# KyanChen/RSPrompter

Measured on NVIDIA H100. Metric: images/sec, higher is better.
Workload: dtype bf16

## Files before the change

### include/rsp_b200.h

```cpp
#ifndef RSP_B200_H_
#define RSP_B200_H_

#include <stdint.h>

#ifdef __cplusplus
extern "C" {
#endif

#define RSP_ABI_VERSION 2

int rsp_abi_version(void);
const char* rsp_last_error(void);

int rsp_gemm_bf16(const void* A, int lda, const void* W, int ldw, void* out, int ldo, int M, int N,
                  int K, const float* bias, const void* residual, int ldr, int res_fp32, int res_mod,
                  const int32_t* row_map, int act, int out_fp32, void* stream);

int rsp_conv3x3_nhwc_bf16(const void* x, int B, int H, int W, int C, const void* Wt, int ldw, void* out, int ldo,
                          int N, const float* bias, const void* residual, int ldr, int res_fp32, int act,
                          int out_fp32, void* stream);
int rsp_conv3x3_geometry_ok(int B, int H, int W, int C);

int rsp_gemm_bf16_simt(const void* A, int lda, const void* W, int ldw, void* out, int ldo, int M,
                       int N, int K, const float* bias, const void* residual, int ldr, int res_fp32,
                       int res_mod, const int32_t* row_map, int act, int out_fp32, void* stream);

int rsp_vit_attention(const void* qkv, const void* rel_h, const void* rel_w, void* out, int n_seq,
                      int T, int S, int H, int hd, void* stream);
int rsp_vit_attention_scatter(const void* qkv, const void* rel_h, const void* rel_w, void* out, int n_seq, int T,
                              int Sg, int H, int hd, const int32_t* out_row_map, void* stream);

int rsp_vit_attention_simt(const void* qkv, const void* rel_h, const void* rel_w, void* out,
                           int n_seq, int T, int S, int H, int hd, void* stream);

int rsp_layernorm(const void* in, int in_fp32, int ld_in, void* out, int out_fp32, int ld_out,
                  const float* gamma, const float* beta, const int32_t* src_map, int rows_out, int C,
                  float eps, int act, void* copy_out, int ld_copy, void* stream);

int rsp_layernorm_add(const void* x, const void* res, int res_fp32, const int32_t* res_block_map,
                      int res_block_rows, const float* gamma, const float* beta, void* out, const float* pos,
                      int pos_mod, void* out_pe, long long rows, int C, float eps, void* stream);

int rsp_patchify16(const float* img, void* out, int B, int H, int W, void* stream);

int rsp_im2col_nhwc(const void* in, void* out, int B, int H, int W, int C, int KH, int KW,
                    int stride, int pad, void* stream);

int rsp_nhwc_to_nchw(const void* in, int in_fp32, float* out, int B, int HW, int C, void* stream);

int rsp_gemm_bf16_ex(const void* A, int lda, const void* W, int ldw, void* out, int ldo, int M, int N,
                     int K, const float* bias, const void* residual, int ldr, int res_fp32, int res_mod,
                     const int32_t* row_map, int act, int out_fp32, int epi_mode, const float* ln_gamma,
                     const float* ln_beta, float ln_eps, const int32_t* res_block_map,
                     int res_block_rows, const float* hyper, float* mask_out, int grid_h, int grid_w,
                     void* stream);

int rsp_add_cast_bf16(const float* a, const float* b, void* out, long long n, long long b_mod,
                      void* stream);

int rsp_token_self_attention(const void* q, const void* k, const void* v, void* out, int N, int T,
                             int heads, int c, void* stream);
int rsp_t2i_attention(const void* q, const void* K, const void* V, int ldkv, const int32_t* kv_block, void* out,
                      int N, int Tq, int HW, void* stream);
int rsp_i2t_attention(const void* Q, const int32_t* q_block, const void* ktok, const void* vtok,
                      void* out, int N, int Tq, int HW, void* stream);


int rsp_rpn_decode(const float* head_out, int ld, const int64_t* topk_idx, int K, int B, int H, int W,
                   int A, int stride, const float* base_anchors, const float* stds4, float img_h, float img_w,
                   float min_size, int out_off, int out_ld, float* boxes, float* scores, void* stream);
int rsp_rpn_decode_shapes(const float* head_out, int ld, const int64_t* topk_idx, int K, int B, int H, int W, int A,
                          int stride, const float* base_anchors, const float* stds4, const float* img_shapes,
                          float min_size, int out_off, int out_ld, float* boxes, float* scores, void* stream);

int rsp_bbox_cls_decode(const float* cls, int ld_cls, const float* reg, int ld_reg, const float* rois,
                        const uint8_t* roi_valid, int n, int C, const float* stds4, float img_h, float img_w,
                        float score_thr, float* scores, float* boxes, int64_t* labels, void* stream);
int rsp_bbox_cls_decode_shapes(const float* cls, int ld_cls, const float* reg, int ld_reg, const float* rois,
                               const uint8_t* roi_valid, int n, int C, const float* stds4, const float* img_shapes,
                               float score_thr, float* scores, float* boxes, int64_t* labels, void* stream);

int rsp_nms_batched(const float* boxes, const int64_t* ids, const int32_t* nvalid, int B, int n, float thr,
                    void* mask_ws, float* max_coord_ws, uint8_t* keep, void* stream);
int rsp_nms_batched_topk(const float* boxes, const int64_t* ids, const int32_t* nvalid, int B, int n, float thr,
                         void* mask_ws, float* max_coord_ws, uint8_t* keep, int max_keep, void* stream);

int rsp_compact_keep(const uint8_t* keep, const float* boxes, const float* scores, const int64_t* labels,
                     int B, int n, int K, float* out_boxes, float* out_scores, int64_t* out_labels,
                     int32_t* out_index, int32_t* counts, void* stream);

int rsp_roi_align_nhwc(const void* const* feats, const float* const* pes, const int32_t* Hs,
                       const int32_t* Ws, const float* scales, int num_levels, const float* rois, int n,
                       int C, int P, float finest_scale, void* out, void* stream);

int rsp_mask_paste(const float* logits, uint8_t* out, int n, int hm, int wm, int H, int W, float thr,
                   int mode, void* stream);

int rsp_sigmoid_f32(const float* in, float* out, long long n, void* stream);

int rsp_pool2_nhwc(const void* in, void* out, int B, int H, int W, int C, int mode, void* stream);

int rsp_zero_border_nhwc(void* x, int N, int H, int W, int C, void* stream);

int rsp_sin_fold(const float* in, float* out, long long n_out, void* stream);


int rsp_groupnorm_nhwc(const void* x, float* stats_ws, const float* gamma, const float* beta, const void* up,
                       void* out, int B, int H, int W, int C, int G, float eps, int relu, void* stream);

int rsp_ms_deform_attn_sample(const void* value, const float* ow, int ld_ow, const int32_t* hs, const int32_t* ws,
                              int L, int P, int B, int NQ, void* out, void* stream);
int rsp_ms_deform_attn_sample_c(const void* value, const float* ow, int ld_ow, const int32_t* hs, const int32_t* ws,
                                int L, int P, int B, int NQ, void* out, int channels, void* stream);

int rsp_mha_small(const void* Q, int ldq, const void* K, int ldk, const void* V, int ldv, const uint64_t* mask_bits,
                  int B, int nq, int nk, void* out, void* stream);
int rsp_mha_small_hd(const void* Q, int ldq, const void* K, int ldk, const void* V, int ldv, const uint64_t* mask_bits,
                     int B, int nq, int nk, void* out, int head_dim, void* stream);

int rsp_attn_mask_bits(const float* logits, int ld, int rows, int nk, uint64_t* mask_bits, void* stream);

int rsp_resize_bilinear_nhwc(const void* x, int B, int H, int W, int C, int h, int w, void* out, void* stream);

int rsp_mask_embed_src(const float* mpp, const float* const* wts, const float* emb, const float* pos, int N,
                       int n_per_img, int hm, int wm, int h, int w, float eps, void* src, void* src_pe, void* stream);

int rsp_mask_paste_rescale(const float* maps, uint8_t* out, int n, int hm, int wm, int Hb, int Wb, int crop_h, int crop_w,
                           int H, int W, float thr, int mode, void* stream);

int rsp_query_postprocess_rescale(const float* logits, const int32_t* sel, const float* cls_scores, int n_inst, int hm,
                                  int wm, int Hb, int Wb, int crop_h, int crop_w, int H, int W, uint8_t* masks,
                                  float* part_ws, float* scores, float* boxes, void* stream);

int rsp_query_postprocess(const float* logits, const int32_t* sel, const float* cls_scores, int n_inst, int hm, int wm,
                          int H, int W, uint8_t* masks, float* part_ws, float* scores, float* boxes, void* stream);

int rsp_attn_softmax_bias(const float* scores, int lds, const float* tab, int ldt, int NT, void* P, int ldp, int n_rows,
                          int T, int S, float scale, void* stream);

int rsp_transpose_cols(const void* in, int ld, int col0, int C, int n_seq, int T, void* out, void* stream);

int rsp_split_heads(const void* in, int ld, int col0, int H, int hd, int n_seq, int T, void* out, void* stream);

int rsp_gemm_bf16_grouped(const void* A, int lda, const void* W, int ldw, void* out, int ldo, int M, int N, int K,
                          int m_group_rows, int w_group_rows, const int32_t* row_map, int out_fp32, void* stream);


int rsp_query_postprocess_bits(const float* logits, const int32_t* sel, const float* cls_scores, int n_inst, int hm,
                               int wm, uint8_t* bits, float* part_ws, float* scores, float* boxes, void* stream);

int rsp_mask_paste_bits(const float* maps, uint8_t* bits, int n, int hm, int wm, float thr, int mode, void* stream);

int rsp_mask_paste_boxes(const float* probs, const float* boxes, uint8_t* out, int n, int hm, int wm, int H, int W,
                         float thr, int packed, void* stream);

int rsp_pack_mask_bits(const uint8_t* masks, uint8_t* bits, long long rows, int W, void* stream);
int rsp_unpack_mask_bits(const uint8_t* bits, uint8_t* masks, long long rows, int W, void* stream);

int rsp_mask_rle_lengths(const uint8_t* src, int packed, const int64_t* desc, const int64_t* desc_host, int n,
                         int64_t* offsets, void* stream);
int rsp_mask_rle_write(const uint8_t* src, int packed, const int64_t* desc, int n, const int64_t* offsets, char* pool,
                       int32_t* lengths, void* stream);
int rsp_mask_rle_placed_lengths(const uint8_t* src, int packed, const int64_t* desc, const int64_t* desc_host, int n,
                                int64_t* offsets, void* stream);
int rsp_mask_rle_placed_write(const uint8_t* src, int packed, const int64_t* desc, int n, const int64_t* offsets,
                              char* pool, int32_t* lengths, void* stream);


int rsp_preprocess_u8(const uint8_t* img, int h, int w, long long stride_c, long long stride_y, long long stride_x,
                      float* out, int H, int W, const float* mean3, const float* std3, int swap_rb, float pad_value,
                      void* stream);

int rsp_patchify16_u8(const uint8_t* img, int hwc, void* out, int B, int H, int W, const float* mean3, const float* std3,
                      int swap_rb, void* stream);

int rsp_cast_f32_bf16(const float* in, void* out, long long n, void* stream);

int rsp_add_table_bf16(const void* x, const float* table, void* out, long long n, long long period, void* stream);

#ifdef __cplusplus
}
#endif
#endif
```

### rsprompter_b200/_lib.py

```python
from __future__ import annotations

import ctypes
import os
import subprocess
from pathlib import Path

import torch

_PKG_DIR = Path(__file__).resolve().parent
LIB_PATH = _PKG_DIR / "librsp_b200.so"
CSRC_DIR = _PKG_DIR / "csrc"


class RspError(RuntimeError):
    """Raised when an ``rsp_*`` entry point returns a non-zero status."""


def build_library(verbose: bool = False) -> Path:
    cmd = ["make", "-C", str(CSRC_DIR), "-j", str(os.cpu_count() or 4), "all"]
    res = subprocess.run(cmd, capture_output=True, text=True)
    if res.returncode != 0:
        raise RuntimeError(f"building librsp_b200.so failed:\n{res.stdout[-4000:]}\n{res.stderr[-4000:]}")
    if verbose:
        print(res.stdout[-2000:])
    return LIB_PATH


def _load() -> ctypes.CDLL:
    if not LIB_PATH.exists():
        raise ImportError(
            f"{LIB_PATH} not found: the CUDA extension is mandatory (no fallback path). "
            "Run `python -c 'import __graft_entry__ as g; g.build()'` or `make -C rsprompter_b200/csrc`.")
    return ctypes.CDLL(str(LIB_PATH))


_lib = _load()

_vp, _i, _f = ctypes.c_void_p, ctypes.c_int, ctypes.c_float

_SIGNATURES = {
    "rsp_abi_version": ([], _i),
    "rsp_last_error": ([], ctypes.c_char_p),
    "rsp_gemm_bf16": ([_vp, _i, _vp, _i, _vp, _i, _i, _i, _i, _vp, _vp, _i, _i, _i, _vp, _i, _i, _vp], _i),
    "rsp_gemm_bf16_simt": ([_vp, _i, _vp, _i, _vp, _i, _i, _i, _i, _vp, _vp, _i, _i, _i, _vp, _i, _i, _vp], _i),
    "rsp_vit_attention": ([_vp, _vp, _vp, _vp, _i, _i, _i, _i, _i, _vp], _i),
    "rsp_vit_attention_scatter": ([_vp, _vp, _vp, _vp, _i, _i, _i, _i, _i, _vp, _vp], _i),
    "rsp_vit_attention_simt": ([_vp, _vp, _vp, _vp, _i, _i, _i, _i, _i, _vp], _i),
    "rsp_layernorm": ([_vp, _i, _i, _vp, _i, _i, _vp, _vp, _vp, _i, _i, _f, _i, _vp, _i, _vp], _i),
    "rsp_patchify16": ([_vp, _vp, _i, _i, _i, _vp], _i),
    "rsp_layernorm_add": ([_vp, _vp, _i, _vp, _i, _vp, _vp, _vp, _vp, _i, _vp, ctypes.c_longlong, _i, _f, _vp], _i),
    "rsp_im2col_nhwc": ([_vp, _vp, _i, _i, _i, _i, _i, _i, _i, _i, _vp], _i),
    "rsp_nhwc_to_nchw": ([_vp, _i, _vp, _i, _i, _i, _vp], _i),
    "rsp_cast_f32_bf16": ([_vp, _vp, ctypes.c_longlong, _vp], _i),
    "rsp_add_table_bf16": ([_vp, _vp, _vp, ctypes.c_longlong, ctypes.c_longlong, _vp], _i),
    "rsp_gemm_bf16_ex": ([_vp, _i, _vp, _i, _vp, _i, _i, _i, _i, _vp, _vp, _i, _i, _i, _vp, _i, _i,
                          _i, _vp, _vp, _f, _vp, _i, _vp, _vp, _i, _i, _vp], _i),
    "rsp_add_cast_bf16": ([_vp, _vp, _vp, ctypes.c_longlong, ctypes.c_longlong, _vp], _i),
    "rsp_token_self_attention": ([_vp, _vp, _vp, _vp, _i, _i, _i, _i, _vp], _i),
    "rsp_t2i_attention": ([_vp, _vp, _vp, _i, _vp, _vp, _i, _i, _i, _vp], _i),
    "rsp_i2t_attention": ([_vp, _vp, _vp, _vp, _vp, _i, _i, _i, _vp], _i),
    "rsp_rpn_decode": ([_vp, _i, _vp, _i, _i, _i, _i, _i, _i, _vp, _vp, _f, _f, _f, _i, _i, _vp, _vp, _vp], _i),
    "rsp_bbox_cls_decode": ([_vp, _i, _vp, _i, _vp, _vp, _i, _i, _vp, _f, _f, _f, _vp, _vp, _vp, _vp], _i),
    "rsp_rpn_decode_shapes": ([_vp, _i, _vp, _i, _i, _i, _i, _i, _i, _vp, _vp, _vp, _f, _i, _i, _vp, _vp, _vp], _i),
    "rsp_nms_batched_topk": ([_vp, _vp, _vp, _i, _i, _f, _vp, _vp, _vp, _i, _vp], _i),
    "rsp_bbox_cls_decode_shapes": ([_vp, _i, _vp, _i, _vp, _vp, _i, _i, _vp, _vp, _f, _vp, _vp, _vp, _vp], _i),
    "rsp_nms_batched": ([_vp, _vp, _vp, _i, _i, _f, _vp, _vp, _vp, _vp], _i),
    "rsp_compact_keep": ([_vp, _vp, _vp, _vp, _i, _i, _i, _vp, _vp, _vp, _vp, _vp, _vp], _i),
    "rsp_roi_align_nhwc": ([_vp, _vp, _vp, _vp, _vp, _i, _vp, _i, _i, _i, _f, _vp, _vp], _i),
    "rsp_mask_paste": ([_vp, _vp, _i, _i, _i, _i, _i, _f, _i, _vp], _i),
    "rsp_pool2_nhwc": ([_vp, _vp, _i, _i, _i, _i, _i, _vp], _i),
    "rsp_zero_border_nhwc": ([_vp, _i, _i, _i, _i, _vp], _i),
    "rsp_sigmoid_f32": ([_vp, _vp, ctypes.c_longlong, _vp], _i),
    "rsp_mask_paste_boxes": ([_vp, _vp, _vp, _i, _i, _i, _i, _i, _f, _i, _vp], _i),
    "rsp_groupnorm_nhwc": ([_vp, _vp, _vp, _vp, _vp, _vp, _i, _i, _i, _i, _i, _f, _i, _vp], _i),
    "rsp_ms_deform_attn_sample": ([_vp, _vp, _i, _vp, _vp, _i, _i, _i, _i, _vp, _vp], _i),
    "rsp_mha_small": ([_vp, _i, _vp, _i, _vp, _i, _vp, _i, _i, _i, _vp, _vp], _i),
    "rsp_ms_deform_attn_sample_c": ([_vp, _vp, _i, _vp, _vp, _i, _i, _i, _i, _vp, _i, _vp], _i),
    "rsp_mha_small_hd": ([_vp, _i, _vp, _i, _vp, _i, _vp, _i, _i, _i, _vp, _i, _vp], _i),
    "rsp_conv3x3_nhwc_bf16": ([_vp, _i, _i, _i, _i, _vp, _i, _vp, _i, _i, _vp, _vp, _i, _i, _i, _i, _vp], _i),
    "rsp_conv3x3_geometry_ok": ([_i, _i, _i, _i], _i),
    "rsp_mask_paste_rescale": ([_vp, _vp, _i, _i, _i, _i, _i, _i, _i, _i, _i, ctypes.c_float, _i, _vp], _i),
    "rsp_query_postprocess_rescale": ([_vp, _vp, _vp, _i, _i, _i, _i, _i, _i, _i, _i, _i, _vp, _vp, _vp, _vp, _vp], _i),
    "rsp_attn_mask_bits": ([_vp, _i, _i, _i, _vp, _vp], _i),
    "rsp_resize_bilinear_nhwc": ([_vp, _i, _i, _i, _i, _i, _i, _vp, _vp], _i),
    "rsp_mask_embed_src": ([_vp, _vp, _vp, _vp, _i, _i, _i, _i, _i, _i, _f, _vp, _vp, _vp], _i),
    "rsp_query_postprocess": ([_vp, _vp, _vp, _i, _i, _i, _i, _i, _vp, _vp, _vp, _vp, _vp], _i),
    "rsp_sin_fold": ([_vp, _vp, ctypes.c_longlong, _vp], _i),
    "rsp_attn_softmax_bias": ([_vp, _i, _vp, _i, _i, _vp, _i, _i, _i, _i, _f, _vp], _i),
    "rsp_transpose_cols": ([_vp, _i, _i, _i, _i, _i, _vp, _vp], _i),
    "rsp_split_heads": ([_vp, _i, _i, _i, _i, _i, _i, _vp, _vp], _i),
    "rsp_gemm_bf16_grouped": ([_vp, _i, _vp, _i, _vp, _i, _i, _i, _i, _i, _i, _vp, _i, _vp], _i),
    "rsp_query_postprocess_bits": ([_vp, _vp, _vp, _i, _i, _i, _vp, _vp, _vp, _vp, _vp], _i),
    "rsp_mask_paste_bits": ([_vp, _vp, _i, _i, _i, _f, _i, _vp], _i),
    "rsp_pack_mask_bits": ([_vp, _vp, ctypes.c_longlong, _i, _vp], _i),
    "rsp_unpack_mask_bits": ([_vp, _vp, ctypes.c_longlong, _i, _vp], _i),
    "rsp_preprocess_u8": ([_vp, _i, _i, ctypes.c_longlong, ctypes.c_longlong, ctypes.c_longlong, _vp, _i, _i, _vp, _vp,
                           _i, _f, _vp], _i),
    "rsp_patchify16_u8": ([_vp, _i, _vp, _i, _i, _i, _vp, _vp, _i, _vp], _i),
    "rsp_mask_rle_lengths": ([_vp, _i, _vp, _vp, _i, _vp, _vp], _i),
    "rsp_mask_rle_write": ([_vp, _i, _vp, _i, _vp, _vp, _vp, _vp], _i),
    "rsp_mask_rle_placed_lengths": ([_vp, _i, _vp, _vp, _i, _vp, _vp], _i),
    "rsp_mask_rle_placed_write": ([_vp, _i, _vp, _i, _vp, _vp, _vp, _vp], _i),
}


def declared_symbols() -> list[str]:
    return sorted(_SIGNATURES)


for _name, (_args, _ret) in _SIGNATURES.items():
    _fn = getattr(_lib, _name)
    _fn.argtypes = _args
    _fn.restype = _ret

ABI_VERSION = _lib.rsp_abi_version()

launch_count = 0

trace: list | None = None
trace_scope = ""


def _log(kind: str, flops: float) -> None:
    if trace is not None:
        trace.append(dict(kind=kind, scope=trace_scope, flops=float(flops)))


def _check(status: int, what: str) -> None:
    if status != 0:
        msg = _lib.rsp_last_error()
        raise RspError(f"{what} failed (status {status}): {msg.decode() if msg else ''}")


def _ptr(t: torch.Tensor | None) -> int | None:
    if t is None:
        return None
    return t.data_ptr()


def _stream() -> int:
    return torch.cuda.current_stream().cuda_stream


def _require_cuda(*ts: torch.Tensor | None) -> None:
    cur = None
    for t in ts:
        if t is None:
            continue
        if not t.is_cuda:
            raise RspError("rsprompter_b200 kernels take CUDA tensors only (there is no CPU path)")
        if cur is None:
            cur = torch.cuda.current_device()
        if t.device.index != cur:
            raise RspError(f"tensor on cuda:{t.device.index} but the current device is cuda:{cur}: "
                           "wrap the call in torch.cuda.device(...) (one process per GPU is the supported layout)")


def _host_f4(v):
    v = tuple(float(x) for x in v)
    assert len(v) == 4
    return (ctypes.c_float * 4)(*v)


ACT = {None: 0, "none": 0, "gelu": 1, "relu": 2}


def gemm(a: torch.Tensor, w: torch.Tensor, bias: torch.Tensor | None = None, *,
         out: torch.Tensor | None = None, out_dtype: torch.dtype = torch.bfloat16,
         act: str | None = None, residual: torch.Tensor | None = None, res_mod: int = 0,
         row_map: torch.Tensor | None = None, out_rows: int | None = None,
         simt: bool = False, ln: tuple | None = None, ln64_gelu: tuple | None = None,
         res_block_map: torch.Tensor | None = None, res_block_rows: int = 0) -> torch.Tensor:
    global launch_count
    _require_cuda(a, w, bias, out, residual, row_map, res_block_map)
    assert a.dtype == torch.bfloat16 and w.dtype == torch.bfloat16, "gemm operands must be bf16"
    assert a.dim() == 2 and w.dim() == 2 and a.stride(1) == 1 and w.stride(1) == 1
    M, K = a.shape
    N, K2 = w.shape
    assert K == K2, f"gemm K mismatch {K} vs {K2}"
    if bias is not None:
        assert bias.dtype == torch.float32 and bias.numel() == N and bias.is_contiguous()
    if out is None:
        rows = out_rows if out_rows is not None else M
        out = torch.empty((rows, N), device=a.device, dtype=out_dtype)
    assert out.dim() == 2 and out.stride(1) == 1 and out.shape[1] >= N
    assert out.dtype in (torch.bfloat16, torch.float32)
    ldr = 0
    res_fp32 = 1
    if residual is not None:
        assert residual.dim() == 2 and residual.stride(1) == 1
        assert residual.dtype in (torch.bfloat16, torch.float32)
        ldr = residual.stride(0)
        res_fp32 = int(residual.dtype == torch.float32)
    if row_map is not None:
        assert row_map.dtype == torch.int32 and row_map.numel() == M and row_map.is_contiguous()
    if res_block_map is not None:
        assert res_block_map.dtype == torch.int32 and res_block_map.is_contiguous() and res_block_rows > 0
    epi, g, b, eps = 0, None, None, 1e-6
    if ln is not None:
        epi, (g, b, eps) = 1, ln
    elif ln64_gelu is not None:
        epi, (g, b, eps) = 2, ln64_gelu
    if epi or res_block_map is not None:
        assert not simt
        if g is not None:
            assert g.dtype == torch.float32 and b.dtype == torch.float32 and g.is_contiguous() and b.is_contiguous()
        st = _lib.rsp_gemm_bf16_ex(_ptr(a), a.stride(0), _ptr(w), w.stride(0), _ptr(out), out.stride(0),
                                   M, N, K, _ptr(bias), _ptr(residual), ldr, res_fp32, res_mod,
                                   _ptr(row_map), ACT[act], int(out.dtype == torch.float32), epi,
                                   _ptr(g), _ptr(b), float(eps), _ptr(res_block_map), res_block_rows,
                                   None, None, 0, 0, _stream())
    else:
        fn = _lib.rsp_gemm_bf16_simt if simt else _lib.rsp_gemm_bf16
        st = fn(_ptr(a), a.stride(0), _ptr(w), w.stride(0), _ptr(out), out.stride(0), M, N, K, _ptr(bias),
                _ptr(residual), ldr, res_fp32, res_mod, _ptr(row_map), ACT[act],
                int(out.dtype == torch.float32), _stream())
    _check(st, "rsp_gemm_bf16")
    launch_count += 1
    if not simt:
        _log("gemm", 2.0 * M * N * K)
    return out


def conv3x3_ok(B: int, H: int, W: int, C: int) -> bool:
    return bool(_lib.rsp_conv3x3_geometry_ok(B, H, W, C))


def conv3x3_nhwc(x: torch.Tensor, w: torch.Tensor, bias: torch.Tensor | None = None, *, act: str | None = None,
                 residual: torch.Tensor | None = None, out_dtype: torch.dtype = torch.bfloat16) -> torch.Tensor:
    global launch_count
    _require_cuda(x, w, bias, residual)
    B, H, W, C = x.shape
    N = w.shape[0]
    assert x.dtype == torch.bfloat16 and x.is_contiguous() and w.dtype == torch.bfloat16 and w.stride(1) == 1
    assert w.shape[1] == 9 * C
    if bias is not None:
        assert bias.dtype == torch.float32 and bias.numel() == N and bias.is_contiguous()
    ldr, res_fp32 = 0, 1
    if residual is not None:
        assert residual.dim() == 2 and residual.stride(1) == 1 and residual.shape[0] == B * H * W
        ldr, res_fp32 = residual.stride(0), int(residual.dtype == torch.float32)
    out = torch.empty(B * H * W, N, device=x.device, dtype=out_dtype)
    _check(_lib.rsp_conv3x3_nhwc_bf16(_ptr(x), B, H, W, C, _ptr(w), w.stride(0), _ptr(out), out.stride(0), N, _ptr(bias),
                                      _ptr(residual), ldr, res_fp32, ACT[act], int(out_dtype == torch.float32),
                                      _stream()), "rsp_conv3x3_nhwc_bf16")
    launch_count += 1
    _log("gemm", 2.0 * B * H * W * N * 9 * C)
    return out


def gemm_upscale_mask(a: torch.Tensor, w: torch.Tensor, bias: torch.Tensor, hyper: torch.Tensor,
                      grid_h: int, grid_w: int, out: torch.Tensor | None = None) -> torch.Tensor:
    global launch_count
    _require_cuda(a, w, bias, hyper, out)
    M, K = a.shape
    P = M // (4 * grid_h * grid_w)
    assert a.dtype == torch.bfloat16 and w.dtype == torch.bfloat16 and w.shape == (128, K)
    assert hyper.dtype == torch.float32 and hyper.shape == (P, 32) and hyper.is_contiguous()
    assert bias.dtype == torch.float32 and bias.numel() == 128
    if out is None:
        out = torch.empty((P, 4 * grid_h, 4 * grid_w), device=a.device, dtype=torch.float32)
    assert out.is_contiguous() and out.dtype == torch.float32
    st = _lib.rsp_gemm_bf16_ex(_ptr(a), a.stride(0), _ptr(w), w.stride(0), None, 0, M, 128, K, _ptr(bias),
                               None, 0, 1, 0, None, 0, 0, 3, None, None, 0.0, None, 0, _ptr(hyper),
                               _ptr(out), grid_h, grid_w, _stream())
    _check(st, "rsp_gemm_bf16_ex(upscale_mask)")
    launch_count += 1
    _log("gemm", 2.0 * M * 128 * K)
    return out


def add_cast_bf16(a: torch.Tensor, b: torch.Tensor | None = None, out: torch.Tensor | None = None) -> torch.Tensor:
    global launch_count
    _require_cuda(a, b, out)
    assert a.dtype == torch.float32 and a.is_contiguous()
    b_mod = 0
    if b is not None:
        assert b.dtype == torch.float32 and b.is_contiguous() and a.numel() % b.numel() == 0
        b_mod = b.numel() if b.numel() != a.numel() else 0
    if out is None:
        out = torch.empty(a.shape, device=a.device, dtype=torch.bfloat16)
    _check(_lib.rsp_add_cast_bf16(_ptr(a), _ptr(b), _ptr(out), a.numel(), b_mod, _stream()), "rsp_add_cast_bf16")
    launch_count += 1
    return out


def token_self_attention(q: torch.Tensor, k: torch.Tensor, v: torch.Tensor, heads: int) -> torch.Tensor:
    global launch_count
    _require_cuda(q, k, v)
    N, T, D = q.shape
    for t in (q, k, v):
        assert t.dtype == torch.bfloat16 and t.is_contiguous() and t.shape == (N, T, D)
    out = torch.empty_like(q)
    _check(_lib.rsp_token_self_attention(_ptr(q), _ptr(k), _ptr(v), _ptr(out), N, T, heads, D // heads, _stream()),
           "rsp_token_self_attention")
    launch_count += 1
    return out


def t2i_attention(q: torch.Tensor, K: torch.Tensor, V: torch.Tensor, hw: int,
                  kv_block: torch.Tensor | None = None) -> torch.Tensor:
    global launch_count
    _require_cuda(q, K, V, kv_block)
    N, Tq, C = q.shape
    assert C == 128 and q.dtype == torch.bfloat16 and q.is_contiguous()
    assert K.dtype == torch.bfloat16 and V.dtype == torch.bfloat16 and K.stride(1) == 1 and V.stride(1) == 1
    assert K.stride(0) == V.stride(0)
    assert K.shape[1] == 128 and V.shape == K.shape and K.shape[0] % hw == 0
    if kv_block is not None:
        assert kv_block.dtype == torch.int32 and kv_block.numel() == N and kv_block.is_contiguous()
    else:
        assert K.shape[0] == N * hw
    out = torch.empty_like(q)
    _check(_lib.rsp_t2i_attention(_ptr(q), _ptr(K), _ptr(V), K.stride(0), _ptr(kv_block), _ptr(out), N, Tq, hw, _stream()),
           "rsp_t2i_attention")
    launch_count += 1
    return out


def i2t_attention(Q: torch.Tensor, ktok: torch.Tensor, vtok: torch.Tensor, hw: int,
                  q_block: torch.Tensor | None = None) -> torch.Tensor:
    global launch_count
    _require_cuda(Q, ktok, vtok, q_block)
    N, Tq, C = ktok.shape
    assert C == 128 and Q.dtype == torch.bfloat16 and Q.is_contiguous() and Q.shape[1] == 128
    assert ktok.dtype == torch.bfloat16 and vtok.dtype == torch.bfloat16
    assert ktok.is_contiguous() and vtok.is_contiguous() and vtok.shape == ktok.shape
    if q_block is not None:
        assert q_block.dtype == torch.int32 and q_block.numel() == N and q_block.is_contiguous()
    else:
        assert Q.shape[0] == N * hw
    out = torch.empty((N * hw, 128), device=Q.device, dtype=torch.bfloat16)
    _check(_lib.rsp_i2t_attention(_ptr(Q), _ptr(q_block), _ptr(ktok), _ptr(vtok), _ptr(out), N, Tq, hw, _stream()),
           "rsp_i2t_attention")
    launch_count += 1
    return out


def vit_attention(qkv: torch.Tensor, rel_h: torch.Tensor, rel_w: torch.Tensor, n_seq: int, S: int,
                  H: int, hd: int, *, out: torch.Tensor | None = None, simt: bool = False,
                  out_row_map: torch.Tensor | None = None, out_rows: int | None = None) -> torch.Tensor:
    global launch_count
    _require_cuda(qkv, rel_h, rel_w, out)
    T = S * S
    D = H * hd
    if not simt and out_row_map is None and S not in (14, 32, 64) and T % 128 == 0 and S % 4 == 0:
        return vit_attention_generic(qkv, rel_h, rel_w, n_seq, S, H, hd, out=out)
    if not simt and S in (14, 32, 64):
        _log("attention_window" if S == 14 else "attention_global", 4.0 * n_seq * H * T * T * hd)
    assert qkv.dtype == torch.bfloat16 and qkv.is_contiguous() and qkv.shape == (n_seq * T, 3 * D)
    assert rel_h.dtype == torch.bfloat16 and rel_h.is_contiguous() and rel_h.shape == (2 * S - 1, hd)
    assert rel_w.dtype == torch.bfloat16 and rel_w.is_contiguous() and rel_w.shape == (2 * S - 1, hd)
    if out_row_map is not None:
        assert not simt and out_row_map.dtype == torch.int32 and out_row_map.is_contiguous()
        assert out_row_map.numel() == n_seq * T and out_rows is not None
        _require_cuda(out_row_map)
        if out is None:
            out = torch.empty((out_rows, D), device=qkv.device, dtype=torch.bfloat16)
        assert out.dtype == torch.bfloat16 and out.is_contiguous() and out.shape == (out_rows, D)
        _check(_lib.rsp_vit_attention_scatter(_ptr(qkv), _ptr(rel_h), _ptr(rel_w), _ptr(out), n_seq, T, S, H, hd,
                                              _ptr(out_row_map), _stream()), "rsp_vit_attention_scatter")
        launch_count += 1
        return out
    if out is None:
        out = torch.empty((n_seq * T, D), device=qkv.device, dtype=torch.bfloat16)
    assert out.dtype == torch.bfloat16 and out.is_contiguous() and out.shape == (n_seq * T, D)
    fn = _lib.rsp_vit_attention_simt if simt else _lib.rsp_vit_attention
    _check(fn(_ptr(qkv), _ptr(rel_h), _ptr(rel_w), _ptr(out), n_seq, T, S, H, hd, _stream()),
           "rsp_vit_attention")
    launch_count += 1
    return out


def gemm_grouped(a: torch.Tensor, w: torch.Tensor, out: torch.Tensor, N: int, m_group_rows: int, w_group_rows: int,
                 row_map: torch.Tensor | None = None) -> torch.Tensor:
    global launch_count
    _require_cuda(a, w, out, row_map)
    assert a.dtype == torch.bfloat16 and w.dtype == torch.bfloat16 and a.dim() == 2 and w.dim() == 2
    assert a.stride(1) == 1 and w.stride(1) == 1 and out.dim() == 2 and out.stride(1) == 1
    M, K = a.shape
    assert w.shape[1] == K and M % m_group_rows == 0 and m_group_rows % 128 == 0
    assert w.shape[0] >= (M // m_group_rows - 1) * w_group_rows + N and out.shape[1] >= N
    assert out.dtype in (torch.bfloat16, torch.float32)
    if row_map is not None:
        assert row_map.dtype == torch.int32 and row_map.numel() == M and row_map.is_contiguous()
    _check(_lib.rsp_gemm_bf16_grouped(_ptr(a), a.stride(0), _ptr(w), w.stride(0), _ptr(out), out.stride(0), M, N, K,
                                      m_group_rows, w_group_rows, _ptr(row_map), int(out.dtype == torch.float32),
                                      _stream()), "rsp_gemm_bf16_grouped")
    launch_count += 1
    _log("gemm", 2.0 * M * N * K)
    return out


_head_scatter_maps: dict = {}


def vit_attention_generic(qkv: torch.Tensor, rel_h: torch.Tensor, rel_w: torch.Tensor, n_seq: int, S: int, H: int,
                          hd: int, out: torch.Tensor | None = None) -> torch.Tensor:
    global launch_count
    _require_cuda(qkv, rel_h, rel_w, out)
    T, D = S * S, H * hd
    assert qkv.dtype == torch.bfloat16 and qkv.is_contiguous() and qkv.shape == (n_seq * T, 3 * D)
    assert T % 128 == 0 and S % 4 == 0 and hd % 8 == 0, "generic attention path: T % 128 == 0, S % 4 == 0"
    dev = qkv.device
    if out is None:
        out = torch.empty((n_seq * T, D), device=dev, dtype=torch.bfloat16)
    assert out.dtype == torch.bfloat16 and out.is_contiguous() and out.shape == (n_seq * T, D)
    NT = (2 * S - 1 + 15) // 16 * 16
    tabs = torch.zeros(2 * NT, hd, device=dev, dtype=torch.bfloat16)
    tabs[:2 * S - 1] = rel_h
    tabs[NT:NT + 2 * S - 1] = rel_w
    qh = torch.empty(n_seq, H * T, hd, device=dev, dtype=torch.bfloat16)
    kh = torch.empty(n_seq, H * T, hd, device=dev, dtype=torch.bfloat16)
    vt = torch.empty(n_seq, D, T, device=dev, dtype=torch.bfloat16)
    _check(_lib.rsp_split_heads(_ptr(qkv), 3 * D, 0, H, hd, n_seq, T, _ptr(qh), _stream()), "rsp_split_heads")
    _check(_lib.rsp_split_heads(_ptr(qkv), 3 * D, D, H, hd, n_seq, T, _ptr(kh), _stream()), "rsp_split_heads")
    _check(_lib.rsp_transpose_cols(_ptr(qkv), 3 * D, 2 * D, D, n_seq, T, _ptr(vt), _stream()), "rsp_transpose_cols")
    launch_count += 3
    key = (T, H, dev)
    if key not in _head_scatter_maps:
        t = torch.arange(T, device=dev, dtype=torch.int32)
        h = torch.arange(H, device=dev, dtype=torch.int32)
        _head_scatter_maps[key] = (t.view(1, T) * H + h.view(H, 1)).reshape(-1).contiguous()
    rmap = _head_scatter_maps[key]
    scores = torch.empty(H * T, T, device=dev, dtype=torch.float32)
    tab = torch.empty(H * T, 2 * NT, device=dev, dtype=torch.float32)
    P = torch.empty(H * T, T, device=dev, dtype=torch.bfloat16)
    scale = float(hd) ** -0.5
    for b in range(n_seq):
        gemm_grouped(qh[b], kh[b], scores, T, T, T)
        gemm(qh[b], tabs, out=tab)
        _check(_lib.rsp_attn_softmax_bias(_ptr(scores), T, _ptr(tab), 2 * NT, NT, _ptr(P), T, H * T, T, S, scale,
                                          _stream()), "rsp_attn_softmax_bias")
        launch_count += 1
        gemm_grouped(P, vt[b], out[b * T:(b + 1) * T].view(T * H, hd), hd, T, hd, row_map=rmap)
    return out


def layernorm(x: torch.Tensor, gamma: torch.Tensor, beta: torch.Tensor, eps: float, *,
              out: torch.Tensor | None = None, out_dtype: torch.dtype = torch.bfloat16,
              src_map: torch.Tensor | None = None, gelu: bool = False,
              copy_out: torch.Tensor | None = None) -> torch.Tensor:
    global launch_count
    _require_cuda(x, gamma, beta, out, src_map, copy_out)
    if copy_out is not None:
        assert x.dtype == torch.float32 and copy_out.dtype == torch.bfloat16 and copy_out.shape == x.shape
        assert copy_out.stride(1) == 1
    assert x.dim() == 2 and x.stride(1) == 1 and x.dtype in (torch.float32, torch.bfloat16)
    C = x.shape[1]
    assert gamma.dtype == torch.float32 and beta.dtype == torch.float32
    assert gamma.numel() == C and beta.numel() == C and gamma.is_contiguous() and beta.is_contiguous()
    rows_out = src_map.numel() if src_map is not None else x.shape[0]
    if src_map is not None:
        assert src_map.dtype == torch.int32 and src_map.is_contiguous()
    if out is None:
        out = torch.empty((rows_out, C), device=x.device, dtype=out_dtype)
    assert out.shape == (rows_out, C) and out.stride(1) == 1
    _check(_lib.rsp_layernorm(_ptr(x), int(x.dtype == torch.float32), x.stride(0), _ptr(out),
                              int(out.dtype == torch.float32), out.stride(0), _ptr(gamma), _ptr(beta),
                              _ptr(src_map), rows_out, C, float(eps), int(gelu), _ptr(copy_out),
                              copy_out.stride(0) if copy_out is not None else 0, _stream()),
           "rsp_layernorm")
    launch_count += 1
    return out


def patchify16(img: torch.Tensor, out: torch.Tensor | None = None) -> torch.Tensor:
    global launch_count
    _require_cuda(img, out)
    assert img.dtype == torch.float32 and img.is_contiguous() and img.dim() == 4 and img.shape[1] == 3
    B, _, H, W = img.shape
    rows = B * (H // 16) * (W // 16)
    if out is None:
        out = torch.empty((rows, 768), device=img.device, dtype=torch.bfloat16)
    assert out.shape == (rows, 768) and out.is_contiguous() and out.dtype == torch.bfloat16
    _check(_lib.rsp_patchify16(_ptr(img), _ptr(out), B, H, W, _stream()), "rsp_patchify16")
    launch_count += 1
    return out


def im2col_nhwc(x: torch.Tensor, kh: int, kw: int, stride: int, pad: int,
                out: torch.Tensor | None = None) -> torch.Tensor:
    global launch_count
    _require_cuda(x, out)
    assert x.dtype == torch.bfloat16 and x.is_contiguous() and x.dim() == 4
    B, H, W, C = x.shape
    Ho = (H + 2 * pad - kh) // stride + 1
    Wo = (W + 2 * pad - kw) // stride + 1
    if out is None:
        out = torch.empty((B * Ho * Wo, kh * kw * C), device=x.device, dtype=torch.bfloat16)
    assert out.shape == (B * Ho * Wo, kh * kw * C) and out.is_contiguous()
    _check(_lib.rsp_im2col_nhwc(_ptr(x), _ptr(out), B, H, W, C, kh, kw, stride, pad, _stream()),
           "rsp_im2col_nhwc")
    launch_count += 1
    return out


def nhwc_to_nchw(x: torch.Tensor, out: torch.Tensor | None = None) -> torch.Tensor:
    global launch_count
    _require_cuda(x, out)
    assert x.is_contiguous() and x.dim() == 4 and x.dtype in (torch.float32, torch.bfloat16)
    B, H, W, C = x.shape
    if out is None:
        out = torch.empty((B, C, H, W), device=x.device, dtype=torch.float32)
    assert out.shape == (B, C, H, W) and out.is_contiguous() and out.dtype == torch.float32
    _check(_lib.rsp_nhwc_to_nchw(_ptr(x), int(x.dtype == torch.float32), _ptr(out), B, H * W, C, _stream()),
           "rsp_nhwc_to_nchw")
    launch_count += 1
    return out


def cast_bf16(x: torch.Tensor, out: torch.Tensor | None = None) -> torch.Tensor:
    global launch_count
    _require_cuda(x, out)
    assert x.dtype == torch.float32 and x.is_contiguous()
    if out is None:
        out = torch.empty(x.shape, device=x.device, dtype=torch.bfloat16)
    assert out.is_contiguous() and out.numel() == x.numel() and out.dtype == torch.bfloat16
    _check(_lib.rsp_cast_f32_bf16(_ptr(x), _ptr(out), x.numel(), _stream()), "rsp_cast_f32_bf16")
    launch_count += 1
    return out


def add_table_bf16(x: torch.Tensor, table: torch.Tensor) -> torch.Tensor:
    global launch_count
    _require_cuda(x, table)
    assert x.dtype == torch.bfloat16 and x.is_contiguous() and table.dtype == torch.float32 and table.is_contiguous()
    assert x.numel() % table.numel() == 0 and table.numel() % 8 == 0
    out = torch.empty_like(x)
    _check(_lib.rsp_add_table_bf16(_ptr(x), _ptr(table), _ptr(out), x.numel(), table.numel(), _stream()),
           "rsp_add_table_bf16")
    launch_count += 1
    return out


def rpn_decode(head_out: torch.Tensor, topk_idx: torch.Tensor, B: int, H: int, W: int, A: int, stride: int,
               base_anchors: torch.Tensor, img_hw: tuple, min_size: float, boxes: torch.Tensor,
               scores: torch.Tensor, out_off: int, stds=(1.0, 1.0, 1.0, 1.0),
               img_shapes: torch.Tensor | None = None) -> None:
    global launch_count
    _require_cuda(head_out, topk_idx, base_anchors, boxes, scores)
    assert head_out.dtype == torch.float32 and head_out.dim() == 2 and head_out.stride(1) == 1
    assert topk_idx.dtype == torch.int64 and topk_idx.is_contiguous() and topk_idx.shape[0] == B
    assert boxes.is_contiguous() and scores.is_contiguous() and boxes.dtype == torch.float32
    K = topk_idx.shape[1]
    if img_shapes is not None:
        _require_cuda(img_shapes)
        assert img_shapes.dtype == torch.float32 and img_shapes.is_contiguous() and img_shapes.shape == (B, 2)
        _check(_lib.rsp_rpn_decode_shapes(_ptr(head_out), head_out.stride(0), _ptr(topk_idx), K, B, H, W, A, stride,
                                          _ptr(base_anchors), _host_f4(stds), _ptr(img_shapes), float(min_size), out_off,
                                          scores.shape[1], _ptr(boxes), _ptr(scores), _stream()), "rsp_rpn_decode_shapes")
        launch_count += 1
        return
    _check(_lib.rsp_rpn_decode(_ptr(head_out), head_out.stride(0), _ptr(topk_idx), K, B, H, W, A, stride,
                               _ptr(base_anchors), _host_f4(stds), float(img_hw[0]), float(img_hw[1]), float(min_size),
                               out_off, scores.shape[1], _ptr(boxes), _ptr(scores), _stream()), "rsp_rpn_decode")
    launch_count += 1


def bbox_cls_decode(cls: torch.Tensor, reg: torch.Tensor, rois: torch.Tensor, roi_valid: torch.Tensor | None,
                    C: int, img_hw: tuple, score_thr: float, stds=(0.1, 0.1, 0.2, 0.2),
                    img_shapes: torch.Tensor | None = None):
    global launch_count
    _require_cuda(cls, reg, rois, roi_valid)
    n = rois.shape[0]
    assert cls.dtype == torch.float32 and reg.dtype == torch.float32 and rois.dtype == torch.float32
    assert cls.stride(1) == 1 and reg.stride(1) == 1 and rois.is_contiguous() and rois.shape[1] == 5
    scores = torch.empty(n * C, device=cls.device, dtype=torch.float32)
    boxes = torch.empty(n * C, 4, device=cls.device, dtype=torch.float32)
    labels = torch.empty(n * C, device=cls.device, dtype=torch.int64)
    if roi_valid is not None:
        assert roi_valid.dtype == torch.uint8 and roi_valid.numel() == n
    if img_shapes is not None:
        _require_cuda(img_shapes)
        assert img_shapes.dtype == torch.float32 and img_shapes.is_contiguous() and img_shapes.shape[1] == 2
        _check(_lib.rsp_bbox_cls_decode_shapes(_ptr(cls), cls.stride(0), _ptr(reg), reg.stride(0), _ptr(rois),
                                               _ptr(roi_valid), n, C, _host_f4(stds), _ptr(img_shapes), float(score_thr),
                                               _ptr(scores), _ptr(boxes), _ptr(labels), _stream()),
               "rsp_bbox_cls_decode_shapes")
    else:
        _check(_lib.rsp_bbox_cls_decode(_ptr(cls), cls.stride(0), _ptr(reg), reg.stride(0), _ptr(rois),
                                        _ptr(roi_valid), n, C, _host_f4(stds), float(img_hw[0]), float(img_hw[1]),
                                        float(score_thr), _ptr(scores), _ptr(boxes), _ptr(labels), _stream()),
               "rsp_bbox_cls_decode")
    launch_count += 1
    return scores, boxes, labels


def nms_batched(boxes: torch.Tensor, ids: torch.Tensor, nvalid: torch.Tensor, iou_thr: float,
                max_keep: int = 0) -> torch.Tensor:
    global launch_count
    _require_cuda(boxes, ids, nvalid)
    B, n, _ = boxes.shape
    assert boxes.dtype == torch.float32 and boxes.is_contiguous()
    assert ids.dtype == torch.int64 and ids.is_contiguous() and ids.shape == (B, n)
    assert nvalid.dtype == torch.int32 and nvalid.numel() == B
    words = (n + 63) // 64
    mask_ws = torch.empty(B * n * words, device=boxes.device, dtype=torch.int64)
    mx = torch.empty(B, device=boxes.device, dtype=torch.float32)
    keep = torch.empty(B, n, device=boxes.device, dtype=torch.uint8)
    _check(_lib.rsp_nms_batched_topk(_ptr(boxes), _ptr(ids), _ptr(nvalid), B, n, float(iou_thr), _ptr(mask_ws),
                                     _ptr(mx), _ptr(keep), int(max_keep), _stream()), "rsp_nms_batched_topk")
    launch_count += 3
    return keep


def compact_keep(keep: torch.Tensor, boxes: torch.Tensor, scores: torch.Tensor, labels: torch.Tensor | None,
                 K: int):
    global launch_count
    _require_cuda(keep, boxes, scores, labels)
    B, n = keep.shape
    dev = keep.device
    ob = torch.empty(B, K, 4, device=dev, dtype=torch.float32)
    os_ = torch.empty(B, K, device=dev, dtype=torch.float32)
    ol = torch.empty(B, K, device=dev, dtype=torch.int64) if labels is not None else None
    oi = torch.empty(B, K, device=dev, dtype=torch.int32)
    cnt = torch.empty(B, device=dev, dtype=torch.int32)
    assert boxes.is_contiguous() and scores.is_contiguous() and keep.is_contiguous()
    _check(_lib.rsp_compact_keep(_ptr(keep), _ptr(boxes), _ptr(scores), _ptr(labels), B, n, K, _ptr(ob),
                                 _ptr(os_), _ptr(ol), _ptr(oi), _ptr(cnt), _stream()), "rsp_compact_keep")
    launch_count += 1
    return ob, os_, ol, oi, cnt
# ... 458 lines not shown
```

### rsprompter_b200/csrc/abi.cu

```cuda
#include "../../include/rsp_b200.h"

#include "attention.h"
#include "gemm.h"
#include "rowops.h"

namespace rsp { const char* last_error(); }
using namespace rsp;

static inline cudaStream_t S(void* s) { return static_cast<cudaStream_t>(s); }

extern "C" {

int rsp_abi_version(void) { return RSP_ABI_VERSION; }
const char* rsp_last_error(void) { return rsp::last_error(); }

static GemmArgs make_gemm_args(const void* A, int lda, const void* W, int ldw, void* out, int ldo,
                               int M, int N, int K, const float* bias, const void* residual, int ldr,
                               int res_fp32, int res_mod, const int32_t* row_map, int act,
                               int out_fp32) {
  GemmArgs a;
  a.A = A; a.lda = lda; a.W = W; a.ldw = ldw; a.out = out; a.ldo = ldo;
  a.M = M; a.N = N; a.K = K; a.bias = bias; a.residual = residual; a.ldr = ldr;
  a.res_fp32 = res_fp32; a.res_mod = res_mod; a.row_map = row_map; a.act = act;
  a.out_fp32 = out_fp32;
  return a;
}

int rsp_gemm_bf16(const void* A, int lda, const void* W, int ldw, void* out, int ldo, int M, int N,
                  int K, const float* bias, const void* residual, int ldr, int res_fp32, int res_mod,
                  const int32_t* row_map, int act, int out_fp32, void* stream) {
  return gemm_bf16(make_gemm_args(A, lda, W, ldw, out, ldo, M, N, K, bias, residual, ldr, res_fp32,
                                  res_mod, row_map, act, out_fp32), S(stream));
}

int rsp_gemm_bf16_grouped(const void* A, int lda, const void* W, int ldw, void* out, int ldo, int M, int N, int K,
                          int m_group_rows, int w_group_rows, const int32_t* row_map, int out_fp32, void* stream) {
  GemmArgs a = make_gemm_args(A, lda, W, ldw, out, ldo, M, N, K, nullptr, nullptr, 0, 1, 0, row_map, 0, out_fp32);
  a.m_group_rows = m_group_rows; a.w_group_rows = w_group_rows;
  return gemm_bf16(a, S(stream));
}

int rsp_conv3x3_nhwc_bf16(const void* x, int B, int H, int W, int C, const void* Wt, int ldw, void* out, int ldo,
                          int N, const float* bias, const void* residual, int ldr, int res_fp32, int act,
                          int out_fp32, void* stream) {
  GemmArgs a = make_gemm_args(x, C, Wt, ldw, out, ldo, B * H * W, N, 9 * C, bias, residual, ldr, res_fp32, 0,
                              nullptr, act, out_fp32);
  a.conv_b = B; a.conv_h = H; a.conv_w = W; a.conv_c = C;
  return conv3x3_bf16(a, S(stream));
}

int rsp_conv3x3_geometry_ok(int B, int H, int W, int C) { return conv3x3_geometry_ok(B, H, W, C) ? 1 : 0; }

int rsp_gemm_bf16_simt(const void* A, int lda, const void* W, int ldw, void* out, int ldo, int M,
                       int N, int K, const float* bias, const void* residual, int ldr, int res_fp32,
                       int res_mod, const int32_t* row_map, int act, int out_fp32, void* stream) {
  return gemm_bf16_simt(make_gemm_args(A, lda, W, ldw, out, ldo, M, N, K, bias, residual, ldr,
                                       res_fp32, res_mod, row_map, act, out_fp32), S(stream));
}

static AttentionArgs make_att_args(const void* qkv, const void* rel_h, const void* rel_w, void* out,
                                   int n_seq, int T, int Sg, int H, int hd, const int32_t* out_row_map = nullptr) {
  AttentionArgs a;
  a.qkv = qkv; a.rel_h = rel_h; a.rel_w = rel_w; a.out = out;
  a.n_seq = n_seq; a.T = T; a.S = Sg; a.H = H; a.hd = hd; a.out_row_map = out_row_map;
  return a;
}

int rsp_vit_attention(const void* qkv, const void* rel_h, const void* rel_w, void* out, int n_seq,
                      int T, int Sg, int H, int hd, void* stream) {
  return vit_attention(make_att_args(qkv, rel_h, rel_w, out, n_seq, T, Sg, H, hd), S(stream));
}

int rsp_vit_attention_scatter(const void* qkv, const void* rel_h, const void* rel_w, void* out, int n_seq, int T,
                              int Sg, int H, int hd, const int32_t* out_row_map, void* stream) {
  return vit_attention(make_att_args(qkv, rel_h, rel_w, out, n_seq, T, Sg, H, hd, out_row_map), S(stream));
}

int rsp_vit_attention_simt(const void* qkv, const void* rel_h, const void* rel_w, void* out,
                           int n_seq, int T, int Sg, int H, int hd, void* stream) {
  return vit_attention_simt(make_att_args(qkv, rel_h, rel_w, out, n_seq, T, Sg, H, hd), S(stream));
}

int rsp_attn_softmax_bias(const float* scores, int lds, const float* tab, int ldt, int NT, void* P, int ldp, int n_rows,
                          int T, int Sg, float scale, void* stream) {
  return attn_softmax_bias(scores, lds, tab, ldt, NT, P, ldp, n_rows, T, Sg, scale, S(stream));
}

int rsp_transpose_cols(const void* in, int ld, int col0, int C, int n_seq, int T, void* out, void* stream) {
  return transpose_cols(in, ld, col0, C, n_seq, T, out, S(stream));
}

int rsp_split_heads(const void* in, int ld, int col0, int H, int hd, int n_seq, int T, void* out, void* stream) {
  return split_heads(in, ld, col0, H, hd, n_seq, T, out, S(stream));
}

int rsp_layernorm(const void* in, int in_fp32, int ld_in, void* out, int out_fp32, int ld_out,
                  const float* gamma, const float* beta, const int32_t* src_map, int rows_out, int C,
                  float eps, int act, void* copy_out, int ld_copy, void* stream) {
  LayerNormArgs a;
  a.copy_out = copy_out; a.ld_copy = ld_copy;
  a.in = in; a.in_fp32 = in_fp32; a.ld_in = ld_in; a.out = out; a.out_fp32 = out_fp32;
  a.ld_out = ld_out; a.gamma = gamma; a.beta = beta; a.src_map = src_map; a.rows_out = rows_out;
  a.C = C; a.eps = eps; a.act = act;
  return layernorm_rows(a, S(stream));
}

int rsp_layernorm_add(const void* x, const void* res, int res_fp32, const int32_t* res_block_map,
                      int res_block_rows, const float* gamma, const float* beta, void* out, const float* pos,
                      int pos_mod, void* out_pe, long long rows, int C, float eps, void* stream) {
  return layernorm_add(x, res, res_fp32, res_block_map, res_block_rows, gamma, beta, out, pos, pos_mod, out_pe, rows,
                       C, eps, S(stream));
}

int rsp_patchify16(const float* img, void* out, int B, int H, int W, void* stream) {
  return patchify16(img, out, B, H, W, S(stream));
}

int rsp_im2col_nhwc(const void* in, void* out, int B, int H, int W, int C, int KH, int KW,
                    int stride, int pad, void* stream) {
  return im2col_nhwc(in, out, B, H, W, C, KH, KW, stride, pad, S(stream));
}

int rsp_nhwc_to_nchw(const void* in, int in_fp32, float* out, int B, int HW, int C, void* stream) {
  return nhwc_to_nchw(in, in_fp32, out, B, HW, C, S(stream));
}

int rsp_cast_f32_bf16(const float* in, void* out, long long n, void* stream) {
  return cast_f32_bf16(in, out, n, S(stream));
}

int rsp_add_table_bf16(const void* x, const float* table, void* out, long long n, long long period, void* stream) {
  return add_table_bf16(x, table, out, n, period, S(stream));
}

}

#include "decoder.h"

extern "C" {

int rsp_gemm_bf16_ex(const void* A, int lda, const void* W, int ldw, void* out, int ldo, int M, int N,
                     int K, const float* bias, const void* residual, int ldr, int res_fp32, int res_mod,
                     const int32_t* row_map, int act, int out_fp32, int epi_mode, const float* ln_gamma,
                     const float* ln_beta, float ln_eps, const int32_t* res_block_map,
                     int res_block_rows, const float* hyper, float* mask_out, int grid_h, int grid_w,
                     void* stream) {
  GemmArgs a = make_gemm_args(A, lda, W, ldw, out, ldo, M, N, K, bias, residual, ldr, res_fp32,
                              res_mod, row_map, act, out_fp32);
  a.epi_mode = epi_mode; a.ln_gamma = ln_gamma; a.ln_beta = ln_beta; a.ln_eps = ln_eps;
  a.res_block_map = res_block_map; a.res_block_rows = res_block_rows;
  a.hyper = hyper; a.mask_out = mask_out; a.grid_h = grid_h; a.grid_w = grid_w;
  return gemm_bf16(a, S(stream));
}

int rsp_add_cast_bf16(const float* a, const float* b, void* out, long long n, long long b_mod,
                      void* stream) {
  return add_cast_bf16(a, b, out, n, b_mod, S(stream));
}

int rsp_token_self_attention(const void* q, const void* k, const void* v, void* out, int N, int T,
                             int heads, int c, void* stream) {
  return token_self_attention(q, k, v, out, N, T, heads, c, S(stream));
}

int rsp_t2i_attention(const void* q, const void* K, const void* V, int ldkv, const int32_t* kv_block, void* out,
                      int N, int Tq, int HW, void* stream) {
  return t2i_attention(q, K, V, ldkv, kv_block, out, N, Tq, HW, S(stream));
}

int rsp_i2t_attention(const void* Q, const int32_t* q_block, const void* ktok, const void* vtok,
                      void* out, int N, int Tq, int HW, void* stream) {
  return i2t_attention(Q, q_block, ktok, vtok, out, N, Tq, HW, S(stream));
}

}

#include "detect.h"

extern "C" {

int rsp_rpn_decode(const float* head_out, int ld, const int64_t* topk_idx, int K, int B, int H, int W,
                   int A, int stride, const float* base_anchors, const float* stds4, float img_h, float img_w,
                   float min_size, int out_off, int out_ld, float* boxes, float* scores, void* stream) {
  return rpn_decode(head_out, ld, reinterpret_cast<const long long*>(topk_idx), K, B, H, W, A, stride,
                    base_anchors, stds4, img_h, img_w, nullptr, min_size, out_off, out_ld, boxes, scores, S(stream));
}

int rsp_rpn_decode_shapes(const float* head_out, int ld, const int64_t* topk_idx, int K, int B, int H, int W, int A,
                          int stride, const float* base_anchors, const float* stds4, const float* img_shapes,
                          float min_size, int out_off, int out_ld, float* boxes, float* scores, void* stream) {
  RSP_CHECK_ARG(img_shapes, "rpn_decode_shapes: img_shapes is null");
  return rpn_decode(head_out, ld, reinterpret_cast<const long long*>(topk_idx), K, B, H, W, A, stride,
                    base_anchors, stds4, 0.f, 0.f, img_shapes, min_size, out_off, out_ld, boxes, scores, S(stream));
}

int rsp_bbox_cls_decode(const float* cls, int ld_cls, const float* reg, int ld_reg, const float* rois,
                        const uint8_t* roi_valid, int n, int C, const float* stds4, float img_h, float img_w,
                        float score_thr, float* scores, float* boxes, int64_t* labels, void* stream) {
  return bbox_cls_decode(cls, ld_cls, reg, ld_reg, rois, roi_valid, n, C, stds4, img_h, img_w, nullptr, score_thr,
                         scores, boxes, reinterpret_cast<long long*>(labels), S(stream));
}

int rsp_bbox_cls_decode_shapes(const float* cls, int ld_cls, const float* reg, int ld_reg, const float* rois,
                               const uint8_t* roi_valid, int n, int C, const float* stds4, const float* img_shapes,
                               float score_thr, float* scores, float* boxes, int64_t* labels, void* stream) {
  RSP_CHECK_ARG(img_shapes, "bbox_cls_decode_shapes: img_shapes is null");
  return bbox_cls_decode(cls, ld_cls, reg, ld_reg, rois, roi_valid, n, C, stds4, 0.f, 0.f, img_shapes, score_thr,
                         scores, boxes, reinterpret_cast<long long*>(labels), S(stream));
}

int rsp_nms_batched(const float* boxes, const int64_t* ids, const int32_t* nvalid, int B, int n, float thr,
                    void* mask_ws, float* max_coord_ws, uint8_t* keep, void* stream) {
  return nms_batched(boxes, reinterpret_cast<const long long*>(ids), nvalid, B, n, thr,
                     static_cast<unsigned long long*>(mask_ws), max_coord_ws, keep, 0, S(stream));
}

int rsp_nms_batched_topk(const float* boxes, const int64_t* ids, const int32_t* nvalid, int B, int n, float thr,
                         void* mask_ws, float* max_coord_ws, uint8_t* keep, int max_keep, void* stream) {
  return nms_batched(boxes, reinterpret_cast<const long long*>(ids), nvalid, B, n, thr,
                     static_cast<unsigned long long*>(mask_ws), max_coord_ws, keep, max_keep, S(stream));
}

int rsp_compact_keep(const uint8_t* keep, const float* boxes, const float* scores, const int64_t* labels,
                     int B, int n, int K, float* out_boxes, float* out_scores, int64_t* out_labels,
                     int32_t* out_index, int32_t* counts, void* stream) {
  return compact_keep(keep, boxes, scores, reinterpret_cast<const long long*>(labels), B, n, K, out_boxes,
                      out_scores, reinterpret_cast<long long*>(out_labels), out_index, counts, S(stream));
}

int rsp_roi_align_nhwc(const void* const* feats, const float* const* pes, const int32_t* Hs,
                       const int32_t* Ws, const float* scales, int num_levels, const float* rois, int n,
                       int C, int P, float finest_scale, void* out, void* stream) {
  return roi_align_nhwc(feats, pes, Hs, Ws, scales, num_levels, rois, n, C, P, finest_scale, out, S(stream));
}

int rsp_mask_paste(const float* logits, uint8_t* out, int n, int hm, int wm, int H, int W, float thr,
                   int mode, void* stream) {
  return mask_paste(logits, out, n, hm, wm, H, W, thr, mode, S(stream));
}

int rsp_sigmoid_f32(const float* in, float* out, long long n, void* stream) {
  return sigmoid_f32(in, out, n, S(stream));
}

int rsp_pool2_nhwc(const void* in, void* out, int B, int H, int W, int C, int mode, void* stream) {
  return pool2_nhwc(in, out, B, H, W, C, mode, S(stream));
}

int rsp_zero_border_nhwc(void* x, int N, int H, int W, int C, void* stream) {
  return zero_border_nhwc(x, N, H, W, C, S(stream));
}

int rsp_sin_fold(const float* in, float* out, long long n_out, void* stream) {
  return sin_fold(in, out, n_out, S(stream));
}

}

#include "query.h"

extern "C" {

int rsp_groupnorm_nhwc(const void* x, float* stats_ws, const float* gamma, const float* beta, const void* up,
                       void* out, int B, int H, int W, int C, int G, float eps, int relu, void* stream) {
  return groupnorm_nhwc(x, stats_ws, gamma, beta, up, out, B, H, W, C, G, eps, relu, S(stream));
}

int rsp_ms_deform_attn_sample(const void* value, const float* ow, int ld_ow, const int32_t* hs, const int32_t* ws,
                              int L, int P, int B, int NQ, void* out, void* stream) {
  return ms_deform_attn_sample(value, ow, ld_ow, hs, ws, L, P, B, NQ, out, 128, S(stream));
}

int rsp_ms_deform_attn_sample_c(const void* value, const float* ow, int ld_ow, const int32_t* hs, const int32_t* ws,
                                int L, int P, int B, int NQ, void* out, int channels, void* stream) {
  return ms_deform_attn_sample(value, ow, ld_ow, hs, ws, L, P, B, NQ, out, channels, S(stream));
}

int rsp_mha_small(const void* Q, int ldq, const void* K, int ldk, const void* V, int ldv, const uint64_t* mask_bits,
                  int B, int nq, int nk, void* out, void* stream) {
  return mha_small(Q, ldq, K, ldk, V, ldv, reinterpret_cast<const unsigned long long*>(mask_bits), B, nq, nk, out, 16,
                   S(stream));
}

int rsp_mha_small_hd(const void* Q, int ldq, const void* K, int ldk, const void* V, int ldv, const uint64_t* mask_bits,
                     int B, int nq, int nk, void* out, int head_dim, void* stream) {
  return mha_small(Q, ldq, K, ldk, V, ldv, reinterpret_cast<const unsigned long long*>(mask_bits), B, nq, nk, out,
                   head_dim, S(stream));
}

int rsp_attn_mask_bits(const float* logits, int ld, int rows, int nk, uint64_t* mask_bits, void* stream) {
  return attn_mask_bits(logits, ld, rows, nk, reinterpret_cast<unsigned long long*>(mask_bits), S(stream));
}

int rsp_resize_bilinear_nhwc(const void* x, int B, int H, int W, int C, int h, int w, void* out, void* stream) {
  return resize_bilinear_nhwc(x, B, H, W, C, h, w, out, S(stream));
}

int rsp_mask_embed_src(const float* mpp, const float* const* wts, const float* emb, const float* pos, int N,
                       int n_per_img, int hm, int wm, int h, int w, float eps, void* src, void* src_pe, void* stream) {
  return mask_embed_src(mpp, wts, emb, pos, N, n_per_img, hm, wm, h, w, eps, src, src_pe, S(stream));
}

int rsp_mask_paste_rescale(const float* maps, uint8_t* out, int n, int hm, int wm, int Hb, int Wb, int crop_h, int crop_w,
                           int H, int W, float thr, int mode, void* stream) {
  return mask_paste_rescale(maps, out, n, hm, wm, Hb, Wb, crop_h, crop_w, H, W, thr, mode, S(stream));
}

int rsp_query_postprocess_rescale(const float* logits, const int32_t* sel, const float* cls_scores, int n_inst, int hm,
                                  int wm, int Hb, int Wb, int crop_h, int crop_w, int H, int W, uint8_t* masks,
                                  float* part_ws, float* scores, float* boxes, void* stream) {
  return query_postprocess_rescale(logits, sel, cls_scores, n_inst, hm, wm, Hb, Wb, crop_h, crop_w, H, W, masks, part_ws,
                                   scores, boxes, S(stream));
}

int rsp_query_postprocess(const float* logits, const int32_t* sel, const float* cls_scores, int n_inst, int hm, int wm,
                          int H, int W, uint8_t* masks, float* part_ws, float* scores, float* boxes, void* stream) {
  return query_postprocess(logits, sel, cls_scores, n_inst, hm, wm, H, W, masks, part_ws, scores, boxes, S(stream));
}

int rsp_query_postprocess_bits(const float* logits, const int32_t* sel, const float* cls_scores, int n_inst, int hm,
                               int wm, uint8_t* bits, float* part_ws, float* scores, float* boxes, void* stream) {
  return query_postprocess_bits(logits, sel, cls_scores, n_inst, hm, wm, bits, part_ws, scores, boxes, S(stream));
}

int rsp_mask_paste_boxes(const float* probs, const float* boxes, uint8_t* out, int n, int hm, int wm, int H, int W,
                         float thr, int packed, void* stream) {
  return mask_paste_boxes(probs, boxes, out, n, hm, wm, H, W, thr, packed, S(stream));
}

int rsp_mask_paste_bits(const float* maps, uint8_t* bits, int n, int hm, int wm, float thr, int mode, void* stream) {
  return mask_paste_bits(maps, bits, n, hm, wm, thr, mode, S(stream));
}

}

#include "records.h"

extern "C" {

int rsp_pack_mask_bits(const uint8_t* masks, uint8_t* bits, long long rows, int W, void* stream) {
  return pack_mask_bits(masks, bits, rows, W, S(stream));
}

int rsp_unpack_mask_bits(const uint8_t* bits, uint8_t* masks, long long rows, int W, void* stream) {
  return unpack_mask_bits(bits, masks, rows, W, S(stream));
}

int rsp_preprocess_u8(const uint8_t* img, int h, int w, long long stride_c, long long stride_y, long long stride_x,
                      float* out, int H, int W, const float* mean3, const float* std3, int swap_rb, float pad_value,
                      void* stream) {
  return preprocess_u8(img, h, w, stride_c, stride_y, stride_x, out, H, W, mean3, std3, swap_rb, pad_value, S(stream));
}

int rsp_patchify16_u8(const uint8_t* img, int hwc, void* out, int B, int H, int W, const float* mean3, const float* std3,
                      int swap_rb, void* stream) {
  return patchify16_u8(img, hwc, out, B, H, W, mean3, std3, swap_rb, S(stream));
}

}

#include "rle.h"

extern "C" {

int rsp_mask_rle_lengths(const uint8_t* src, int packed, const int64_t* desc, const int64_t* desc_host, int n,
                         int64_t* offsets, void* stream) {
  return mask_rle_lengths(src, packed, reinterpret_cast<const long long*>(desc),
                          reinterpret_cast<const long long*>(desc_host), n, reinterpret_cast<long long*>(offsets),
                          S(stream));
}

int rsp_mask_rle_write(const uint8_t* src, int packed, const int64_t* desc, int n, const int64_t* offsets, char* pool,
                       int32_t* lengths, void* stream) {
  return mask_rle_write(src, packed, reinterpret_cast<const long long*>(desc), n,
                        reinterpret_cast<const long long*>(offsets), pool, lengths, S(stream));
}

int rsp_mask_rle_placed_lengths(const uint8_t* src, int packed, const int64_t* desc, const int64_t* desc_host, int n,
                                int64_t* offsets, void* stream) {
  return mask_rle_placed_lengths(src, packed, reinterpret_cast<const long long*>(desc),
                                 reinterpret_cast<const long long*>(desc_host), n, reinterpret_cast<long long*>(offsets),
                                 S(stream));
}

int rsp_mask_rle_placed_write(const uint8_t* src, int packed, const int64_t* desc, int n, const int64_t* offsets,
                              char* pool, int32_t* lengths, void* stream) {
  return mask_rle_placed_write(src, packed, reinterpret_cast<const long long*>(desc), n,
                               reinterpret_cast<const long long*>(offsets), pool, lengths, S(stream));
}

}
```

### rsprompter_b200/csrc/decoder.cu

```cuda
#include "decoder.h"
#include "sm90.cuh"

namespace rsp {

__device__ __forceinline__ void unpack8(const uint4& u, float (&f)[8]) {
  const uint32_t w[4] = {u.x, u.y, u.z, u.w};
#pragma unroll
  for (int j = 0; j < 4; ++j) {
    const __nv_bfloat162 h = *reinterpret_cast<const __nv_bfloat162*>(&w[j]);
    f[2 * j] = __bfloat162float(h.x);
    f[2 * j + 1] = __bfloat162float(h.y);
  }
}

__global__ void add_cast_bf16_kernel(const float* __restrict__ a, const float* __restrict__ b,
                                     __nv_bfloat16* __restrict__ out, long long n, long long b_mod) {
  const long long i = (static_cast<long long>(blockIdx.x) * blockDim.x + threadIdx.x) * 4;
  if (i >= n) return;
  float4 x = *reinterpret_cast<const float4*>(a + i);
  if (b) {
    const float4 y = *reinterpret_cast<const float4*>(b + (b_mod > 0 ? i % b_mod : i));
    x.x += y.x; x.y += y.y; x.z += y.z; x.w += y.w;
  }
  *reinterpret_cast<uint2*>(out + i) = make_uint2(pack_bf16x2(x.x, x.y), pack_bf16x2(x.z, x.w));
}

int add_cast_bf16(const float* a, const float* b, void* out, long long n, long long b_mod,
                  cudaStream_t stream) {
  RSP_CHECK_ARG(a && out && n > 0 && n % 4 == 0 && (b_mod == 0 || b_mod % 4 == 0), "add_cast: bad args");
  const long long n4 = n / 4;
  add_cast_bf16_kernel<<<static_cast<unsigned>((n4 + 255) / 256), 256, 0, stream>>>(
      a, b, static_cast<__nv_bfloat16*>(out), n, b_mod);
  RSP_CHECK_LAUNCH();
  return RSP_OK;
}

template <int C>
__global__ void token_self_attention_kernel(const __nv_bfloat16* __restrict__ q,
                                            const __nv_bfloat16* __restrict__ k,
                                            const __nv_bfloat16* __restrict__ v,
                                            __nv_bfloat16* __restrict__ out, int N, int T, int heads,
                                            float scale) {
  const int gw = (blockIdx.x * blockDim.x + threadIdx.x) >> 5;
  const int lane = threadIdx.x & 31;
  if (gw >= N * heads) return;
  const int n = gw / heads, h = gw % heads;
  const int D = heads * C;
  if (lane >= T) return;
  const __nv_bfloat16* qp = q + (static_cast<size_t>(n) * T + lane) * D + h * C;
  float qf[C];
#pragma unroll
  for (int d = 0; d < C; d += 8) {
    float t[8];
    unpack8(*reinterpret_cast<const uint4*>(qp + d), t);
#pragma unroll
    for (int j = 0; j < 8; ++j) qf[d + j] = t[j];
  }
  float s[16];
  float mx = -INFINITY;
  for (int j = 0; j < T; ++j) {
    const __nv_bfloat16* kp = k + (static_cast<size_t>(n) * T + j) * D + h * C;
    float acc = 0.f;
#pragma unroll
    for (int d = 0; d < C; d += 8) {
      float t[8];
      unpack8(*reinterpret_cast<const uint4*>(kp + d), t);
#pragma unroll
      for (int jj = 0; jj < 8; ++jj) acc += qf[d + jj] * t[jj];
    }
    s[j] = acc * scale;
    mx = fmaxf(mx, s[j]);
  }
  float l = 0.f;
  float o[C];
#pragma unroll
  for (int d = 0; d < C; ++d) o[d] = 0.f;
  for (int j = 0; j < T; ++j) {
    const float pj = __expf(s[j] - mx);
    l += pj;
    const __nv_bfloat16* vp = v + (static_cast<size_t>(n) * T + j) * D + h * C;
#pragma unroll
    for (int d = 0; d < C; d += 8) {
      float t[8];
      unpack8(*reinterpret_cast<const uint4*>(vp + d), t);
#pragma unroll
      for (int jj = 0; jj < 8; ++jj) o[d + jj] += pj * t[jj];
    }
  }
  const float inv = 1.0f / l;
  __nv_bfloat16* op = out + (static_cast<size_t>(n) * T + lane) * D + h * C;
#pragma unroll
  for (int d = 0; d < C; d += 8)
    *reinterpret_cast<uint4*>(op + d) =
        make_uint4(pack_bf16x2(o[d] * inv, o[d + 1] * inv), pack_bf16x2(o[d + 2] * inv, o[d + 3] * inv),
                   pack_bf16x2(o[d + 4] * inv, o[d + 5] * inv), pack_bf16x2(o[d + 6] * inv, o[d + 7] * inv));
}

int token_self_attention(const void* q, const void* k, const void* v, void* out, int N, int T,
                         int heads, int c, cudaStream_t stream) {
  RSP_CHECK_ARG(q && k && v && out && N > 0 && T > 0 && T <= 16 && heads > 0, "token_self_attention: bad args");
  RSP_CHECK_ARG(c == 32 || c == 16, "token_self_attention: per-head dim %d (16 or 32)", c);
  const int warps = N * heads;
  const int threads = 128;
  const int blocks = (warps * 32 + threads - 1) / threads;
  const float scale = 1.0f / sqrtf(static_cast<float>(c));
  if (c == 32)
    token_self_attention_kernel<32><<<blocks, threads, 0, stream>>>(
        static_cast<const __nv_bfloat16*>(q), static_cast<const __nv_bfloat16*>(k),
        static_cast<const __nv_bfloat16*>(v), static_cast<__nv_bfloat16*>(out), N, T, heads, scale);
  else
    token_self_attention_kernel<16><<<blocks, threads, 0, stream>>>(
        static_cast<const __nv_bfloat16*>(q), static_cast<const __nv_bfloat16*>(k),
        static_cast<const __nv_bfloat16*>(v), static_cast<__nv_bfloat16*>(out), N, T, heads, scale);
  RSP_CHECK_LAUNCH();
  return RSP_OK;
}

constexpr int T2I_TILE = 64;
constexpr int T2I_ROWB = 272;
constexpr int T2I_STAGE = 2 * T2I_TILE * T2I_ROWB;

__device__ __forceinline__ void mma_bf16_16816(float (&d)[4], const uint32_t (&a)[4], uint32_t b0, uint32_t b1) {
  asm volatile(
      "mma.sync.aligned.m16n8k16.row.col.f32.bf16.bf16.f32 {%0, %1, %2, %3}, {%4, %5, %6, %7}, {%8, %9}, "
      "{%0, %1, %2, %3};"
      : "+f"(d[0]), "+f"(d[1]), "+f"(d[2]), "+f"(d[3])
      : "r"(a[0]), "r"(a[1]), "r"(a[2]), "r"(a[3]), "r"(b0), "r"(b1));
}

__device__ __forceinline__ void cp_async16(uint32_t dst, const void* src) {
  asm volatile("cp.async.cg.shared.global [%0], [%1], 16;" ::"r"(dst), "l"(src) : "memory");
}

__global__ void __launch_bounds__(256)
t2i_attention_kernel(const __nv_bfloat16* __restrict__ q,
                     const __nv_bfloat16* __restrict__ K,
                     const __nv_bfloat16* __restrict__ V,
                     const int* __restrict__ kv_block,
                     __nv_bfloat16* __restrict__ out,
                     int Tq, int HW, int ldkv, float scale) {
  extern __shared__ __align__(16) uint8_t t2i_smem[];
  const uint32_t s_base = smem_u32(t2i_smem);
  const int n = blockIdx.x;
  const int blk = kv_block ? kv_block[n] : n;
  const __nv_bfloat16* Kb = K + static_cast<size_t>(blk) * HW * ldkv;
  const __nv_bfloat16* Vb = V + static_cast<size_t>(blk) * HW * ldkv;
  const int tid = threadIdx.x, lane = tid & 31, h = tid >> 5;
  const int g = lane >> 2, t = lane & 3;
  const int n_tiles = (HW + T2I_TILE - 1) / T2I_TILE;

  auto issue_tile = [&](int tile, int stage) {
    const int t0 = tile * T2I_TILE;
#pragma unroll
    for (int i = 0; i < 8; ++i) {
      const int idx = tid + i * 256;
      const int which = idx >> 10, j = idx & 1023;
      const int row = j >> 4, ch = j & 15;
      const int grow = min(t0 + row, HW - 1);
      const __nv_bfloat16* src = (which ? Vb : Kb) + static_cast<size_t>(grow) * ldkv + ch * 8;
      cp_async16(s_base + stage * T2I_STAGE + which * (T2I_TILE * T2I_ROWB) + row * T2I_ROWB + ch * 16, src);
    }
    asm volatile("cp.async.commit_group;" ::: "memory");
  };

  uint32_t qa[4];
  {
    auto ldq = [&](int row, int col) -> uint32_t {
      if (row >= Tq) return 0u;
      const __nv_bfloat162 v = *reinterpret_cast<const __nv_bfloat162*>(
          q + (static_cast<size_t>(n) * Tq + row) * 128 + h * 16 + col);
      return pack_bf16x2(__bfloat162float(v.x) * scale, __bfloat162float(v.y) * scale);
    };
    qa[0] = ldq(g, 2 * t); qa[1] = ldq(g + 8, 2 * t); qa[2] = ldq(g, 2 * t + 8); qa[3] = ldq(g + 8, 2 * t + 8);
  }
  float m0 = -INFINITY, m1 = -INFINITY, l0 = 0.f, l1 = 0.f;
  float o[2][4] = {{0.f, 0.f, 0.f, 0.f}, {0.f, 0.f, 0.f, 0.f}};

  issue_tile(0, 0);
  for (int tile = 0; tile < n_tiles; ++tile) {
    const int stage = tile & 1;
    if (tile + 1 < n_tiles) {
      issue_tile(tile + 1, stage ^ 1);
      asm volatile("cp.async.wait_group 1;" ::: "memory");
    } else {
      asm volatile("cp.async.wait_group 0;" ::: "memory");
    }
    __syncthreads();
    const uint32_t sK = s_base + stage * T2I_STAGE + h * 32;
    const uint32_t sV = sK + T2I_TILE * T2I_ROWB;
    const int valid = min(T2I_TILE, HW - tile * T2I_TILE);
    float s[8][4];
#pragma unroll
    for (int j = 0; j < 8; ++j) {
      uint32_t b0, b1;
      const uint32_t addr = sK + (j * 8 + g) * T2I_ROWB + t * 4;
      asm volatile("ld.shared.b32 %0, [%1];" : "=r"(b0) : "r"(addr));
      asm volatile("ld.shared.b32 %0, [%1];" : "=r"(b1) : "r"(addr + 16));
      s[j][0] = s[j][1] = s[j][2] = s[j][3] = 0.f;
      mma_bf16_16816(s[j], qa, b0, b1);
      if (valid < T2I_TILE) {
        const int key = j * 8 + 2 * t;
        if (key >= valid) { s[j][0] = -INFINITY; s[j][2] = -INFINITY; }
        if (key + 1 >= valid) { s[j][1] = -INFINITY; s[j][3] = -INFINITY; }
      }
    }
    float mx0 = -INFINITY, mx1 = -INFINITY;
#pragma unroll
    for (int j = 0; j < 8; ++j) {
      mx0 = fmaxf(mx0, fmaxf(s[j][0], s[j][1]));
      mx1 = fmaxf(mx1, fmaxf(s[j][2], s[j][3]));
    }
    mx0 = fmaxf(mx0, __shfl_xor_sync(0xffffffffu, mx0, 1)); mx0 = fmaxf(mx0, __shfl_xor_sync(0xffffffffu, mx0, 2));
    mx1 = fmaxf(mx1, __shfl_xor_sync(0xffffffffu, mx1, 1)); mx1 = fmaxf(mx1, __shfl_xor_sync(0xffffffffu, mx1, 2));
    const float mn0 = fmaxf(m0, mx0), mn1 = fmaxf(m1, mx1);
    const float a0 = __expf(m0 - mn0), a1 = __expf(m1 - mn1);
    m0 = mn0; m1 = mn1;
    float ps0 = 0.f, ps1 = 0.f;
#pragma unroll
    for (int j = 0; j < 8; ++j) {
      s[j][0] = __expf(s[j][0] - mn0); s[j][1] = __expf(s[j][1] - mn0);
      s[j][2] = __expf(s[j][2] - mn1); s[j][3] = __expf(s[j][3] - mn1);
      ps0 += s[j][0] + s[j][1];
      ps1 += s[j][2] + s[j][3];
    }
    l0 = l0 * a0 + ps0; l1 = l1 * a1 + ps1;
#pragma unroll
    for (int d = 0; d < 2; ++d) { o[d][0] *= a0; o[d][1] *= a0; o[d][2] *= a1; o[d][3] *= a1; }
#pragma unroll
    for (int c = 0; c < 4; ++c) {
      uint32_t pa[4];
      pa[0] = pack_bf16x2(s[2 * c][0], s[2 * c][1]);
      pa[1] = pack_bf16x2(s[2 * c][2], s[2 * c][3]);
      pa[2] = pack_bf16x2(s[2 * c + 1][0], s[2 * c + 1][1]);
      pa[3] = pack_bf16x2(s[2 * c + 1][2], s[2 * c + 1][3]);
#pragma unroll
      for (int d = 0; d < 2; ++d) {
        const uint32_t addr = sV + (c * 16 + 2 * t) * T2I_ROWB + (d * 8 + g) * 2;
        uint16_t v00, v01, v10, v11;
        asm volatile("ld.shared.u16 %0, [%1];" : "=h"(v00) : "r"(addr));
        asm volatile("ld.shared.u16 %0, [%1];" : "=h"(v01) : "r"(addr + T2I_ROWB));
        asm volatile("ld.shared.u16 %0, [%1];" : "=h"(v10) : "r"(addr + 8 * T2I_ROWB));
        asm volatile("ld.shared.u16 %0, [%1];" : "=h"(v11) : "r"(addr + 9 * T2I_ROWB));
        const uint32_t b0 = static_cast<uint32_t>(v00) | (static_cast<uint32_t>(v01) << 16);
        const uint32_t b1 = static_cast<uint32_t>(v10) | (static_cast<uint32_t>(v11) << 16);
        mma_bf16_16816(o[d], pa, b0, b1);
      }
    }
    __syncthreads();
  }
  l0 += __shfl_xor_sync(0xffffffffu, l0, 1); l0 += __shfl_xor_sync(0xffffffffu, l0, 2);
  l1 += __shfl_xor_sync(0xffffffffu, l1, 1); l1 += __shfl_xor_sync(0xffffffffu, l1, 2);
  const float i0 = 1.0f / l0, i1 = 1.0f / l1;
#pragma unroll
  for (int d = 0; d < 2; ++d) {
    if (g < Tq)
      *reinterpret_cast<uint32_t*>(out + (static_cast<size_t>(n) * Tq + g) * 128 + h * 16 + d * 8 + 2 * t) =
          pack_bf16x2(o[d][0] * i0, o[d][1] * i0);
    if (g + 8 < Tq)
      *reinterpret_cast<uint32_t*>(out + (static_cast<size_t>(n) * Tq + g + 8) * 128 + h * 16 + d * 8 + 2 * t) =
          pack_bf16x2(o[d][2] * i1, o[d][3] * i1);
  }
}

int t2i_attention(const void* q, const void* K, const void* V, int ldkv, const int* kv_block, void* out, int N,
                  int Tq, int HW, cudaStream_t stream) {
  RSP_CHECK_ARG(q && K && V && out && N > 0 && Tq > 0 && Tq <= 16 && HW > 0, "t2i_attention: bad args");
  RSP_CHECK_ARG(ldkv >= 128 && ldkv % 8 == 0 && (reinterpret_cast<uintptr_t>(K) & 15) == 0 &&
                (reinterpret_cast<uintptr_t>(V) & 15) == 0, "t2i_attention: K / V row stride / alignment");
  const int smem = 2 * T2I_STAGE;
  static bool attr_set_dev[kMaxDevices] = {};
  bool& attr_set = attr_set_dev[current_device()];
  if (!attr_set) {
    RSP_CHECK_CUDA(cudaFuncSetAttribute(t2i_attention_kernel, cudaFuncAttributeMaxDynamicSharedMemorySize, smem));
    attr_set = true;
  }
  t2i_attention_kernel<<<N, 256, smem, stream>>>(
      static_cast<const __nv_bfloat16*>(q), static_cast<const __nv_bfloat16*>(K),
      static_cast<const __nv_bfloat16*>(V), kv_block, static_cast<__nv_bfloat16*>(out), Tq, HW, ldkv, 0.25f);
  RSP_CHECK_LAUNCH();
  return RSP_OK;
}

constexpr int I2T_PIX = 128;
constexpr int I2T_ROWB = 272;

__global__ void __launch_bounds__(256)
i2t_attention_kernel(const __nv_bfloat16* __restrict__ Q,
                     const int* __restrict__ q_block,
                     const __nv_bfloat16* __restrict__ ktok,
                     const __nv_bfloat16* __restrict__ vtok,
                     __nv_bfloat16* __restrict__ out,
                     int Tq, int HW, float scale) {
  __shared__ __align__(16) uint8_t tile[I2T_PIX * I2T_ROWB];
  const uint32_t s_tile = smem_u32(tile);
  const int n = blockIdx.y;
  const int p0 = blockIdx.x * I2T_PIX;
  const int tid = threadIdx.x, lane = tid & 31, h = tid >> 5;
  const int g = lane >> 2, t = lane & 3;
  const int blk = q_block ? q_block[n] : n;
  const __nv_bfloat16* Qb = Q + (static_cast<size_t>(blk) * HW + p0) * 128;
  const int npix = min(I2T_PIX, HW - p0);
#pragma unroll
  for (int i = 0; i < 8; ++i) {
    const int idx = tid + i * 256;
    const int row = idx >> 4, ch = idx & 15;
    const int srow = min(row, npix - 1);
    cp_async16(s_tile + row * I2T_ROWB + ch * 16, Qb + static_cast<size_t>(srow) * 128 + ch * 8);
  }
  asm volatile("cp.async.commit_group;" ::: "memory");
  uint32_t kb[2][2], vb[2][2];
  {
    const __nv_bfloat16* kp = ktok + static_cast<size_t>(n) * Tq * 128 + h * 16;
    const __nv_bfloat16* vp = vtok + static_cast<size_t>(n) * Tq * 128 + h * 16;
#pragma unroll
    for (int j = 0; j < 2; ++j) {
      const int tok = j * 8 + g;
      kb[j][0] = kb[j][1] = 0u;
      if (tok < Tq) {
        const __nv_bfloat162 k0 = *reinterpret_cast<const __nv_bfloat162*>(kp + tok * 128 + 2 * t);
        const __nv_bfloat162 k1 = *reinterpret_cast<const __nv_bfloat162*>(kp + tok * 128 + 2 * t + 8);
        kb[j][0] = pack_bf16x2(__bfloat162float(k0.x) * scale, __bfloat162float(k0.y) * scale);
        kb[j][1] = pack_bf16x2(__bfloat162float(k1.x) * scale, __bfloat162float(k1.y) * scale);
      }
      auto ldv = [&](int tok2) -> uint32_t {
        return tok2 < Tq ? static_cast<uint32_t>(*reinterpret_cast<const uint16_t*>(vp + tok2 * 128 + j * 8 + g)) : 0u;
      };
      vb[j][0] = ldv(2 * t) | (ldv(2 * t + 1) << 16);
      vb[j][1] = ldv(2 * t + 8) | (ldv(2 * t + 9) << 16);
    }
  }
  asm volatile("cp.async.wait_group 0;" ::: "memory");
  __syncthreads();
  const uint32_t sq = s_tile + h * 32;
#pragma unroll 2
  for (int c = 0; c < I2T_PIX / 16; ++c) {
    uint32_t qa[4];
    const uint32_t a0 = sq + (c * 16 + g) * I2T_ROWB + t * 4;
    asm volatile("ld.shared.b32 %0, [%1];" : "=r"(qa[0]) : "r"(a0));
    asm volatile("ld.shared.b32 %0, [%1];" : "=r"(qa[1]) : "r"(a0 + 8 * I2T_ROWB));
    asm volatile("ld.shared.b32 %0, [%1];" : "=r"(qa[2]) : "r"(a0 + 16));
    asm volatile("ld.shared.b32 %0, [%1];" : "=r"(qa[3]) : "r"(a0 + 8 * I2T_ROWB + 16));
    float s0[4] = {0.f, 0.f, 0.f, 0.f}, s1[4] = {0.f, 0.f, 0.f, 0.f};
    mma_bf16_16816(s0, qa, kb[0][0], kb[0][1]);
    mma_bf16_16816(s1, qa, kb[1][0], kb[1][1]);
    if (2 * t >= Tq) { s0[0] = -INFINITY; s0[2] = -INFINITY; }
    if (2 * t + 1 >= Tq) { s0[1] = -INFINITY; s0[3] = -INFINITY; }
    if (8 + 2 * t >= Tq) { s1[0] = -INFINITY; s1[2] = -INFINITY; }
    if (9 + 2 * t >= Tq) { s1[1] = -INFINITY; s1[3] = -INFINITY; }
    float m0 = fmaxf(fmaxf(s0[0], s0[1]), fmaxf(s1[0], s1[1]));
    float m1 = fmaxf(fmaxf(s0[2], s0[3]), fmaxf(s1[2], s1[3]));
    m0 = fmaxf(m0, __shfl_xor_sync(0xffffffffu, m0, 1)); m0 = fmaxf(m0, __shfl_xor_sync(0xffffffffu, m0, 2));
    m1 = fmaxf(m1, __shfl_xor_sync(0xffffffffu, m1, 1)); m1 = fmaxf(m1, __shfl_xor_sync(0xffffffffu, m1, 2));
    s0[0] = __expf(s0[0] - m0); s0[1] = __expf(s0[1] - m0); s1[0] = __expf(s1[0] - m0); s1[1] = __expf(s1[1] - m0);
    s0[2] = __expf(s0[2] - m1); s0[3] = __expf(s0[3] - m1); s1[2] = __expf(s1[2] - m1); s1[3] = __expf(s1[3] - m1);
    float l0 = s0[0] + s0[1] + s1[0] + s1[1], l1 = s0[2] + s0[3] + s1[2] + s1[3];
    l0 += __shfl_xor_sync(0xffffffffu, l0, 1); l0 += __shfl_xor_sync(0xffffffffu, l0, 2);
    l1 += __shfl_xor_sync(0xffffffffu, l1, 1); l1 += __shfl_xor_sync(0xffffffffu, l1, 2);
    uint32_t pa[4] = {pack_bf16x2(s0[0], s0[1]), pack_bf16x2(s0[2], s0[3]), pack_bf16x2(s1[0], s1[1]),
                      pack_bf16x2(s1[2], s1[3])};
    float o0[4] = {0.f, 0.f, 0.f, 0.f}, o1[4] = {0.f, 0.f, 0.f, 0.f};
    mma_bf16_16816(o0, pa, vb[0][0], vb[0][1]);
    mma_bf16_16816(o1, pa, vb[1][0], vb[1][1]);
    const float i0 = 1.0f / l0, i1 = 1.0f / l1;
    __syncwarp();
    asm volatile("st.shared.b32 [%0], %1;" ::"r"(a0), "r"(pack_bf16x2(o0[0] * i0, o0[1] * i0)) : "memory");
    asm volatile("st.shared.b32 [%0], %1;" ::"r"(a0 + 8 * I2T_ROWB), "r"(pack_bf16x2(o0[2] * i1, o0[3] * i1)) : "memory");
    asm volatile("st.shared.b32 [%0], %1;" ::"r"(a0 + 16), "r"(pack_bf16x2(o1[0] * i0, o1[1] * i0)) : "memory");
    asm volatile("st.shared.b32 [%0], %1;" ::"r"(a0 + 8 * I2T_ROWB + 16), "r"(pack_bf16x2(o1[2] * i1, o1[3] * i1)) : "memory");
  }
  __syncthreads();
  __nv_bfloat16* Ob = out + (static_cast<size_t>(n) * HW + p0) * 128;
#pragma unroll
  for (int i = 0; i < 8; ++i) {
    const int idx = tid + i * 256;
    const int row = idx >> 4, ch = idx & 15;
    if (row < npix)
      *reinterpret_cast<uint4*>(Ob + static_cast<size_t>(row) * 128 + ch * 8) =
          *reinterpret_cast<const uint4*>(tile + row * I2T_ROWB + ch * 16);
  }
}

int i2t_attention(const void* Q, const int* q_block, const void* ktok, const void* vtok, void* out,
                  int N, int Tq, int HW, cudaStream_t stream) {
  RSP_CHECK_ARG(Q && ktok && vtok && out && N > 0 && Tq > 0 && Tq <= 16 && HW > 0, "i2t_attention: bad args");
  dim3 grid((HW + I2T_PIX - 1) / I2T_PIX, N);
  i2t_attention_kernel<<<grid, 256, 0, stream>>>(
      static_cast<const __nv_bfloat16*>(Q), q_block, static_cast<const __nv_bfloat16*>(ktok),
      static_cast<const __nv_bfloat16*>(vtok), static_cast<__nv_bfloat16*>(out), Tq, HW, 0.25f);
  RSP_CHECK_LAUNCH();
  return RSP_OK;
}

}
```

### rsprompter_b200/csrc/decoder.h

```cpp
#pragma once
#include "host_util.h"

namespace rsp {

int add_cast_bf16(const float* a, const float* b, void* out, long long n, long long b_mod,
                  cudaStream_t stream);
int token_self_attention(const void* q, const void* k, const void* v, void* out, int N, int T,
                         int heads, int c, cudaStream_t stream);
int t2i_attention(const void* q, const void* K, const void* V, int ldkv, const int* kv_block, void* out, int N,
                  int Tq, int HW, cudaStream_t stream);
int i2t_attention(const void* Q, const int* q_block, const void* ktok, const void* vtok, void* out,
                  int N, int Tq, int HW, cudaStream_t stream);

}
```

### rsprompter_b200/csrc/sm90.cuh

```cuda
#pragma once
#include <cuda.h>
#include <cuda_bf16.h>
#include <cuda_runtime.h>
#include <stdint.h>

namespace rsp {

__device__ __forceinline__ uint32_t smem_u32(const void* p) {
  return static_cast<uint32_t>(__cvta_generic_to_shared(p));
}

__device__ __forceinline__ uint32_t elect_one() {
  uint32_t pred = 0;
  asm volatile(
      "{\n"
      ".reg .b32 rx;\n"
      ".reg .pred px;\n"
      "elect.sync rx|px, 0xffffffff;\n"
      "selp.u32 %0, 1, 0, px;\n"
      "}\n"
      : "=r"(pred));
  return pred;
}

__device__ __forceinline__ void mbar_init(uint32_t bar, uint32_t count) {
  asm volatile("mbarrier.init.shared::cta.b64 [%0], %1;" ::"r"(bar), "r"(count) : "memory");
}
__device__ __forceinline__ void fence_barrier_init() {
  asm volatile("fence.mbarrier_init.release.cluster;" ::: "memory");
}
__device__ __forceinline__ void fence_proxy_async_smem() {
  asm volatile("fence.proxy.async.shared::cta;" ::: "memory");
}
__device__ __forceinline__ void mbar_expect_tx(uint32_t bar, uint32_t bytes) {
  asm volatile("mbarrier.arrive.expect_tx.shared::cta.b64 _, [%0], %1;" ::"r"(bar), "r"(bytes)
               : "memory");
}
__device__ __forceinline__ void mbar_arrive(uint32_t bar) {
  asm volatile("mbarrier.arrive.shared::cta.b64 _, [%0];" ::"r"(bar) : "memory");
}
__device__ __forceinline__ uint32_t mbar_try_wait(uint32_t bar, uint32_t parity) {
  uint32_t ok;
  asm volatile(
      "{\n"
      ".reg .pred p;\n"
      "mbarrier.try_wait.parity.shared::cta.b64 p, [%1], %2;\n"
      "selp.u32 %0, 1, 0, p;\n"
      "}\n"
      : "=r"(ok)
      : "r"(bar), "r"(parity)
      : "memory");
  return ok;
}
__device__ __forceinline__ void mbar_wait(uint32_t bar, uint32_t parity) {
  if (mbar_try_wait(bar, parity)) return;
  long long t0 = clock64();
  uint32_t spins = 0;
  while (!mbar_try_wait(bar, parity)) {
    if ((++spins & 0x3ff) == 0 && clock64() - t0 > (1ll << 31)) __trap();
  }
}

__device__ __forceinline__ void tma_prefetch_desc(const CUtensorMap* m) {
  asm volatile("prefetch.tensormap [%0];" ::"l"(m) : "memory");
}
__device__ __forceinline__ void tma_load_2d(uint32_t dst, const CUtensorMap* m, uint32_t bar,
                                            int c0, int c1) {
  asm volatile(
      "cp.async.bulk.tensor.2d.shared::cluster.global.mbarrier::complete_tx::bytes"
      " [%0], [%1, {%3, %4}], [%2];" ::"r"(dst),
      "l"(m), "r"(bar), "r"(c0), "r"(c1)
      : "memory");
}
__device__ __forceinline__ void tma_load_3d(uint32_t dst, const CUtensorMap* m, uint32_t bar,
                                            int c0, int c1, int c2) {
  asm volatile(
      "cp.async.bulk.tensor.3d.shared::cluster.global.mbarrier::complete_tx::bytes"
      " [%0], [%1, {%3, %4, %5}], [%2];" ::"r"(dst),
      "l"(m), "r"(bar), "r"(c0), "r"(c1), "r"(c2)
      : "memory");
}
__device__ __forceinline__ void tma_load_4d(uint32_t dst, const CUtensorMap* m, uint32_t bar,
                                            int c0, int c1, int c2, int c3) {
  asm volatile(
      "cp.async.bulk.tensor.4d.shared::cluster.global.mbarrier::complete_tx::bytes"
      " [%0], [%1, {%3, %4, %5, %6}], [%2];" ::"r"(dst),
      "l"(m), "r"(bar), "r"(c0), "r"(c1), "r"(c2), "r"(c3)
      : "memory");
}

__device__ __forceinline__ void tma_store_2d(const CUtensorMap* m, uint32_t src, int c0, int c1) {
  asm volatile("cp.async.bulk.tensor.2d.global.shared::cta.bulk_group [%0, {%2, %3}], [%1];" ::"l"(m), "r"(src),
               "r"(c0), "r"(c1)
               : "memory");
}
__device__ __forceinline__ void bulk_commit() { asm volatile("cp.async.bulk.commit_group;" ::: "memory"); }
__device__ __forceinline__ void bulk_wait_read0() { asm volatile("cp.async.bulk.wait_group.read 0;" ::: "memory"); }
__device__ __forceinline__ void bulk_wait0() { asm volatile("cp.async.bulk.wait_group 0;" ::: "memory"); }

__device__ __forceinline__ uint64_t make_gdesc(uint32_t saddr, uint32_t lbo_bytes, uint32_t sbo_bytes) {
  uint64_t d = 0;
  d |= static_cast<uint64_t>((saddr & 0x3ffff) >> 4);
  d |= static_cast<uint64_t>((lbo_bytes >> 4) & 0x3fff) << 16;
  d |= static_cast<uint64_t>((sbo_bytes >> 4) & 0x3fff) << 32;
  d |= 1ull << 62;
  return d;
}

__device__ __forceinline__ uint64_t make_gdesc_sw32(uint32_t saddr, uint32_t lbo_bytes, uint32_t sbo_bytes) {
  uint64_t d = 0;
  d |= static_cast<uint64_t>((saddr & 0x3ffff) >> 4);
  d |= static_cast<uint64_t>((lbo_bytes >> 4) & 0x3fff) << 16;
  d |= static_cast<uint64_t>((sbo_bytes >> 4) & 0x3fff) << 32;
  d |= 3ull << 62;
  return d;
}

__device__ __forceinline__ void wgmma_fence() { asm volatile("wgmma.fence.sync.aligned;" ::: "memory"); }
__device__ __forceinline__ void wgmma_commit() { asm volatile("wgmma.commit_group.sync.aligned;" ::: "memory"); }
template <int N>
__device__ __forceinline__ void wgmma_wait() { asm volatile("wgmma.wait_group.sync.aligned %0;" ::"n"(N) : "memory"); }
template <int R>
__device__ __forceinline__ void acc_fence(float (&d)[R]) {
#pragma unroll
  for (int i = 0; i < R; ++i) asm volatile("" : "+f"(d[i])::"memory");
}

template <int N>
struct Wgmma;
template <> struct Wgmma<32> {
  template <int TB>
  __device__ __forceinline__ static void ss(float (&d)[16], uint64_t a, uint64_t b, uint32_t acc) {
    asm volatile(
        "{\n.reg .pred p;\n"
        "setp.ne.b32 p, %18, 0;\n"
        "wgmma.mma_async.sync.aligned.m64n32k16.f32.bf16.bf16 "
        "{" 
        "%0, %1, %2, %3, %4, %5, %6, %7, %8, %9, %10, %11, %12, %13, %14, %15"
        "}, %16, %17, p, 1, 1, 0, %19;\n}\n"
        : "+f"(d[0]), "+f"(d[1]), "+f"(d[2]), "+f"(d[3]), "+f"(d[4]), "+f"(d[5]), "+f"(d[6]), "+f"(d[7]),
          "+f"(d[8]), "+f"(d[9]), "+f"(d[10]), "+f"(d[11]), "+f"(d[12]), "+f"(d[13]), "+f"(d[14]), "+f"(d[15])
        : "l"(a), "l"(b), "r"(acc), "n"(TB));
  }
};
template <> struct Wgmma<64> {
  template <int TB>
  __device__ __forceinline__ static void ss(float (&d)[32], uint64_t a, uint64_t b, uint32_t acc) {
    asm volatile(
        "{\n.reg .pred p;\n"
        "setp.ne.b32 p, %34, 0;\n"
        "wgmma.mma_async.sync.aligned.m64n64k16.f32.bf16.bf16 "
        "{" 
        "%0, %1, %2, %3, %4, %5, %6, %7, %8, %9, %10, %11, %12, %13, %14, %15, "
        "%16, %17, %18, %19, %20, %21, %22, %23, %24, %25, %26, %27, %28, %29, %30, %31"
        "}, %32, %33, p, 1, 1, 0, %35;\n}\n"
        : "+f"(d[0]), "+f"(d[1]), "+f"(d[2]), "+f"(d[3]), "+f"(d[4]), "+f"(d[5]), "+f"(d[6]), "+f"(d[7]),
          "+f"(d[8]), "+f"(d[9]), "+f"(d[10]), "+f"(d[11]), "+f"(d[12]), "+f"(d[13]), "+f"(d[14]), "+f"(d[15]),
          "+f"(d[16]), "+f"(d[17]), "+f"(d[18]), "+f"(d[19]), "+f"(d[20]), "+f"(d[21]), "+f"(d[22]), "+f"(d[23]),
          "+f"(d[24]), "+f"(d[25]), "+f"(d[26]), "+f"(d[27]), "+f"(d[28]), "+f"(d[29]), "+f"(d[30]), "+f"(d[31])
        : "l"(a), "l"(b), "r"(acc), "n"(TB));
  }
};
template <> struct Wgmma<128> {
  template <int TB>
  __device__ __forceinline__ static void ss(float (&d)[64], uint64_t a, uint64_t b, uint32_t acc) {
    asm volatile(
        "{\n.reg .pred p;\n"
        "setp.ne.b32 p, %66, 0;\n"
        "wgmma.mma_async.sync.aligned.m64n128k16.f32.bf16.bf16 "
        "{" 
        "%0, %1, %2, %3, %4, %5, %6, %7, %8, %9, %10, %11, %12, %13, %14, %15, "
        "%16, %17, %18, %19, %20, %21, %22, %23, %24, %25, %26, %27, %28, %29, %30, %31, "
        "%32, %33, %34, %35, %36, %37, %38, %39, %40, %41, %42, %43, %44, %45, %46, %47, "
        "%48, %49, %50, %51, %52, %53, %54, %55, %56, %57, %58, %59, %60, %61, %62, %63"
        "}, %64, %65, p, 1, 1, 0, %67;\n}\n"
        : "+f"(d[0]), "+f"(d[1]), "+f"(d[2]), "+f"(d[3]), "+f"(d[4]), "+f"(d[5]), "+f"(d[6]), "+f"(d[7]),
          "+f"(d[8]), "+f"(d[9]), "+f"(d[10]), "+f"(d[11]), "+f"(d[12]), "+f"(d[13]), "+f"(d[14]), "+f"(d[15]),
          "+f"(d[16]), "+f"(d[17]), "+f"(d[18]), "+f"(d[19]), "+f"(d[20]), "+f"(d[21]), "+f"(d[22]), "+f"(d[23]),
          "+f"(d[24]), "+f"(d[25]), "+f"(d[26]), "+f"(d[27]), "+f"(d[28]), "+f"(d[29]), "+f"(d[30]), "+f"(d[31]),
          "+f"(d[32]), "+f"(d[33]), "+f"(d[34]), "+f"(d[35]), "+f"(d[36]), "+f"(d[37]), "+f"(d[38]), "+f"(d[39]),
          "+f"(d[40]), "+f"(d[41]), "+f"(d[42]), "+f"(d[43]), "+f"(d[44]), "+f"(d[45]), "+f"(d[46]), "+f"(d[47]),
          "+f"(d[48]), "+f"(d[49]), "+f"(d[50]), "+f"(d[51]), "+f"(d[52]), "+f"(d[53]), "+f"(d[54]), "+f"(d[55]),
          "+f"(d[56]), "+f"(d[57]), "+f"(d[58]), "+f"(d[59]), "+f"(d[60]), "+f"(d[61]), "+f"(d[62]), "+f"(d[63])
        : "l"(a), "l"(b), "r"(acc), "n"(TB));
  }
};
template <> struct Wgmma<256> {
  template <int TB>
  __device__ __forceinline__ static void ss(float (&d)[128], uint64_t a, uint64_t b, uint32_t acc) {
    asm volatile(
        "{\n.reg .pred p;\n"
        "setp.ne.b32 p, %130, 0;\n"
        "wgmma.mma_async.sync.aligned.m64n256k16.f32.bf16.bf16 "
        "{" 
        "%0, %1, %2, %3, %4, %5, %6, %7, %8, %9, %10, %11, %12, %13, %14, %15, "
        "%16, %17, %18, %19, %20, %21, %22, %23, %24, %25, %26, %27, %28, %29, %30, %31, "
        "%32, %33, %34, %35, %36, %37, %38, %39, %40, %41, %42, %43, %44, %45, %46, %47, "
        "%48, %49, %50, %51, %52, %53, %54, %55, %56, %57, %58, %59, %60, %61, %62, %63, "
        "%64, %65, %66, %67, %68, %69, %70, %71, %72, %73, %74, %75, %76, %77, %78, %79, "
        "%80, %81, %82, %83, %84, %85, %86, %87, %88, %89, %90, %91, %92, %93, %94, %95, "
        "%96, %97, %98, %99, %100, %101, %102, %103, %104, %105, %106, %107, %108, %109, %110, %111, "
        "%112, %113, %114, %115, %116, %117, %118, %119, %120, %121, %122, %123, %124, %125, %126, %127"
        "}, %128, %129, p, 1, 1, 0, %131;\n}\n"
        : "+f"(d[0]), "+f"(d[1]), "+f"(d[2]), "+f"(d[3]), "+f"(d[4]), "+f"(d[5]), "+f"(d[6]), "+f"(d[7]),
          "+f"(d[8]), "+f"(d[9]), "+f"(d[10]), "+f"(d[11]), "+f"(d[12]), "+f"(d[13]), "+f"(d[14]), "+f"(d[15]),
          "+f"(d[16]), "+f"(d[17]), "+f"(d[18]), "+f"(d[19]), "+f"(d[20]), "+f"(d[21]), "+f"(d[22]), "+f"(d[23]),
          "+f"(d[24]), "+f"(d[25]), "+f"(d[26]), "+f"(d[27]), "+f"(d[28]), "+f"(d[29]), "+f"(d[30]), "+f"(d[31]),
          "+f"(d[32]), "+f"(d[33]), "+f"(d[34]), "+f"(d[35]), "+f"(d[36]), "+f"(d[37]), "+f"(d[38]), "+f"(d[39]),
          "+f"(d[40]), "+f"(d[41]), "+f"(d[42]), "+f"(d[43]), "+f"(d[44]), "+f"(d[45]), "+f"(d[46]), "+f"(d[47]),
          "+f"(d[48]), "+f"(d[49]), "+f"(d[50]), "+f"(d[51]), "+f"(d[52]), "+f"(d[53]), "+f"(d[54]), "+f"(d[55]),
          "+f"(d[56]), "+f"(d[57]), "+f"(d[58]), "+f"(d[59]), "+f"(d[60]), "+f"(d[61]), "+f"(d[62]), "+f"(d[63]),
          "+f"(d[64]), "+f"(d[65]), "+f"(d[66]), "+f"(d[67]), "+f"(d[68]), "+f"(d[69]), "+f"(d[70]), "+f"(d[71]),
          "+f"(d[72]), "+f"(d[73]), "+f"(d[74]), "+f"(d[75]), "+f"(d[76]), "+f"(d[77]), "+f"(d[78]), "+f"(d[79]),
          "+f"(d[80]), "+f"(d[81]), "+f"(d[82]), "+f"(d[83]), "+f"(d[84]), "+f"(d[85]), "+f"(d[86]), "+f"(d[87]),
          "+f"(d[88]), "+f"(d[89]), "+f"(d[90]), "+f"(d[91]), "+f"(d[92]), "+f"(d[93]), "+f"(d[94]), "+f"(d[95]),
          "+f"(d[96]), "+f"(d[97]), "+f"(d[98]), "+f"(d[99]), "+f"(d[100]), "+f"(d[101]), "+f"(d[102]), "+f"(d[103]),
          "+f"(d[104]), "+f"(d[105]), "+f"(d[106]), "+f"(d[107]), "+f"(d[108]), "+f"(d[109]), "+f"(d[110]), "+f"(d[111]),
          "+f"(d[112]), "+f"(d[113]), "+f"(d[114]), "+f"(d[115]), "+f"(d[116]), "+f"(d[117]), "+f"(d[118]), "+f"(d[119]),
          "+f"(d[120]), "+f"(d[121]), "+f"(d[122]), "+f"(d[123]), "+f"(d[124]), "+f"(d[125]), "+f"(d[126]), "+f"(d[127])
        : "l"(a), "l"(b), "r"(acc), "n"(TB));
  }
};

template <int N>
struct WgmmaRsF16;
template <> struct WgmmaRsF16<16> {
  __device__ __forceinline__ static void rs(float (&d)[8], const uint32_t (&a)[4], uint64_t b) {
    asm volatile(
        "{\n.reg .pred p;\n"
        "setp.ne.b32 p, 1, 0;\n"
        "wgmma.mma_async.sync.aligned.m64n16k16.f32.f16.f16 "
        "{%0, %1, %2, %3, %4, %5, %6, %7}, {%8, %9, %10, %11}, %12, p, 1, 1, 1;\n}\n"
        : "+f"(d[0]), "+f"(d[1]), "+f"(d[2]), "+f"(d[3]), "+f"(d[4]), "+f"(d[5]), "+f"(d[6]), "+f"(d[7])
        : "r"(a[0]), "r"(a[1]), "r"(a[2]), "r"(a[3]), "l"(b));
  }
};
template <> struct WgmmaRsF16<64> {
  __device__ __forceinline__ static void rs(float (&d)[32], const uint32_t (&a)[4], uint64_t b) {
    asm volatile(
        "{\n.reg .pred p;\n"
        "setp.ne.b32 p, 1, 0;\n"
        "wgmma.mma_async.sync.aligned.m64n64k16.f32.f16.f16 "
        "{"
        "%0, %1, %2, %3, %4, %5, %6, %7, %8, %9, %10, %11, %12, %13, %14, %15, "
        "%16, %17, %18, %19, %20, %21, %22, %23, %24, %25, %26, %27, %28, %29, %30, %31"
        "}, {%32, %33, %34, %35}, %36, p, 1, 1, 1;\n}\n"
        : "+f"(d[0]), "+f"(d[1]), "+f"(d[2]), "+f"(d[3]), "+f"(d[4]), "+f"(d[5]), "+f"(d[6]), "+f"(d[7]),
          "+f"(d[8]), "+f"(d[9]), "+f"(d[10]), "+f"(d[11]), "+f"(d[12]), "+f"(d[13]), "+f"(d[14]), "+f"(d[15]),
          "+f"(d[16]), "+f"(d[17]), "+f"(d[18]), "+f"(d[19]), "+f"(d[20]), "+f"(d[21]), "+f"(d[22]), "+f"(d[23]),
          "+f"(d[24]), "+f"(d[25]), "+f"(d[26]), "+f"(d[27]), "+f"(d[28]), "+f"(d[29]), "+f"(d[30]), "+f"(d[31])
        : "r"(a[0]), "r"(a[1]), "r"(a[2]), "r"(a[3]), "l"(b));
  }
};

__device__ __forceinline__ uint32_t acc_row(uint32_t base, int ld, int row) {
  return base + static_cast<uint32_t>(row * ld) * 4u;
}
__device__ __forceinline__ void acc_ld32(uint32_t addr, uint32_t (&r)[32]) {
#pragma unroll
  for (int i = 0; i < 8; ++i)
    asm volatile("ld.shared.v4.b32 {%0, %1, %2, %3}, [%4];"
                 : "=r"(r[4 * i]), "=r"(r[4 * i + 1]), "=r"(r[4 * i + 2]), "=r"(r[4 * i + 3])
                 : "r"(addr + 16 * i));
}
__device__ __forceinline__ void acc_st32(uint32_t addr, const uint32_t (&r)[32]) {
#pragma unroll
  for (int i = 0; i < 8; ++i)
    asm volatile("st.shared.v4.b32 [%0], {%1, %2, %3, %4};" ::"r"(addr + 16 * i), "r"(r[4 * i]), "r"(r[4 * i + 1]),
                 "r"(r[4 * i + 2]), "r"(r[4 * i + 3])
                 : "memory");
}
template <int BN>
__device__ __forceinline__ void acc_store(const float (&d)[BN / 2], uint32_t base, int ld, int wg, int t) {
  const int row = wg * 64 + (t >> 5) * 16 + ((t & 31) >> 2);
  const int col = 2 * (t & 3);
  const uint32_t a0 = acc_row(base, ld, row) + col * 4, a1 = acc_row(base, ld, row + 8) + col * 4;
#pragma unroll
  for (int j = 0; j < BN / 8; ++j) {
    asm volatile("st.shared.v2.f32 [%0], {%1, %2};" ::"r"(a0 + 32 * j), "f"(d[4 * j]), "f"(d[4 * j + 1]) : "memory");
    asm volatile("st.shared.v2.f32 [%0], {%1, %2};" ::"r"(a1 + 32 * j), "f"(d[4 * j + 2]), "f"(d[4 * j + 3]) : "memory");
  }
}
__device__ __forceinline__ void named_bar_sync(int id, int nthreads) {
  asm volatile("bar.sync %0, %1;" ::"r"(id), "r"(nthreads) : "memory");
}

template <int R>
__device__ __forceinline__ void setmaxnreg_inc() { asm volatile("setmaxnreg.inc.sync.aligned.u32 %0;" ::"n"(R)); }
template <int R>
__device__ __forceinline__ void setmaxnreg_dec() { asm volatile("setmaxnreg.dec.sync.aligned.u32 %0;" ::"n"(R)); }

template <int BN, bool B_MN, int STAGES>
__device__ __forceinline__ void wg_mainloop(float (&d)[BN / 2], uint32_t base, int stage_bytes, int a_bytes,
                                            int num_kb, int wg, int& stage, uint32_t& phase, uint64_t* bar_full,
                                            uint64_t* bar_empty) {
  constexpr bool IN_FLIGHT = STAGES > 1;
  const int lane = threadIdx.x & 31;
  int prev = 0;
#pragma unroll 1
  for (int kb = 0; kb < num_kb; ++kb) {
    mbar_wait(smem_u32(&bar_full[stage]), phase);
    const uint32_t sa = base + stage * stage_bytes + wg * 8192;
    const uint32_t sb = base + stage * stage_bytes + a_bytes;
    acc_fence(d);
    wgmma_fence();
#pragma unroll
    for (int k = 0; k < 4; ++k) {
      const uint64_t adesc = make_gdesc(sa + k * 32, 16, 1024);
      const uint64_t bdesc = B_MN ? make_gdesc(sb + k * 2048, 64 * 128, 1024) : make_gdesc(sb + k * 32, 16, 1024);
      Wgmma<BN>::template ss<B_MN ? 1 : 0>(d, adesc, bdesc, (kb | k) != 0);
    }
    wgmma_commit();
    if constexpr (IN_FLIGHT) {
      wgmma_wait<1>();
      acc_fence(d);
      if (kb > 0) {
        __syncwarp();
        if (lane == 0) mbar_arrive(smem_u32(&bar_empty[prev]));
      }
    } else {
      wgmma_wait<0>();
      acc_fence(d);
      __syncwarp();
      if (lane == 0) mbar_arrive(smem_u32(&bar_empty[stage]));
    }
    prev = stage;
    if (++stage == STAGES) { stage = 0; phase ^= 1; }
  }
  if constexpr (IN_FLIGHT) {
    wgmma_wait<0>();
    acc_fence(d);
    __syncwarp();
    if (lane == 0 && num_kb > 0) mbar_arrive(smem_u32(&bar_empty[prev]));
  }
}

__device__ __forceinline__ uint32_t pack_bf16x2(float lo, float hi) {
  __nv_bfloat162 v = __floats2bfloat162_rn(lo, hi);
  return *reinterpret_cast<uint32_t*>(&v);
}
__device__ __forceinline__ float gelu_erf(float x) {
  return 0.5f * x * (1.0f + erff(x * 0.70710678118654752440f));
}

__device__ __forceinline__ float gelu_fast(float x) {
  const float x2 = x * x;
  float p = fmaf(3.229002131292087e-06f, x2, -8.823835998556129e-05f);
  p = fmaf(p, x2, -0.0003602734064506858f);
  p = fmaf(p, x2, 0.10522668605353103f);
  p = fmaf(p, x2, 2.302045390974673f);
  float e;
  asm("ex2.approx.ftz.f32 %0, %1;" : "=f"(e) : "f"(-p * x));
  return __fdividef(x, 1.0f + e);
}

}
```

### rsprompter_b200/sam_decoder.py

```python
from __future__ import annotations

import math

import torch
from torch import nn

from . import _lib
from .registry import MODELS, BaseModule
from .sam_config import SamDecoderArch, decoder_arch, vision_arch
from .sam_encoder import _Affine, _load_pretrained


class _Embedding(nn.Module):
    def __init__(self, n: int, c: int):
        super().__init__()
        self.weight = nn.Parameter(torch.empty(n, c), requires_grad=False)


class _SamAttention(nn.Module):
    def __init__(self, C: int, internal: int):
        super().__init__()
        self.q_proj = _Affine((internal, C))
        self.k_proj = _Affine((internal, C))
        self.v_proj = _Affine((internal, C))
        self.out_proj = _Affine((C, internal))


class _Mlp(nn.Module):
    def __init__(self, C: int, M: int):
        super().__init__()
        self.lin1 = _Affine((M, C))
        self.lin2 = _Affine((C, M))


class _TwoWayBlock(nn.Module):
    def __init__(self, a: SamDecoderArch):
        super().__init__()
        C = a.hidden_size
        self.self_attn = _SamAttention(C, C)
        self.layer_norm1 = _Affine((C,))
        self.cross_attn_token_to_image = _SamAttention(C, C // a.attention_downsample_rate)
        self.layer_norm2 = _Affine((C,))
        self.mlp = _Mlp(C, a.mlp_dim)
        self.layer_norm3 = _Affine((C,))
        self.layer_norm4 = _Affine((C,))
        self.cross_attn_image_to_token = _SamAttention(C, C // a.attention_downsample_rate)


class _TwoWayTransformer(nn.Module):
    def __init__(self, a: SamDecoderArch):
        super().__init__()
        self.layers = nn.ModuleList(_TwoWayBlock(a) for _ in range(a.num_layers))
        self.final_attn_token_to_image = _SamAttention(a.hidden_size, a.hidden_size // a.attention_downsample_rate)
        self.layer_norm_final_attn = _Affine((a.hidden_size,))


class _FeedForward(nn.Module):
    def __init__(self, cin: int, hidden: int, cout: int, num_layers: int):
        super().__init__()
        self.proj_in = _Affine((hidden, cin))
        self.proj_out = _Affine((cout, hidden))
        self.layers = nn.ModuleList(_Affine((hidden, hidden)) for _ in range(num_layers - 2))


class _ConvT(nn.Module):
    def __init__(self, cin: int, cout: int):
        super().__init__()
        self.weight = nn.Parameter(torch.empty(cin, cout, 2, 2), requires_grad=False)
        self.bias = nn.Parameter(torch.empty(cout), requires_grad=False)


class SamMaskDecoderB200(nn.Module):

    def __init__(self, arch: SamDecoderArch | None = None):
        super().__init__()
        a = self.arch = arch or SamDecoderArch()
        C = a.hidden_size
        self.num_mask_tokens = a.num_multimask_outputs + 1
        self.iou_token = _Embedding(1, C)
        self.mask_tokens = _Embedding(self.num_mask_tokens, C)
        self.transformer = _TwoWayTransformer(a)
        self.upscale_conv1 = _ConvT(C, C // 4)
        self.upscale_conv2 = _ConvT(C // 4, C // 8)
        self.upscale_layer_norm = _Affine((C // 4,))
        self.output_hypernetworks_mlps = nn.ModuleList(
            _FeedForward(C, C, C // 8, 3) for _ in range(self.num_mask_tokens))
        self.iou_prediction_head = _FeedForward(C, a.iou_head_hidden_dim, self.num_mask_tokens, a.iou_head_depth)
        self._prep: dict | None = None
        self.register_load_state_dict_post_hook(lambda *_: setattr(self, "_prep", None))

    def _apply(self, fn, *a, **k):
        self._prep = None
        return super()._apply(fn, *a, **k)

    @torch.no_grad()
    def _prepare(self) -> dict:
        if self.iou_token.weight.device.type != "cuda":
            raise _lib.RspError("SamMaskDecoderB200 runs on CUDA only")
        bf = lambda t: t.detach().to(torch.bfloat16).contiguous()
        f32 = lambda t: t.detach().to(torch.float32).contiguous()

        def attn(m: _SamAttention) -> dict:
            return dict(qw=bf(m.q_proj.weight), qb=f32(m.q_proj.bias), kw=bf(m.k_proj.weight),
                        kb=f32(m.k_proj.bias), vw=bf(m.v_proj.weight), vb=f32(m.v_proj.bias),
                        ow=bf(m.out_proj.weight), ob=f32(m.out_proj.bias),
                        kvw=bf(torch.cat([m.k_proj.weight, m.v_proj.weight], dim=0)),
                        kvb=f32(torch.cat([m.k_proj.bias, m.v_proj.bias], dim=0)))

        def ln(m: _Affine) -> tuple:
            return (f32(m.weight), f32(m.bias))

        def ff(m: _FeedForward) -> list:
            mods = [m.proj_in, *m.layers, m.proj_out]
            return [(bf(x.weight), f32(x.bias)) for x in mods]

        p: dict = {"layers": []}
        for blk in self.transformer.layers:
            p["layers"].append(dict(
                sa=attn(blk.self_attn), t2i=attn(blk.cross_attn_token_to_image),
                i2t=attn(blk.cross_attn_image_to_token),
                w1=bf(blk.mlp.lin1.weight), b1=f32(blk.mlp.lin1.bias),
                w2=bf(blk.mlp.lin2.weight), b2=f32(blk.mlp.lin2.bias),
                ln1=ln(blk.layer_norm1), ln2=ln(blk.layer_norm2), ln3=ln(blk.layer_norm3),
                ln4=ln(blk.layer_norm4)))
        p["final"] = attn(self.transformer.final_attn_token_to_image)
        p["lnf"] = ln(self.transformer.layer_norm_final_attn)
        c4, c8 = self.upscale_conv1.weight.shape[1], self.upscale_conv2.weight.shape[1]
        p["up1_w"] = bf(self.upscale_conv1.weight.permute(2, 3, 1, 0).reshape(4 * c4, -1))
        p["up1_b"] = f32(self.upscale_conv1.bias.repeat(4))
        p["up_ln"] = ln(self.upscale_layer_norm)
        p["up2_w"] = bf(self.upscale_conv2.weight.permute(2, 3, 1, 0).reshape(4 * c8, -1))
        p["up2_b"] = f32(self.upscale_conv2.bias.repeat(4))
        p["hyper"] = [ff(m) for m in self.output_hypernetworks_mlps]
        p["iou"] = ff(self.iou_prediction_head)
        p["out_tokens"] = f32(torch.cat([self.iou_token.weight, self.mask_tokens.weight], dim=0))
        p["pos_terms"] = {}
        self._prep = p
        return p

    def _pos_terms(self, p: dict, pos_rows: torch.Tensor) -> dict:
        key = (pos_rows.data_ptr(), pos_rows.shape[0])
        if key not in p["pos_terms"]:
            pb = _lib.cast_bf16(pos_rows)
            layers = [L["t2i"] for L in p["layers"]] + [p["final"]]
            kv = []
            for a in layers:
                t = torch.zeros(pos_rows.shape[0], a["kvw"].shape[0], device=pos_rows.device, dtype=torch.bfloat16)
                n_k = a["kw"].shape[0]
                t[:, :n_k] = _lib.gemm(pb, a["kw"])
                kv.append(t)
            q = [_lib.gemm(pb, L["i2t"]["qw"]) for L in p["layers"]]
            p["pos_terms"] = {key: dict(kv=kv, q=q)}
        return p["pos_terms"][key]

    @staticmethod
    def _ff(x_bf: torch.Tensor, layers: list) -> torch.Tensor:
        h = x_bf
        for w, b in layers[:-1]:
            h = _lib.gemm(h, w, b, act="relu")
        w, b = layers[-1]
        return _lib.gemm(h, w, b, out_dtype=torch.float32)

    @torch.no_grad()
    def decode(self, emb_rows: torch.Tensor, pos_rows: torch.Tensor, sparse: torch.Tensor,
               hw: tuple[int, int], prompt_img: torch.Tensor | None = None,
               dense_vec: torch.Tensor | None = None, dense_rows: torch.Tensor | None = None,
               multimask_output: bool = False, src_pair: tuple | None = None):
        p = self._prep or self._prepare()
        a = self.arch
        C, H = a.hidden_size, a.num_heads
        h, w = hw
        HW = h * w
        N, P, _ = sparse.shape
        Tt = 1 + self.num_mask_tokens + P
        dev = sparse.device
        assert pos_rows.shape == (HW, C) and (emb_rows is None or emb_rows.shape[1] == C)
        shared = prompt_img is not None and dense_rows is None
        pos_rows = pos_rows.contiguous()
        if src_pair is not None:
            src_b = src_pair[0]
            src32, blk = src_b, None
        elif dense_rows is not None:
            if prompt_img is not None:
                emb_rows = emb_rows.view(-1, HW, C)[prompt_img.long()].reshape(N * HW, C)
            src32 = emb_rows + dense_rows
            blk = None
        else:
            src32 = emb_rows if dense_vec is None else emb_rows + dense_vec.view(1, C)
            blk = prompt_img if shared else None
        if src_pair is None:
            src32 = src32.contiguous()
            src_b = _lib.cast_bf16(src32)
        pt = self._pos_terms(p, pos_rows)
        tokens = torch.cat([p["out_tokens"].unsqueeze(0).expand(N, -1, -1), sparse.to(torch.float32)], dim=1)
        tokens = tokens.reshape(N * Tt, C).contiguous()

        def t2i(layer: dict, queries: torch.Tensor, keys_b: torch.Tensor, pos_kv: torch.Tensor, kv_blk, ln):
            qin = _lib.add_cast_bf16(queries, tokens)
            q = _lib.gemm(qin, layer["qw"], layer["qb"])
            KV = _lib.gemm(keys_b, layer["kvw"], layer["kvb"], residual=pos_kv, res_mod=HW)
            n_k = layer["kw"].shape[0]
            att = _lib.t2i_attention(q.view(N, Tt, -1), KV[:, :n_k], KV[:, n_k:], HW, kv_block=kv_blk)
            return _lib.gemm(att.view(N * Tt, -1), layer["ow"], layer["ob"], residual=queries,
                             out_dtype=torch.float32, ln=ln)

        keys_b, keys_res, kblk = src_b, src_b, blk
        queries = None
        for li, L in enumerate(p["layers"]):
            sa = L["sa"]
            if li == 0:
                tb = _lib.cast_bf16(tokens)
                q = _lib.gemm(tb, sa["qw"], sa["qb"])
                k = _lib.gemm(tb, sa["kw"], sa["kb"])
                v = _lib.gemm(tb, sa["vw"], sa["vb"])
                att = _lib.token_self_attention(q.view(N, Tt, C), k.view(N, Tt, C), v.view(N, Tt, C), H)
                queries = _lib.gemm(att.view(N * Tt, C), sa["ow"], sa["ob"], out_dtype=torch.float32,
                                    ln=(*L["ln1"], a.layer_norm_eps))
            else:
                qin = _lib.add_cast_bf16(queries, tokens)
                q = _lib.gemm(qin, sa["qw"], sa["qb"])
                k = _lib.gemm(qin, sa["kw"], sa["kb"])
                v = _lib.gemm(_lib.cast_bf16(queries), sa["vw"], sa["vb"])
                att = _lib.token_self_attention(q.view(N, Tt, C), k.view(N, Tt, C), v.view(N, Tt, C), H)
                queries = _lib.gemm(att.view(N * Tt, C), sa["ow"], sa["ob"], residual=queries,
                                    out_dtype=torch.float32, ln=(*L["ln1"], a.layer_norm_eps))
            queries = t2i(L["t2i"], queries, keys_b, pt["kv"][li], kblk, (*L["ln2"], a.layer_norm_eps))
            hdn = _lib.gemm(_lib.cast_bf16(queries), L["w1"], L["b1"], act="relu")
            queries = _lib.gemm(hdn, L["w2"], L["b2"], residual=queries, out_dtype=torch.float32,
                                ln=(*L["ln3"], a.layer_norm_eps))
            i2t = L["i2t"]
            qin = _lib.add_cast_bf16(queries, tokens)
            ktok = _lib.gemm(qin, i2t["kw"], i2t["kb"])
            vtok = _lib.gemm(_lib.cast_bf16(queries), i2t["vw"], i2t["vb"])
            Qimg = _lib.gemm(keys_b, i2t["qw"], i2t["qb"], residual=pt["q"][li], res_mod=HW)
            att = _lib.i2t_attention(Qimg, ktok.view(N, Tt, -1), vtok.view(N, Tt, -1), HW, q_block=kblk)
            keys_b = _lib.gemm(att, i2t["ow"], i2t["ob"], residual=keys_res, ln=(*L["ln4"], a.layer_norm_eps),
                               res_block_map=kblk, res_block_rows=HW if kblk is not None else 0)
            keys_res, kblk = keys_b, None
        queries = t2i(p["final"], queries, keys_b, pt["kv"][-1], None, (*p["lnf"], 1e-5))
        qv = queries.view(N, Tt, C)
        iou_tok = _lib.cast_bf16(qv[:, 0].contiguous())
        iou = self._ff(iou_tok, p["iou"])
        up1 = _lib.gemm(keys_b, p["up1_w"], p["up1_b"], ln64_gelu=(*p["up_ln"], 1e-6))
        up1 = up1.view(N * HW * 4, -1)
        sel = range(1, self.num_mask_tokens) if multimask_output else range(0, 1)
        masks = []
        for i in sel:
            mt = _lib.cast_bf16(qv[:, 1 + i].contiguous())
            hyper = self._ff(mt, p["hyper"][i])
            masks.append(_lib.gemm_upscale_mask(up1, p["up2_w"], p["up2_b"], hyper, h, w))
        masks = torch.stack(masks, dim=1) if len(masks) > 1 else masks[0].unsqueeze(1)
        iou = iou[:, 1:] if multimask_output else iou[:, 0:1]
        return masks, iou

    def forward(self, image_embeddings, image_positional_embeddings, sparse_prompt_embeddings,
                dense_prompt_embeddings, multimask_output, attention_similarity=None,
                target_embedding=None, output_attentions=None):
        if attention_similarity is not None or target_embedding is not None:
            raise NotImplementedError("attention_similarity / target_embedding are not used by RSPrompter")
        N, C, h, w = image_embeddings.shape
        assert sparse_prompt_embeddings.shape[1] == 1, "point_batch_size must be 1"
        to_rows = lambda t: t.to(torch.float32).permute(0, 2, 3, 1).reshape(-1, C).contiguous()
        pos_rows = to_rows(image_positional_embeddings[:1])
        masks, iou = self.decode(to_rows(image_embeddings), pos_rows, sparse_prompt_embeddings[:, 0],
                                 (h, w), dense_rows=to_rows(dense_prompt_embeddings),
                                 multimask_output=multimask_output)
        return masks.unsqueeze(1), iou.unsqueeze(1), None


@MODELS.register_module(force=True)
class RSSamMaskDecoder(BaseModule):

    def __init__(self, hf_pretrain_name, extra_config=None, init_cfg=None):
        BaseModule.__init__(self, init_cfg=None)
        self.mask_decoder = SamMaskDecoderB200(decoder_arch(hf_pretrain_name, extra_config))
        _load_pretrained(self.mask_decoder, init_cfg, [(r"^module\.", ""), (r"^mask_decoder\.", "")])

    def init_weights(self):
        pass

    def forward(self, *args, **kwargs):
        return self.mask_decoder(*args, **kwargs)


class SamPositionalEmbeddingB200(nn.Module):

    def __init__(self, num_pos_feats: int = 128, scale: float = 1.0):
        super().__init__()
        self.scale = scale
        self.positional_embedding = nn.Parameter(scale * torch.randn(2, num_pos_feats), requires_grad=False)
        self._cache: dict = {}

    def forward(self, input_coords, input_shape=None):
        c = input_coords.clone()
        if input_shape is not None:
            c[..., 0] = c[..., 0] / input_shape[1]
            c[..., 1] = c[..., 1] / input_shape[0]
        c = (2 * c - 1).to(self.positional_embedding.dtype) @ self.positional_embedding
        c = 2 * math.pi * c
        return torch.cat([torch.sin(c), torch.cos(c)], dim=-1)

    def image_wide_rows(self, size: int) -> torch.Tensor:
        key = (size, self.positional_embedding.device, self.positional_embedding._version)
        if key not in self._cache:
            g = torch.ones(size, size, device=self.positional_embedding.device, dtype=torch.float32)
            y = (g.cumsum(0) - 0.5) / size
            x = (g.cumsum(1) - 0.5) / size
            self._cache = {key: self.forward(torch.stack([x, y], dim=-1)).reshape(size * size, -1).contiguous()}
        return self._cache[key]


@MODELS.register_module(force=True)
class RSSamPositionalEmbedding(BaseModule):

    def __init__(self, hf_pretrain_name, extra_config=None, init_cfg=None):
        BaseModule.__init__(self, init_cfg=None)
        va = vision_arch(hf_pretrain_name, extra_config)
        self.shared_image_embedding = SamPositionalEmbeddingB200(va.num_pos_feats, va.pe_scale())
        _load_pretrained(self.shared_image_embedding, init_cfg,
                         [(r"^module\.", ""), (r"^shared_image_embedding\.", "")])

    def init_weights(self):
        pass

    def forward(self, *args, **kwargs):
        return self.shared_image_embedding(*args, **kwargs)


class _MaskEmbed(nn.Module):

    def __init__(self, a: SamDecoderArch):
        super().__init__()
        mc = a.mask_input_channels
        self.conv1 = _Affine((mc // 4, 1, 2, 2))
        self.conv2 = _Affine((mc, mc // 4, 2, 2))
        self.conv3 = _Affine((a.hidden_size, mc, 1, 1))
        self.layer_norm1 = _Affine((mc // 4,))
        self.layer_norm2 = _Affine((mc,))


class SamPromptEncoderB200(nn.Module):

    def __init__(self, a: SamDecoderArch):
        super().__init__()
        self.no_mask_embed = _Embedding(1, a.hidden_size)
        self.mask_embed = _MaskEmbed(a)


@MODELS.register_module(force=True)
class RSSamPromptEncoder(BaseModule):

    def __init__(self, hf_pretrain_name, extra_config=None, init_cfg=None):
        BaseModule.__init__(self, init_cfg=None)
        self.prompt_encoder = SamPromptEncoderB200(decoder_arch(hf_pretrain_name, extra_config))
        _load_pretrained(self.prompt_encoder, init_cfg, [(r"^module\.", ""), (r"^prompt_encoder\.", "")])

    def init_weights(self):
        pass


__all__ = ["SamMaskDecoderB200", "RSSamMaskDecoder", "RSSamPositionalEmbedding", "RSSamPromptEncoder",
           "SamPositionalEmbeddingB200", "SamPromptEncoderB200"]
```

Measured before the change: 43.42.

## Fuse SAM decoder image-side projections with t2i and i2t attention

Adds two fused kernels. t2i_fused computes the k|v projection of image keys on the fly inside the token-to-image attention, so the large KV intermediate is never written to global memory. i2t_fused combines the image-side q projection, image-to-token attention, out_proj, residual add and LayerNorm in one TMA/wgmma kernel, removing the round trips of the Qimg and attention-output tensors. The old path remains for the first layer, where a block map is used, and for grids where HW is not a multiple of 64. A profiling script is also added. The trade-off is much more complex kernels with higher register and shared-memory pressure, which may lower occupancy.

```diff
diff --git a/include/rsp_b200.h b/include/rsp_b200.h
--- a/include/rsp_b200.h
+++ b/include/rsp_b200.h
@@ -64,6 +64,13 @@
                       int N, int Tq, int HW, void* stream);
 int rsp_i2t_attention(const void* Q, const int32_t* q_block, const void* ktok, const void* vtok,
                       void* out, int N, int Tq, int HW, void* stream);
+
+int rsp_t2i_fused(const void* keys, int ldk, const void* kvw, const float* kvb, const void* pe_kv, const void* q,
+                  void* out, int N, int Tq, int HW, void* stream);
+
+int rsp_i2t_fused(const void* keys, int ldk, const void* wq, const float* qb, const void* pe_q, const void* ktok,
+                  const void* vtok, const void* wo, const float* ob, const float* ln_g, const float* ln_b, float eps,
+                  void* out, int N, int Tq, int HW, void* stream);
 
 
 int rsp_rpn_decode(const float* head_out, int ld, const int64_t* topk_idx, int K, int B, int H, int W,
diff --git a/profiles/decoder_bench.py b/profiles/decoder_bench.py
--- /dev/null
+++ b/profiles/decoder_bench.py
@@ -0,0 +1,214 @@
+#!/usr/bin/env python
+from __future__ import annotations
+
+import argparse
+import collections
+import json
+import os
+import subprocess
+import sys
+
+ROOT = os.path.dirname(os.path.dirname(os.path.abspath(__file__)))
+if ROOT not in sys.path:
+    sys.path.insert(0, ROOT)
+
+import torch
+
+from rsprompter_b200 import _lib, synthetic
+from rsprompter_b200.sam_config import SamDecoderArch
+from rsprompter_b200.sam_decoder import SamMaskDecoderB200
+
+NQ = 100
+
+
+def _card() -> dict:
+    q = subprocess.run(["nvidia-smi", "--query-gpu=name,power.limit,clocks.max.sm", "--format=csv,noheader"],
+                       capture_output=True, text=True)
+    name, power, clk = (s.strip() for s in q.stdout.strip().splitlines()[0].split(","))
+    return dict(name=name, power_limit=power, max_sm_clock=clk)
+
+
+def setup(n: int, side: int, points: int, seed: int = 0):
+    arch = SamDecoderArch()
+    dec = SamMaskDecoderB200(arch)
+    dec.load_state_dict(synthetic.mask_decoder_state_dict(arch, seed=seed + 1))
+    dec = dec.cuda()
+    pe = synthetic.prompt_encoder_state_dict(arch, seed=seed + 2)
+    C = arch.hidden_size
+    me = [pe[k].float().contiguous().cuda() for k in (
+        "mask_embed.conv1.weight", "mask_embed.conv1.bias", "mask_embed.layer_norm1.weight",
+        "mask_embed.layer_norm1.bias", "mask_embed.conv2.weight", "mask_embed.conv2.bias",
+        "mask_embed.layer_norm2.weight", "mask_embed.layer_norm2.bias")]
+    me += [pe["mask_embed.conv3.weight"].reshape(C, -1).float().contiguous().cuda(),
+           pe["mask_embed.conv3.bias"].float().contiguous().cuda()]
+    g = torch.Generator().manual_seed(seed)
+    B = max(1, n // NQ)
+    hw = side * side
+    emb_rows = (0.5 * torch.randn(B * hw, C, generator=g)).cuda()
+    pos_rows = torch.randn(hw, C, generator=g).cuda()
+    mpp = (2.0 * torch.randn(n, 4 * side, 4 * side, generator=g)).cuda()
+    sparse = (0.5 * torch.randn(n, points, C, generator=g)).cuda()
+    src_pair = _lib.mask_embed_src(mpp, me, emb_rows, pos_rows, min(NQ, n), (side, side))
+    return dec, pos_rows, sparse, src_pair
+
+
+def _nb(t) -> int:
+    return 0 if t is None else t.numel() * t.element_size()
+
+
+def _gemm_cost(a, w, *args, **kw):
+    M, K = a.shape
+    N = w.shape[0]
+    out_b = 4 if kw.get("out_dtype", torch.bfloat16) == torch.float32 else 2
+    res = kw.get("residual")
+    byts = M * K * 2 + _nb(w) + M * N * out_b + (_nb(res) if res is not None and res.shape[0] <= M else 0)
+    if res is not None and res.shape[0] > M:
+        byts += M * N * res.element_size()
+    return 2.0 * M * N * K, byts
+
+
+def _upscale_cost(a, w, bias, hyper, gh, gw, *args, **kw):
+    M, K = a.shape
+    P = M // (4 * gh * gw)
+    return 2.0 * M * 128 * K, M * K * 2 + P * 16 * gh * gw * 4
+
+
+def _t2i_cost(q, K, V, hw, kv_block=None):
+    N, Tq, C = q.shape
+    rows = K.shape[0]
+    return 4.0 * N * Tq * hw * C, 2 * rows * C * 2 + 2 * _nb(q)
+
+
+def _i2t_cost(Q, ktok, vtok, hw, q_block=None):
+    N, Tq, C = ktok.shape
+    return 4.0 * N * Tq * hw * C, Q.shape[0] * C * 2 + N * hw * C * 2
+
+
+def _t2i_fused_cost(q, keys, kvw, kvb, pe_kv, hw):
+    N, Tq, C = q.shape
+    return 2.0 * keys.shape[0] * 256 * 256 + 4.0 * N * Tq * hw * C, keys.shape[0] * 256 * 2 + 2 * _nb(q)
+
+
+def _i2t_fused_cost(keys, wq, qb, pe_q, ktok, vtok, wo, ob, ln, hw):
+    N, Tq, C = ktok.shape
+    R = keys.shape[0]
+    return 2.0 * R * 256 * 128 * 2 + 4.0 * N * Tq * hw * C, R * 256 * 2 * 2
+
+
+def _family(name: str, args, kw, n_img_rows: int) -> str:
+    if name == "gemm":
+        a, w = args[0], args[1]
+        if a.shape[0] < n_img_rows:
+            return "token-side gemm"
+        if kw.get("ln64_gelu") is not None:
+            return "up1 gemm (LN64 + GELU)"
+        if kw.get("ln") is not None:
+            return "i2t out_proj gemm (+ LN4)"
+        if w.shape[0] == 256:
+            return "t2i k|v gemm"
+        return "i2t q gemm"
+    return {"gemm_upscale_mask": "up2 gemm (GELU + hyper)", "t2i_attention": "t2i attention",
+            "i2t_attention": "i2t attention", "t2i_fused": "t2i fused (k|v gemm + attention)",
+            "i2t_fused": "i2t fused (q gemm + attention + out_proj + LN4)"}.get(name, "token-side " + name)
+
+
+COSTS = {"gemm": _gemm_cost, "gemm_upscale_mask": _upscale_cost, "t2i_attention": _t2i_cost,
+         "i2t_attention": _i2t_cost, "t2i_fused": _t2i_fused_cost, "i2t_fused": _i2t_fused_cost}
+WRAPPED = ("gemm", "gemm_upscale_mask", "t2i_attention", "i2t_attention", "t2i_fused", "i2t_fused", "add_cast_bf16",
+           "cast_bf16", "token_self_attention")
+
+
+def per_family(run, n_img_rows: int, iters: int) -> dict:
+    calls = []
+    orig = {k: getattr(_lib, k) for k in WRAPPED if hasattr(_lib, k)}
+
+    def wrap(name, fn):
+        def inner(*args, **kw):
+            s, e = torch.cuda.Event(enable_timing=True), torch.cuda.Event(enable_timing=True)
+            s.record()
+            out = fn(*args, **kw)
+            e.record()
+            cost = COSTS[name](*args, **kw) if name in COSTS else (0.0, 0)
+            calls.append((_family(name, args, kw, n_img_rows), s, e, cost))
+            return out
+        return inner
+
+    try:
+        for k, fn in orig.items():
+            setattr(_lib, k, wrap(k, fn))
+        for _ in range(iters):
+            run()
+        torch.cuda.synchronize()
+    finally:
+        for k, fn in orig.items():
+            setattr(_lib, k, fn)
+    fam = collections.defaultdict(lambda: [0.0, 0.0, 0, 0])
+    for f, s, e, (fl, by) in calls:
+        r = fam[f]
+        r[0] += s.elapsed_time(e) / iters
+        r[1] += fl / iters
+        r[2] += by // iters
+        r[3] += 1
+    out = {}
+    for f, (ms, fl, by, cnt) in sorted(fam.items(), key=lambda kv: -kv[1][0]):
+        out[f] = dict(ms=round(ms, 3), calls=cnt // iters, GB=round(by / 1e9, 3),
+                      GB_s=round(by / (ms * 1e-3) / 1e9, 1) if ms > 0 and by else None,
+                      TFLOP_s=round(fl / (ms * 1e-3) / 1e12, 1) if ms > 0 and fl else None)
+    return out
+
+
+def main():
+    ap = argparse.ArgumentParser()
+    ap.add_argument("--n", type=int, default=800, help="prompts (C3: 8 images x 100 queries)")
+    ap.add_argument("--hw", type=int, default=64, help="side of the image-token grid")
+    ap.add_argument("--points", type=int, default=5, help="sparse points per prompt (Tt = 5 + points)")
+    ap.add_argument("--iters", type=int, default=20)
+    ap.add_argument("--warmup", type=int, default=3)
+    ap.add_argument("--multimask", action="store_true")
+    ap.add_argument("--trace-dir", default=None, help="also write the profiler's kernel table here")
+    args = ap.parse_args()
+    if not torch.cuda.is_available():
+        raise SystemExit("decoder_bench needs a GPU")
+    torch.cuda.set_device(0)
+    dec, pos_rows, sparse, src_pair = setup(args.n, args.hw, args.points)
+    hw = (args.hw, args.hw)
+
+    def run():
+        return dec.decode(None, pos_rows, sparse, hw, src_pair=src_pair, multimask_output=args.multimask)
+
+    for _ in range(args.warmup):
+        run()
+    torch.cuda.synchronize()
+    s, e = torch.cuda.Event(enable_timing=True), torch.cuda.Event(enable_timing=True)
+    s.record()
+    for _ in range(args.iters):
+        run()
+    e.record()
+    torch.cuda.synchronize()
+    decode_ms = s.elapsed_time(e) / args.iters
+    fams = per_family(run, args.n * args.hw * args.hw, args.iters)
+    from torch.profiler import ProfilerActivity, profile
+    n_prof = max(3, args.iters // 4)
+    with profile(activities=[ProfilerActivity.CUDA]) as prof:
+        for _ in range(n_prof):
+            run()
+        torch.cuda.synchronize()
+    kern = collections.defaultdict(lambda: [0.0, 0])
+    for ev in prof.events():
+        if ev.device_type == torch.autograd.DeviceType.CUDA:
+            kern[ev.name][0] += ev.device_time_total / 1e3 / n_prof
+            kern[ev.name][1] += 1
+    kernels = {k[:120]: dict(ms=round(v[0], 3), launches=v[1] // n_prof)
+               for k, v in sorted(kern.items(), key=lambda kv: -kv[1][0])}
+    if args.trace_dir:
+        os.makedirs(args.trace_dir, exist_ok=True)
+        with open(os.path.join(args.trace_dir, "decoder_kernels.txt"), "w") as f:
+            f.write(prof.key_averages().table(sort_by="cuda_time_total", row_limit=60))
+    res = dict(card=_card(), n=args.n, hw=args.hw * args.hw, tt=5 + args.points, multimask=args.multimask,
+               decode_ms=round(decode_ms, 3), kernel_ms=round(sum(v["ms"] for v in kernels.values()), 3),
+               families=fams, kernels=kernels)
+    print(json.dumps(res))
+
+
+if __name__ == "__main__":
+    main()
diff --git a/rsprompter_b200/_lib.py b/rsprompter_b200/_lib.py
--- a/rsprompter_b200/_lib.py
+++ b/rsprompter_b200/_lib.py
@@ -59,6 +59,8 @@
     "rsp_token_self_attention": ([_vp, _vp, _vp, _vp, _i, _i, _i, _i, _vp], _i),
     "rsp_t2i_attention": ([_vp, _vp, _vp, _i, _vp, _vp, _i, _i, _i, _vp], _i),
     "rsp_i2t_attention": ([_vp, _vp, _vp, _vp, _vp, _i, _i, _i, _vp], _i),
+    "rsp_t2i_fused": ([_vp, _i, _vp, _vp, _vp, _vp, _vp, _i, _i, _i, _vp], _i),
+    "rsp_i2t_fused": ([_vp, _i, _vp, _vp, _vp, _vp, _vp, _vp, _vp, _vp, _vp, _f, _vp, _i, _i, _i, _vp], _i),
     "rsp_rpn_decode": ([_vp, _i, _vp, _i, _i, _i, _i, _i, _i, _vp, _vp, _f, _f, _f, _i, _i, _vp, _vp, _vp], _i),
     "rsp_bbox_cls_decode": ([_vp, _i, _vp, _i, _vp, _vp, _i, _i, _vp, _f, _f, _f, _vp, _vp, _vp, _vp], _i),
     "rsp_rpn_decode_shapes": ([_vp, _i, _vp, _i, _i, _i, _i, _i, _i, _vp, _vp, _vp, _f, _i, _i, _vp, _vp, _vp], _i),
@@ -318,6 +320,45 @@
     return out
 
 
+def t2i_fused(q: torch.Tensor, keys: torch.Tensor, kvw: torch.Tensor, kvb: torch.Tensor, pe_kv: torch.Tensor,
+              hw: int) -> torch.Tensor:
+    global launch_count
+    _require_cuda(q, keys, kvw, kvb, pe_kv)
+    N, Tq, C = q.shape
+    assert C == 128 and q.dtype == torch.bfloat16 and q.is_contiguous()
+    assert keys.dtype == torch.bfloat16 and keys.dim() == 2 and keys.stride(1) == 1 and keys.shape == (N * hw, 256)
+    assert kvw.dtype == torch.bfloat16 and kvw.shape == (256, 256) and kvw.is_contiguous()
+    assert kvb.dtype == torch.float32 and kvb.numel() == 256 and kvb.is_contiguous()
+    assert pe_kv.dtype == torch.bfloat16 and pe_kv.shape == (hw, 256) and pe_kv.is_contiguous()
+    out = torch.empty_like(q)
+    _check(_lib.rsp_t2i_fused(_ptr(keys), keys.stride(0), _ptr(kvw), _ptr(kvb), _ptr(pe_kv), _ptr(q), _ptr(out), N, Tq,
+                              hw, _stream()), "rsp_t2i_fused")
+    launch_count += 1
+    _log("gemm", 2.0 * N * hw * 256 * 256)
+    return out
+
+
+def i2t_fused(keys: torch.Tensor, wq: torch.Tensor, qb: torch.Tensor, pe_q: torch.Tensor, ktok: torch.Tensor,
+              vtok: torch.Tensor, wo: torch.Tensor, ob: torch.Tensor, ln: tuple, hw: int) -> torch.Tensor:
+    global launch_count
+    g, b, eps = ln
+    _require_cuda(keys, wq, qb, pe_q, ktok, vtok, wo, ob, g, b)
+    N, Tq, C = ktok.shape
+    assert C == 128 and hw % 64 == 0
+    assert keys.dtype == torch.bfloat16 and keys.dim() == 2 and keys.stride(1) == 1 and keys.shape == (N * hw, 256)
+    for t, shape in ((wq, (128, 256)), (pe_q, (hw, 128)), (ktok, (N, Tq, 128)), (vtok, (N, Tq, 128)), (wo, (256, 128))):
+        assert t.dtype == torch.bfloat16 and t.shape == shape and t.is_contiguous()
+    for t, n in ((qb, 128), (ob, 256), (g, 256), (b, 256)):
+        assert t.dtype == torch.float32 and t.numel() == n and t.is_contiguous()
+    out = torch.empty((N * hw, 256), device=keys.device, dtype=torch.bfloat16)
+    _check(_lib.rsp_i2t_fused(_ptr(keys), keys.stride(0), _ptr(wq), _ptr(qb), _ptr(pe_q), _ptr(ktok), _ptr(vtok),
+                              _ptr(wo), _ptr(ob), _ptr(g), _ptr(b), float(eps), _ptr(out), N, Tq, hw, _stream()),
+           "rsp_i2t_fused")
+    launch_count += 1
+    _log("gemm", 2.0 * N * hw * 256 * 256)
+    return out
+
+
 def i2t_attention(Q: torch.Tensor, ktok: torch.Tensor, vtok: torch.Tensor, hw: int,
                   q_block: torch.Tensor | None = None) -> torch.Tensor:
     global launch_count
diff --git a/rsprompter_b200/csrc/abi.cu b/rsprompter_b200/csrc/abi.cu
--- a/rsprompter_b200/csrc/abi.cu
+++ b/rsprompter_b200/csrc/abi.cu
@@ -173,6 +173,17 @@
   return i2t_attention(Q, q_block, ktok, vtok, out, N, Tq, HW, S(stream));
 }
 
+int rsp_t2i_fused(const void* keys, int ldk, const void* kvw, const float* kvb, const void* pe_kv, const void* q,
+                  void* out, int N, int Tq, int HW, void* stream) {
+  return t2i_fused(keys, ldk, kvw, kvb, pe_kv, q, out, N, Tq, HW, S(stream));
+}
+
+int rsp_i2t_fused(const void* keys, int ldk, const void* wq, const float* qb, const void* pe_q, const void* ktok,
+                  const void* vtok, const void* wo, const float* ob, const float* ln_g, const float* ln_b, float eps,
+                  void* out, int N, int Tq, int HW, void* stream) {
+  return i2t_fused(keys, ldk, wq, qb, pe_q, ktok, vtok, wo, ob, ln_g, ln_b, eps, out, N, Tq, HW, S(stream));
+}
+
 }
 
 #include "detect.h"
diff --git a/rsprompter_b200/csrc/decoder.cu b/rsprompter_b200/csrc/decoder.cu
--- a/rsprompter_b200/csrc/decoder.cu
+++ b/rsprompter_b200/csrc/decoder.cu
@@ -132,6 +132,108 @@
   asm volatile("cp.async.cg.shared.global [%0], [%1], 16;" ::"r"(dst), "l"(src) : "memory");
 }
 
+struct T2iHead {
+  uint32_t qa[4];
+  float m0, m1, l0, l1;
+  float o[2][4];
+};
+
+__device__ __forceinline__ void t2i_head_init(T2iHead& st, const __nv_bfloat16* __restrict__ q, int n, int Tq, int h,
+                                              float scale) {
+  const int lane = threadIdx.x & 31, g = lane >> 2, t = lane & 3;
+  auto ldq = [&](int row, int col) -> uint32_t {
+    if (row >= Tq) return 0u;
+    const __nv_bfloat162 v = *reinterpret_cast<const __nv_bfloat162*>(
+        q + (static_cast<size_t>(n) * Tq + row) * 128 + h * 16 + col);
+    return pack_bf16x2(__bfloat162float(v.x) * scale, __bfloat162float(v.y) * scale);
+  };
+  st.qa[0] = ldq(g, 2 * t); st.qa[1] = ldq(g + 8, 2 * t); st.qa[2] = ldq(g, 2 * t + 8); st.qa[3] = ldq(g + 8, 2 * t + 8);
+  st.m0 = -INFINITY; st.m1 = -INFINITY; st.l0 = 0.f; st.l1 = 0.f;
+#pragma unroll
+  for (int d = 0; d < 2; ++d) st.o[d][0] = st.o[d][1] = st.o[d][2] = st.o[d][3] = 0.f;
+}
+
+__device__ __forceinline__ void t2i_head_tile(T2iHead& st, uint32_t sK, uint32_t sV, int valid) {
+  const int lane = threadIdx.x & 31, g = lane >> 2, t = lane & 3;
+  float& m0 = st.m0; float& m1 = st.m1; float& l0 = st.l0; float& l1 = st.l1;
+  float (&o)[2][4] = st.o;
+  const uint32_t (&qa)[4] = st.qa;
+  float s[8][4];
+#pragma unroll
+  for (int j = 0; j < 8; ++j) {
+    uint32_t b0, b1;
+    const uint32_t addr = sK + (j * 8 + g) * T2I_ROWB + t * 4;
+    asm volatile("ld.shared.b32 %0, [%1];" : "=r"(b0) : "r"(addr));
+    asm volatile("ld.shared.b32 %0, [%1];" : "=r"(b1) : "r"(addr + 16));
+    s[j][0] = s[j][1] = s[j][2] = s[j][3] = 0.f;
+    mma_bf16_16816(s[j], qa, b0, b1);
+    if (valid < T2I_TILE) {
+      const int key = j * 8 + 2 * t;
+      if (key >= valid) { s[j][0] = -INFINITY; s[j][2] = -INFINITY; }
+      if (key + 1 >= valid) { s[j][1] = -INFINITY; s[j][3] = -INFINITY; }
+    }
+  }
+  float mx0 = -INFINITY, mx1 = -INFINITY;
+#pragma unroll
+  for (int j = 0; j < 8; ++j) {
+    mx0 = fmaxf(mx0, fmaxf(s[j][0], s[j][1]));
+    mx1 = fmaxf(mx1, fmaxf(s[j][2], s[j][3]));
+  }
+  mx0 = fmaxf(mx0, __shfl_xor_sync(0xffffffffu, mx0, 1)); mx0 = fmaxf(mx0, __shfl_xor_sync(0xffffffffu, mx0, 2));
+  mx1 = fmaxf(mx1, __shfl_xor_sync(0xffffffffu, mx1, 1)); mx1 = fmaxf(mx1, __shfl_xor_sync(0xffffffffu, mx1, 2));
+  const float mn0 = fmaxf(m0, mx0), mn1 = fmaxf(m1, mx1);
+  const float a0 = __expf(m0 - mn0), a1 = __expf(m1 - mn1);
+  m0 = mn0; m1 = mn1;
+  float ps0 = 0.f, ps1 = 0.f;
+#pragma unroll
+  for (int j = 0; j < 8; ++j) {
+    s[j][0] = __expf(s[j][0] - mn0); s[j][1] = __expf(s[j][1] - mn0);
+    s[j][2] = __expf(s[j][2] - mn1); s[j][3] = __expf(s[j][3] - mn1);
+    ps0 += s[j][0] + s[j][1];
+    ps1 += s[j][2] + s[j][3];
+  }
+  l0 = l0 * a0 + ps0; l1 = l1 * a1 + ps1;
+#pragma unroll
+  for (int d = 0; d < 2; ++d) { o[d][0] *= a0; o[d][1] *= a0; o[d][2] *= a1; o[d][3] *= a1; }
+#pragma unroll
+  for (int c = 0; c < 4; ++c) {
+    uint32_t pa[4];
+    pa[0] = pack_bf16x2(s[2 * c][0], s[2 * c][1]);
+    pa[1] = pack_bf16x2(s[2 * c][2], s[2 * c][3]);
+    pa[2] = pack_bf16x2(s[2 * c + 1][0], s[2 * c + 1][1]);
+    pa[3] = pack_bf16x2(s[2 * c + 1][2], s[2 * c + 1][3]);
+#pragma unroll
+    for (int d = 0; d < 2; ++d) {
+      const uint32_t addr = sV + (c * 16 + 2 * t) * T2I_ROWB + (d * 8 + g) * 2;
+      uint16_t v00, v01, v10, v11;
+      asm volatile("ld.shared.u16 %0, [%1];" : "=h"(v00) : "r"(addr));
+      asm volatile("ld.shared.u16 %0, [%1];" : "=h"(v01) : "r"(addr + T2I_ROWB));
+      asm volatile("ld.shared.u16 %0, [%1];" : "=h"(v10) : "r"(addr + 8 * T2I_ROWB));
+      asm volatile("ld.shared.u16 %0, [%1];" : "=h"(v11) : "r"(addr + 9 * T2I_ROWB));
+      const uint32_t b0 = static_cast<uint32_t>(v00) | (static_cast<uint32_t>(v01) << 16);
+      const uint32_t b1 = static_cast<uint32_t>(v10) | (static_cast<uint32_t>(v11) << 16);
+      mma_bf16_16816(o[d], pa, b0, b1);
+    }
+  }
+}
+
+__device__ __forceinline__ void t2i_head_store(T2iHead& st, __nv_bfloat16* __restrict__ out, int n, int Tq, int h) {
+  const int lane = threadIdx.x & 31, g = lane >> 2, t = lane & 3;
+  float l0 = st.l0, l1 = st.l1;
+  l0 += __shfl_xor_sync(0xffffffffu, l0, 1); l0 += __shfl_xor_sync(0xffffffffu, l0, 2);
+  l1 += __shfl_xor_sync(0xffffffffu, l1, 1); l1 += __shfl_xor_sync(0xffffffffu, l1, 2);
+  const float i0 = 1.0f / l0, i1 = 1.0f / l1;
+#pragma unroll
+  for (int d = 0; d < 2; ++d) {
+    if (g < Tq)
+      *reinterpret_cast<uint32_t*>(out + (static_cast<size_t>(n) * Tq + g) * 128 + h * 16 + d * 8 + 2 * t) =
+          pack_bf16x2(st.o[d][0] * i0, st.o[d][1] * i0);
+    if (g + 8 < Tq)
+      *reinterpret_cast<uint32_t*>(out + (static_cast<size_t>(n) * Tq + g + 8) * 128 + h * 16 + d * 8 + 2 * t) =
+          pack_bf16x2(st.o[d][2] * i1, st.o[d][3] * i1);
+  }
+}
+
 __global__ void __launch_bounds__(256)
 t2i_attention_kernel(const __nv_bfloat16* __restrict__ q,
                      const __nv_bfloat16* __restrict__ K,
@@ -145,8 +247,7 @@
   const int blk = kv_block ? kv_block[n] : n;
   const __nv_bfloat16* Kb = K + static_cast<size_t>(blk) * HW * ldkv;
   const __nv_bfloat16* Vb = V + static_cast<size_t>(blk) * HW * ldkv;
-  const int tid = threadIdx.x, lane = tid & 31, h = tid >> 5;
-  const int g = lane >> 2, t = lane & 3;
+  const int tid = threadIdx.x, h = tid >> 5;
   const int n_tiles = (HW + T2I_TILE - 1) / T2I_TILE;
 
   auto issue_tile = [&](int tile, int stage) {
@@ -163,19 +264,8 @@
     asm volatile("cp.async.commit_group;" ::: "memory");
   };
 
-  uint32_t qa[4];
-  {
-    auto ldq = [&](int row, int col) -> uint32_t {
-      if (row >= Tq) return 0u;
-      const __nv_bfloat162 v = *reinterpret_cast<const __nv_bfloat162*>(
-          q + (static_cast<size_t>(n) * Tq + row) * 128 + h * 16 + col);
-      return pack_bf16x2(__bfloat162float(v.x) * scale, __bfloat162float(v.y) * scale);
-    };
-    qa[0] = ldq(g, 2 * t); qa[1] = ldq(g + 8, 2 * t); qa[2] = ldq(g, 2 * t + 8); qa[3] = ldq(g + 8, 2 * t + 8);
-  }
-  float m0 = -INFINITY, m1 = -INFINITY, l0 = 0.f, l1 = 0.f;
-  float o[2][4] = {{0.f, 0.f, 0.f, 0.f}, {0.f, 0.f, 0.f, 0.f}};
-
+  T2iHead st;
+  t2i_head_init(st, q, n, Tq, h, scale);
   issue_tile(0, 0);
   for (int tile = 0; tile < n_tiles; ++tile) {
     const int stage = tile & 1;
@@ -187,79 +277,10 @@
     }
     __syncthreads();
     const uint32_t sK = s_base + stage * T2I_STAGE + h * 32;
-    const uint32_t sV = sK + T2I_TILE * T2I_ROWB;
-    const int valid = min(T2I_TILE, HW - tile * T2I_TILE);
-    float s[8][4];
-#pragma unroll
-    for (int j = 0; j < 8; ++j) {
-      uint32_t b0, b1;
-      const uint32_t addr = sK + (j * 8 + g) * T2I_ROWB + t * 4;
-      asm volatile("ld.shared.b32 %0, [%1];" : "=r"(b0) : "r"(addr));
-      asm volatile("ld.shared.b32 %0, [%1];" : "=r"(b1) : "r"(addr + 16));
-      s[j][0] = s[j][1] = s[j][2] = s[j][3] = 0.f;
-      mma_bf16_16816(s[j], qa, b0, b1);
-      if (valid < T2I_TILE) {
-        const int key = j * 8 + 2 * t;
-        if (key >= valid) { s[j][0] = -INFINITY; s[j][2] = -INFINITY; }
-        if (key + 1 >= valid) { s[j][1] = -INFINITY; s[j][3] = -INFINITY; }
-      }
-    }
-    float mx0 = -INFINITY, mx1 = -INFINITY;
-#pragma unroll
-    for (int j = 0; j < 8; ++j) {
-      mx0 = fmaxf(mx0, fmaxf(s[j][0], s[j][1]));
-      mx1 = fmaxf(mx1, fmaxf(s[j][2], s[j][3]));
-    }
-    mx0 = fmaxf(mx0, __shfl_xor_sync(0xffffffffu, mx0, 1)); mx0 = fmaxf(mx0, __shfl_xor_sync(0xffffffffu, mx0, 2));
-    mx1 = fmaxf(mx1, __shfl_xor_sync(0xffffffffu, mx1, 1)); mx1 = fmaxf(mx1, __shfl_xor_sync(0xffffffffu, mx1, 2));
-    const float mn0 = fmaxf(m0, mx0), mn1 = fmaxf(m1, mx1);
-    const float a0 = __expf(m0 - mn0), a1 = __expf(m1 - mn1);
-    m0 = mn0; m1 = mn1;
-    float ps0 = 0.f, ps1 = 0.f;
-#pragma unroll
-    for (int j = 0; j < 8; ++j) {
-      s[j][0] = __expf(s[j][0] - mn0); s[j][1] = __expf(s[j][1] - mn0);
-      s[j][2] = __expf(s[j][2] - mn1); s[j][3] = __expf(s[j][3] - mn1);
-      ps0 += s[j][0] + s[j][1];
-      ps1 += s[j][2] + s[j][3];
-    }
-    l0 = l0 * a0 + ps0; l1 = l1 * a1 + ps1;
-#pragma unroll
-    for (int d = 0; d < 2; ++d) { o[d][0] *= a0; o[d][1] *= a0; o[d][2] *= a1; o[d][3] *= a1; }
-#pragma unroll
-    for (int c = 0; c < 4; ++c) {
-      uint32_t pa[4];
-      pa[0] = pack_bf16x2(s[2 * c][0], s[2 * c][1]);
-      pa[1] = pack_bf16x2(s[2 * c][2], s[2 * c][3]);
-      pa[2] = pack_bf16x2(s[2 * c + 1][0], s[2 * c + 1][1]);
-      pa[3] = pack_bf16x2(s[2 * c + 1][2], s[2 * c + 1][3]);
-#pragma unroll
-      for (int d = 0; d < 2; ++d) {
-        const uint32_t addr = sV + (c * 16 + 2 * t) * T2I_ROWB + (d * 8 + g) * 2;
-        uint16_t v00, v01, v10, v11;
-        asm volatile("ld.shared.u16 %0, [%1];" : "=h"(v00) : "r"(addr));
-        asm volatile("ld.shared.u16 %0, [%1];" : "=h"(v01) : "r"(addr + T2I_ROWB));
-        asm volatile("ld.shared.u16 %0, [%1];" : "=h"(v10) : "r"(addr + 8 * T2I_ROWB));
-        asm volatile("ld.shared.u16 %0, [%1];" : "=h"(v11) : "r"(addr + 9 * T2I_ROWB));
-        const uint32_t b0 = static_cast<uint32_t>(v00) | (static_cast<uint32_t>(v01) << 16);
-        const uint32_t b1 = static_cast<uint32_t>(v10) | (static_cast<uint32_t>(v11) << 16);
-        mma_bf16_16816(o[d], pa, b0, b1);
-      }
-    }
+    t2i_head_tile(st, sK, sK + T2I_TILE * T2I_ROWB, min(T2I_TILE, HW - tile * T2I_TILE));
     __syncthreads();
   }
-  l0 += __shfl_xor_sync(0xffffffffu, l0, 1); l0 += __shfl_xor_sync(0xffffffffu, l0, 2);
-  l1 += __shfl_xor_sync(0xffffffffu, l1, 1); l1 += __shfl_xor_sync(0xffffffffu, l1, 2);
-  const float i0 = 1.0f / l0, i1 = 1.0f / l1;
-#pragma unroll
-  for (int d = 0; d < 2; ++d) {
-    if (g < Tq)
-      *reinterpret_cast<uint32_t*>(out + (static_cast<size_t>(n) * Tq + g) * 128 + h * 16 + d * 8 + 2 * t) =
-          pack_bf16x2(o[d][0] * i0, o[d][1] * i0);
-    if (g + 8 < Tq)
-      *reinterpret_cast<uint32_t*>(out + (static_cast<size_t>(n) * Tq + g + 8) * 128 + h * 16 + d * 8 + 2 * t) =
-          pack_bf16x2(o[d][2] * i1, o[d][3] * i1);
-  }
+  t2i_head_store(st, out, n, Tq, h);
 }
 
 int t2i_attention(const void* q, const void* K, const void* V, int ldkv, const int* kv_block, void* out, int N,
@@ -281,8 +302,195 @@
   return RSP_OK;
 }
 
+constexpr int TF_THREADS = 256;
+constexpr int TF_W_BYTES = 4 * 256 * 128;
+constexpr int TF_A_BYTES = 4 * T2I_TILE * 128;
+constexpr int TF_STAGES = 2;
+constexpr int TF_BAR_OFF = TF_W_BYTES + TF_STAGES * TF_A_BYTES + T2I_STAGE;
+constexpr int TF_SMEM = TF_BAR_OFF + 64;
+static_assert(TF_SMEM <= 227 * 1024, "t2i_fused shared memory");
+
+__global__ void __launch_bounds__(TF_THREADS, 1)
+t2i_fused_kernel(const __grid_constant__ CUtensorMap tma_keys,
+                 const __grid_constant__ CUtensorMap tma_w,
+                 const float* __restrict__ kvb,
+                 const __nv_bfloat16* __restrict__ pe_kv,
+                 const __nv_bfloat16* __restrict__ q,
+                 __nv_bfloat16* __restrict__ out,
+                 int Tq, int HW, float scale) {
+  extern __shared__ __align__(1024) uint8_t smem[];
+  const uint32_t s_w = smem_u32(smem);
+  const uint32_t s_a = s_w + TF_W_BYTES;
+  const uint32_t s_kv = s_a + TF_STAGES * TF_A_BYTES;
+  uint64_t* bars = reinterpret_cast<uint64_t*>(smem + TF_BAR_OFF);
+  const uint32_t bar_w = smem_u32(&bars[0]);
+  auto bar_full = [&](int s) { return smem_u32(&bars[1 + s]); };
+  const int n = blockIdx.x;
+  const int warp = threadIdx.x >> 5, lane = threadIdx.x & 31;
+  const int n_tiles = (HW + T2I_TILE - 1) / T2I_TILE;
+  auto load_tile = [&](int tile) {
+    const uint32_t full = bar_full(tile % TF_STAGES);
+    mbar_expect_tx(full, TF_A_BYTES);
+    for (int kb = 0; kb < 4; ++kb)
+      tma_load_2d(s_a + (tile % TF_STAGES) * TF_A_BYTES + kb * (T2I_TILE * 128), &tma_keys, full, kb * 64,
+                  n * HW + tile * T2I_TILE);
+  };
+
+  if (threadIdx.x == 0) {
+    tma_prefetch_desc(&tma_keys);
+    tma_prefetch_desc(&tma_w);
+    mbar_init(bar_w, 1);
+    for (int s = 0; s < TF_STAGES; ++s) mbar_init(bar_full(s), 1);
+    fence_barrier_init();
+  }
+  __syncthreads();
+  if (threadIdx.x == 0) {
+    mbar_expect_tx(bar_w, TF_W_BYTES);
+    for (int kb = 0; kb < 4; ++kb) tma_load_2d(s_w + kb * (256 * 128), &tma_w, bar_w, kb * 64, 0);
+    for (int tile = 0; tile < TF_STAGES && tile < n_tiles; ++tile) load_tile(tile);
+  }
+
+  const int wg = warp >> 2;
+  const int h = warp;
+  const int tw = threadIdx.x & 127;
+  const int g = lane >> 2, t = lane & 3;
+  const int frow = (tw >> 5) * 16 + g;
+  T2iHead st;
+  t2i_head_init(st, q, n, Tq, h, scale);
+  const uint32_t sK = s_kv + h * 32, sV = sK + T2I_TILE * T2I_ROWB;
+  const uint32_t s_dst = s_kv + wg * (T2I_TILE * T2I_ROWB) + frow * T2I_ROWB + t * 4;
+  const float* bias = kvb + wg * 128 + 2 * t;
+  const __nv_bfloat16* pe = pe_kv + wg * 128 + 2 * t;
+  const uint32_t sb = s_w + wg * (128 * 128);
+  mbar_wait(bar_w, 0);
+  float acc[64];
+#pragma unroll 1
+  for (int tile = 0; tile < n_tiles; ++tile) {
+    const int stage = tile % TF_STAGES;
+    mbar_wait(bar_full(stage), (tile / TF_STAGES) & 1);
+    const uint32_t sa = s_a + stage * TF_A_BYTES;
+    acc_fence(acc);
+    wgmma_fence();
+#pragma unroll
+    for (int kb = 0; kb < 4; ++kb) {
+#pragma unroll
+      for (int k = 0; k < 4; ++k)
+        Wgmma<128>::ss<0>(acc, make_gdesc(sa + kb * (T2I_TILE * 128) + k * 32, 16, 1024),
+                          make_gdesc(sb + kb * (256 * 128) + k * 32, 16, 1024), (kb | k) != 0);
+    }
+    wgmma_commit();
+    uint32_t r[2][16];
+    {
+      const int r0 = min(tile * T2I_TILE + frow, HW - 1), r1 = min(tile * T2I_TILE + frow + 8, HW - 1);
+#pragma unroll
+      for (int j = 0; j < 16; ++j) {
+        r[0][j] = __ldg(reinterpret_cast<const unsigned int*>(pe + static_cast<size_t>(r0) * 256 + 8 * j));
+        r[1][j] = __ldg(reinterpret_cast<const unsigned int*>(pe + static_cast<size_t>(r1) * 256 + 8 * j));
+      }
+    }
+    if (tile > 0) t2i_head_tile(st, sK, sV, T2I_TILE);
+    wgmma_wait<0>();
+    acc_fence(acc);
+    named_bar_sync(1, 256);
+    if (threadIdx.x == 0 && tile + TF_STAGES < n_tiles) load_tile(tile + TF_STAGES);
+#pragma unroll
+    for (int j = 0; j < 16; ++j) {
+      const float2 b = __ldg(reinterpret_cast<const float2*>(bias + 8 * j));
+      const float v0 = (acc[4 * j] + b.x) + __uint_as_float(r[0][j] << 16);
+      const float v1 = (acc[4 * j + 1] + b.y) + __uint_as_float(r[0][j] & 0xffff0000u);
+      const float v2 = (acc[4 * j + 2] + b.x) + __uint_as_float(r[1][j] << 16);
+      const float v3 = (acc[4 * j + 3] + b.y) + __uint_as_float(r[1][j] & 0xffff0000u);
+      asm volatile("st.shared.b32 [%0], %1;" ::"r"(s_dst + 16 * j), "r"(pack_bf16x2(v0, v1)) : "memory");
+      asm volatile("st.shared.b32 [%0], %1;" ::"r"(s_dst + 8 * T2I_ROWB + 16 * j), "r"(pack_bf16x2(v2, v3))
+                   : "memory");
+    }
+    named_bar_sync(1, 256);
+  }
+  t2i_head_tile(st, sK, sV, HW - (n_tiles - 1) * T2I_TILE);
+  t2i_head_store(st, out, n, Tq, h);
+}
+
+int t2i_fused(const void* keys, int ldk, const void* kvw, const float* kvb, const void* pe_kv, const void* q,
+              void* out, int N, int Tq, int HW, cudaStream_t stream) {
+  RSP_CHECK_ARG(keys && kvw && kvb && pe_kv && q && out, "t2i_fused: null pointer");
+  RSP_CHECK_ARG(N > 0 && Tq > 0 && Tq <= 16 && HW > 0 && static_cast<long long>(N) * HW < (1ll << 31),
+                "t2i_fused: N %d, Tq %d, HW %d (Tq <= 16, N * HW < 2^31)", N, Tq, HW);
+  RSP_CHECK_ARG(ldk >= 256 && ldk % 8 == 0 && (reinterpret_cast<uintptr_t>(keys) & 15) == 0 &&
+                (reinterpret_cast<uintptr_t>(kvw) & 15) == 0, "t2i_fused: keys / Wkv row stride or alignment");
+  RSP_CHECK_ARG((reinterpret_cast<uintptr_t>(kvb) & 7) == 0 && (reinterpret_cast<uintptr_t>(pe_kv) & 3) == 0 &&
+                (reinterpret_cast<uintptr_t>(q) & 3) == 0 && (reinterpret_cast<uintptr_t>(out) & 3) == 0,
+                "t2i_fused: bias / positional term / q / out alignment");
+  CUtensorMap ta, tw;
+  RSP_TRY(make_tmap_bf16_2d(&ta, keys, static_cast<uint64_t>(N) * HW, 256, static_cast<uint64_t>(ldk) * 2,
+                            T2I_TILE, 64));
+  RSP_TRY(make_tmap_bf16_2d(&tw, kvw, 256, 256, 256 * 2, 256, 64));
+  static bool attr_set_dev[kMaxDevices] = {};
+  bool& attr_set = attr_set_dev[current_device()];
+  if (!attr_set) {
+    RSP_CHECK_CUDA(cudaFuncSetAttribute(t2i_fused_kernel, cudaFuncAttributeMaxDynamicSharedMemorySize, TF_SMEM));
+    attr_set = true;
+  }
+  t2i_fused_kernel<<<N, TF_THREADS, TF_SMEM, stream>>>(
+      ta, tw, kvb, static_cast<const __nv_bfloat16*>(pe_kv), static_cast<const __nv_bfloat16*>(q),
+      static_cast<__nv_bfloat16*>(out), Tq, HW, 0.25f);
+  RSP_CHECK_LAUNCH();
+  return RSP_OK;
+}
+
 constexpr int I2T_PIX = 128;
 constexpr int I2T_ROWB = 272;
+
+__device__ __forceinline__ void i2t_token_frags(const __nv_bfloat16* kp, const __nv_bfloat16* vp, int Tq, float scale,
+                                                uint32_t (&kb)[2][2], uint32_t (&vb)[2][2]) {
+  const int lane = threadIdx.x & 31, g = lane >> 2, t = lane & 3;
+#pragma unroll
+  for (int j = 0; j < 2; ++j) {
+    const int tok = j * 8 + g;
+    kb[j][0] = kb[j][1] = 0u;
+    if (tok < Tq) {
+      const __nv_bfloat162 k0 = *reinterpret_cast<const __nv_bfloat162*>(kp + tok * 128 + 2 * t);
+      const __nv_bfloat162 k1 = *reinterpret_cast<const __nv_bfloat162*>(kp + tok * 128 + 2 * t + 8);
+      kb[j][0] = pack_bf16x2(__bfloat162float(k0.x) * scale, __bfloat162float(k0.y) * scale);
+      kb[j][1] = pack_bf16x2(__bfloat162float(k1.x) * scale, __bfloat162float(k1.y) * scale);
+    }
+    auto ldv = [&](int tok2) -> uint32_t {
+      return tok2 < Tq ? static_cast<uint32_t>(*reinterpret_cast<const uint16_t*>(vp + tok2 * 128 + j * 8 + g)) : 0u;
+    };
+    vb[j][0] = ldv(2 * t) | (ldv(2 * t + 1) << 16);
+    vb[j][1] = ldv(2 * t + 8) | (ldv(2 * t + 9) << 16);
+  }
+}
+
+__device__ __forceinline__ void i2t_chunk(const uint32_t (&qa)[4], const uint32_t (&kb)[2][2], const uint32_t (&vb)[2][2],
+                                          int Tq, uint32_t (&o)[4]) {
+  const int t = threadIdx.x & 3;
+  float s0[4] = {0.f, 0.f, 0.f, 0.f}, s1[4] = {0.f, 0.f, 0.f, 0.f};
+  mma_bf16_16816(s0, qa, kb[0][0], kb[0][1]);
+  mma_bf16_16816(s1, qa, kb[1][0], kb[1][1]);
+  if (2 * t >= Tq) { s0[0] = -INFINITY; s0[2] = -INFINITY; }
+  if (2 * t + 1 >= Tq) { s0[1] = -INFINITY; s0[3] = -INFINITY; }
+  if (8 + 2 * t >= Tq) { s1[0] = -INFINITY; s1[2] = -INFINITY; }
+  if (9 + 2 * t >= Tq) { s1[1] = -INFINITY; s1[3] = -INFINITY; }
+  float m0 = fmaxf(fmaxf(s0[0], s0[1]), fmaxf(s1[0], s1[1]));
+  float m1 = fmaxf(fmaxf(s0[2], s0[3]), fmaxf(s1[2], s1[3]));
+  m0 = fmaxf(m0, __shfl_xor_sync(0xffffffffu, m0, 1)); m0 = fmaxf(m0, __shfl_xor_sync(0xffffffffu, m0, 2));
+  m1 = fmaxf(m1, __shfl_xor_sync(0xffffffffu, m1, 1)); m1 = fmaxf(m1, __shfl_xor_sync(0xffffffffu, m1, 2));
+  s0[0] = __expf(s0[0] - m0); s0[1] = __expf(s0[1] - m0); s1[0] = __expf(s1[0] - m0); s1[1] = __expf(s1[1] - m0);
+  s0[2] = __expf(s0[2] - m1); s0[3] = __expf(s0[3] - m1); s1[2] = __expf(s1[2] - m1); s1[3] = __expf(s1[3] - m1);
+  float l0 = s0[0] + s0[1] + s1[0] + s1[1], l1 = s0[2] + s0[3] + s1[2] + s1[3];
+  l0 += __shfl_xor_sync(0xffffffffu, l0, 1); l0 += __shfl_xor_sync(0xffffffffu, l0, 2);
+  l1 += __shfl_xor_sync(0xffffffffu, l1, 1); l1 += __shfl_xor_sync(0xffffffffu, l1, 2);
+  uint32_t pa[4] = {pack_bf16x2(s0[0], s0[1]), pack_bf16x2(s0[2], s0[3]), pack_bf16x2(s1[0], s1[1]),
+                    pack_bf16x2(s1[2], s1[3])};
+  float o0[4] = {0.f, 0.f, 0.f, 0.f}, o1[4] = {0.f, 0.f, 0.f, 0.f};
+  mma_bf16_16816(o0, pa, vb[0][0], vb[0][1]);
+  mma_bf16_16816(o1, pa, vb[1][0], vb[1][1]);
+  const float i0 = 1.0f / l0, i1 = 1.0f / l1;
+  o[0] = pack_bf16x2(o0[0] * i0, o0[1] * i0);
+  o[1] = pack_bf16x2(o0[2] * i1, o0[3] * i1);
+  o[2] = pack_bf16x2(o1[0] * i0, o1[1] * i0);
+  o[3] = pack_bf16x2(o1[2] * i1, o1[3] * i1);
+}
 
 __global__ void __launch_bounds__(256)
 i2t_attention_kernel(const __nv_bfloat16* __restrict__ Q,
@@ -309,26 +517,8 @@
   }
   asm volatile("cp.async.commit_group;" ::: "memory");
   uint32_t kb[2][2], vb[2][2];
-  {
-    const __nv_bfloat16* kp = ktok + static_cast<size_t>(n) * Tq * 128 + h * 16;
-    const __nv_bfloat16* vp = vtok + static_cast<size_t>(n) * Tq * 128 + h * 16;
-#pragma unroll
-    for (int j = 0; j < 2; ++j) {
-      const int tok = j * 8 + g;
-      kb[j][0] = kb[j][1] = 0u;
-      if (tok < Tq) {
-        const __nv_bfloat162 k0 = *reinterpret_cast<const __nv_bfloat162*>(kp + tok * 128 + 2 * t);
-        const __nv_bfloat162 k1 = *reinterpret_cast<const __nv_bfloat162*>(kp + tok * 128 + 2 * t + 8);
-        kb[j][0] = pack_bf16x2(__bfloat162float(k0.x) * scale, __bfloat162float(k0.y) * scale);
-        kb[j][1] = pack_bf16x2(__bfloat162float(k1.x) * scale, __bfloat162float(k1.y) * scale);
-      }
-      auto ldv = [&](int tok2) -> uint32_t {
-        return tok2 < Tq ? static_cast<uint32_t>(*reinterpret_cast<const uint16_t*>(vp + tok2 * 128 + j * 8 + g)) : 0u;
-      };
-      vb[j][0] = ldv(2 * t) | (ldv(2 * t + 1) << 16);
-      vb[j][1] = ldv(2 * t + 8) | (ldv(2 * t + 9) << 16);
-    }
-  }
+  i2t_token_frags(ktok + static_cast<size_t>(n) * Tq * 128 + h * 16, vtok + static_cast<size_t>(n) * Tq * 128 + h * 16,
+                  Tq, scale, kb, vb);
   asm volatile("cp.async.wait_group 0;" ::: "memory");
   __syncthreads();
   const uint32_t sq = s_tile + h * 32;
@@ -340,33 +530,13 @@
     asm volatile("ld.shared.b32 %0, [%1];" : "=r"(qa[1]) : "r"(a0 + 8 * I2T_ROWB));
     asm volatile("ld.shared.b32 %0, [%1];" : "=r"(qa[2]) : "r"(a0 + 16));
     asm volatile("ld.shared.b32 %0, [%1];" : "=r"(qa[3]) : "r"(a0 + 8 * I2T_ROWB + 16));
-    float s0[4] = {0.f, 0.f, 0.f, 0.f}, s1[4] = {0.f, 0.f, 0.f, 0.f};
-    mma_bf16_16816(s0, qa, kb[0][0], kb[0][1]);
-    mma_bf16_16816(s1, qa, kb[1][0], kb[1][1]);
-    if (2 * t >= Tq) { s0[0] = -INFINITY; s0[2] = -INFINITY; }
-    if (2 * t + 1 >= Tq) { s0[1] = -INFINITY; s0[3] = -INFINITY; }
-    if (8 + 2 * t >= Tq) { s1[0] = -INFINITY; s1[2] = -INFINITY; }
-    if (9 + 2 * t >= Tq) { s1[1] = -INFINITY; s1[3] = -INFINITY; }
-    float m0 = fmaxf(fmaxf(s0[0], s0[1]), fmaxf(s1[0], s1[1]));
-    float m1 = fmaxf(fmaxf(s0[2], s0[3]), fmaxf(s1[2], s1[3]));
-    m0 = fmaxf(m0, __shfl_xor_sync(0xffffffffu, m0, 1)); m0 = fmaxf(m0, __shfl_xor_sync(0xffffffffu, m0, 2));
-    m1 = fmaxf(m1, __shfl_xor_sync(0xffffffffu, m1, 1)); m1 = fmaxf(m1, __shfl_xor_sync(0xffffffffu, m1, 2));
-    s0[0] = __expf(s0[0] - m0); s0[1] = __expf(s0[1] - m0); s1[0] = __expf(s1[0] - m0); s1[1] = __expf(s1[1] - m0);
-    s0[2] = __expf(s0[2] - m1); s0[3] = __expf(s0[3] - m1); s1[2] = __expf(s1[2] - m1); s1[3] = __expf(s1[3] - m1);
-    float l0 = s0[0] + s0[1] + s1[0] + s1[1], l1 = s0[2] + s0[3] + s1[2] + s1[3];
-    l0 += __shfl_xor_sync(0xffffffffu, l0, 1); l0 += __shfl_xor_sync(0xffffffffu, l0, 2);
-    l1 += __shfl_xor_sync(0xffffffffu, l1, 1); l1 += __shfl_xor_sync(0xffffffffu, l1, 2);
-    uint32_t pa[4] = {pack_bf16x2(s0[0], s0[1]), pack_bf16x2(s0[2], s0[3]), pack_bf16x2(s1[0], s1[1]),
-                      pack_bf16x2(s1[2], s1[3])};
-    float o0[4] = {0.f, 0.f, 0.f, 0.f}, o1[4] = {0.f, 0.f, 0.f, 0.f};
-    mma_bf16_16816(o0, pa, vb[0][0], vb[0][1]);
-    mma_bf16_16816(o1, pa, vb[1][0], vb[1][1]);
-    const float i0 = 1.0f / l0, i1 = 1.0f / l1;
+    uint32_t o[4];
+    i2t_chunk(qa, kb, vb, Tq, o);
     __syncwarp();
-    asm volatile("st.shared.b32 [%0], %1;" ::"r"(a0), "r"(pack_bf16x2(o0[0] * i0, o0[1] * i0)) : "memory");
-    asm volatile("st.shared.b32 [%0], %1;" ::"r"(a0 + 8 * I2T_ROWB), "r"(pack_bf16x2(o0[2] * i1, o0[3] * i1)) : "memory");
-    asm volatile("st.shared.b32 [%0], %1;" ::"r"(a0 + 16), "r"(pack_bf16x2(o1[0] * i0, o1[1] * i0)) : "memory");
-    asm volatile("st.shared.b32 [%0], %1;" ::"r"(a0 + 8 * I2T_ROWB + 16), "r"(pack_bf16x2(o1[2] * i1, o1[3] * i1)) : "memory");
+    asm volatile("st.shared.b32 [%0], %1;" ::"r"(a0), "r"(o[0]) : "memory");
+    asm volatile("st.shared.b32 [%0], %1;" ::"r"(a0 + 8 * I2T_ROWB), "r"(o[1]) : "memory");
+    asm volatile("st.shared.b32 [%0], %1;" ::"r"(a0 + 16), "r"(o[2]) : "memory");
+    asm volatile("st.shared.b32 [%0], %1;" ::"r"(a0 + 8 * I2T_ROWB + 16), "r"(o[3]) : "memory");
   }
   __syncthreads();
   __nv_bfloat16* Ob = out + (static_cast<size_t>(n) * HW + p0) * 128;
@@ -391,4 +561,250 @@
   return RSP_OK;
 }
 
-}
+constexpr int IF_THREADS = 256;
+constexpr int IF_TILE = 64;
+constexpr int IF_WQ_BYTES = 4 * 128 * 128;
+constexpr int IF_WO_BYTES = 2 * 256 * 128;
+constexpr int IF_A_BYTES = 4 * IF_TILE * 128;
+constexpr int IF_TOK_BYTES = 2 * 16 * 256;
+constexpr int IF_A_OFF = IF_WQ_BYTES + IF_WO_BYTES;
+constexpr int IF_TOK_OFF = IF_A_OFF + 2 * IF_A_BYTES;
+constexpr int IF_VEC_OFF = IF_TOK_OFF + 2 * IF_TOK_BYTES;
+constexpr int IF_BAR_OFF = IF_VEC_OFF + 3 * 256 * 4;
+constexpr int IF_SMEM = IF_BAR_OFF + 64;
+static_assert(IF_SMEM <= 227 * 1024, "i2t_fused shared memory");
+
+__device__ __forceinline__ float sel4(int c, float a0, float a1, float a2, float a3) {
+  const float lo = (c & 1) ? a1 : a0, hi = (c & 1) ? a3 : a2;
+  return (c & 2) ? hi : lo;
+}
+
+__global__ void __launch_bounds__(IF_THREADS, 1)
+i2t_fused_kernel(const __grid_constant__ CUtensorMap tma_keys,
+                 const __grid_constant__ CUtensorMap tma_out,
+                 const __grid_constant__ CUtensorMap tma_wq,
+                 const __grid_constant__ CUtensorMap tma_wo,
+                 const float* __restrict__ qb,
+                 const __nv_bfloat16* __restrict__ pe_q,
+                 const __nv_bfloat16* __restrict__ ktok,
+                 const __nv_bfloat16* __restrict__ vtok,
+                 const float* __restrict__ ob,
+                 const float* __restrict__ ln_g, const float* __restrict__ ln_b, float eps,
+                 int Tq, int HW, int num_tiles, float scale) {
+  extern __shared__ __align__(1024) uint8_t smem[];
+  const uint32_t s_wq = smem_u32(smem);
+  const uint32_t s_wo = s_wq + IF_WQ_BYTES;
+  const uint32_t s_a = s_wq + IF_A_OFF;
+  uint64_t* bars = reinterpret_cast<uint64_t*>(smem + IF_BAR_OFF);
+  const uint32_t bar_w = smem_u32(&bars[0]);
+  const int warp = threadIdx.x >> 5, lane = threadIdx.x & 31;
+  const int wg = warp >> 2;
+  const int tw = threadIdx.x & 127;
+  const uint32_t bar_full = smem_u32(&bars[1 + wg]);
+  const int stride = 2 * gridDim.x;
+  auto load_tile = [&](int tile) {
+    mbar_expect_tx(bar_full, IF_A_BYTES);
+    for (int kb = 0; kb < 4; ++kb)
+      tma_load_2d(s_a + wg * IF_A_BYTES + kb * (IF_TILE * 128), &tma_keys, bar_full, kb * 64, tile * IF_TILE);
+  };
+
+  float* vec = reinterpret_cast<float*>(smem + IF_VEC_OFF);
+  for (int i = threadIdx.x; i < 256; i += IF_THREADS) {
+    vec[i] = ob[i];
+    vec[256 + i] = ln_g[i];
+    vec[512 + i] = ln_b[i];
+  }
+  if (threadIdx.x == 0) {
+    tma_prefetch_desc(&tma_keys);
+    tma_prefetch_desc(&tma_out);
+    for (int b = 0; b < 3; ++b) mbar_init(smem_u32(&bars[b]), 1);
+    fence_barrier_init();
+  }
+  __syncthreads();
+  if (threadIdx.x == 0) {
+    mbar_expect_tx(bar_w, IF_WQ_BYTES + IF_WO_BYTES);
+    for (int kb = 0; kb < 4; ++kb) tma_load_2d(s_wq + kb * (128 * 128), &tma_wq, bar_w, kb * 64, 0);
+    for (int kb = 0; kb < 2; ++kb) tma_load_2d(s_wo + kb * (256 * 128), &tma_wo, bar_w, kb * 64, 0);
+  }
+  const int first = blockIdx.x + wg * gridDim.x;
+  if (tw == 0 && first < num_tiles) load_tile(first);
+  const int g = lane >> 2, t = lane & 3;
+  const int frow = (warp & 3) * 16 + g;
+  const uint32_t sa = s_a + wg * IF_A_BYTES;
+  uint8_t* tok = smem + IF_TOK_OFF + wg * IF_TOK_BYTES;
+  const __nv_bfloat16* tok_k = reinterpret_cast<const __nv_bfloat16*>(tok);
+  const __nv_bfloat16* tok_v = tok_k + 16 * 128;
+  const uint32_t rs_off = frow * 128 + 4 * t;
+  mbar_wait(bar_w, 0);
+  uint32_t phase = 0;
+#pragma unroll 1
+  for (int tile = first; tile < num_tiles; tile += stride, phase ^= 1) {
+    const int row0 = tile * IF_TILE;
+    const int p = row0 / HW, prow = row0 - p * HW + frow;
+    {
+      const __nv_bfloat16* kp = ktok + static_cast<size_t>(p) * Tq * 128;
+      const __nv_bfloat16* vp = vtok + static_cast<size_t>(p) * Tq * 128;
+      for (int i = tw; i < 2 * Tq * 16; i += 128) {
+        const int which = i >= Tq * 16, j = i - which * Tq * 16;
+        cp_async16(smem_u32(tok) + which * (16 * 256) + j * 16, (which ? vp : kp) + j * 8);
+      }
+      asm volatile("cp.async.commit_group;" ::: "memory");
+    }
+    mbar_wait(bar_full, phase);
+    uint32_t qf[16][2];
+    {
+      float acc[64];
+      wgmma_fence();
+#pragma unroll
+      for (int kb = 0; kb < 4; ++kb) {
+#pragma unroll
+        for (int k = 0; k < 4; ++k)
+          Wgmma<128>::ss<0>(acc, make_gdesc(sa + kb * (IF_TILE * 128) + k * 32, 16, 1024),
+                            make_gdesc(s_wq + kb * (128 * 128) + k * 32, 16, 1024), (kb | k) != 0);
+      }
+      wgmma_commit();
+      uint32_t r[2][16];
+#pragma unroll
+      for (int j = 0; j < 16; ++j) {
+        r[0][j] = __ldg(reinterpret_cast<const unsigned int*>(pe_q + static_cast<size_t>(prow) * 128 + 8 * j + 2 * t));
+        r[1][j] = __ldg(reinterpret_cast<const unsigned int*>(pe_q + static_cast<size_t>(prow + 8) * 128 + 8 * j + 2 * t));
+      }
+      wgmma_wait<0>();
+      acc_fence(acc);
+#pragma unroll
+      for (int j = 0; j < 16; ++j) {
+        const float2 b = __ldg(reinterpret_cast<const float2*>(qb + 8 * j + 2 * t));
+        qf[j][0] = pack_bf16x2((acc[4 * j] + b.x) + __uint_as_float(r[0][j] << 16),
+                               (acc[4 * j + 1] + b.y) + __uint_as_float(r[0][j] & 0xffff0000u));
+        qf[j][1] = pack_bf16x2((acc[4 * j + 2] + b.x) + __uint_as_float(r[1][j] << 16),
+                               (acc[4 * j + 3] + b.y) + __uint_as_float(r[1][j] & 0xffff0000u));
+      }
+    }
+    asm volatile("cp.async.wait_group 0;" ::: "memory");
+    named_bar_sync(1 + wg, 128);
+    uint32_t af[8][4];
+#pragma unroll
+    for (int h = 0; h < 8; ++h) {
+      uint32_t kb[2][2], vb[2][2];
+      i2t_token_frags(tok_k + h * 16, tok_v + h * 16, Tq, scale, kb, vb);
+      const uint32_t qa[4] = {qf[2 * h][0], qf[2 * h][1], qf[2 * h + 1][0], qf[2 * h + 1][1]};
+      i2t_chunk(qa, kb, vb, Tq, af[h]);
+    }
+    float acc[128];
+    wgmma_fence();
+#pragma unroll
+    for (int h = 0; h < 8; ++h)
+      wgmma_rs_bf16_n256(acc, af[h], make_gdesc(s_wo + (h >> 2) * (256 * 128) + (h & 3) * 32, 16, 1024), h != 0);
+    wgmma_commit();
+    wgmma_wait<0>();
+    acc_fence(acc);
+#pragma unroll
+    for (int j = 0; j < 32; ++j) {
+      const uint32_t a0 = sa + (j >> 3) * (IF_TILE * 128) + rs_off + ((((j & 7) ^ g)) << 4);
+      uint32_t w0, w1;
+      asm volatile("ld.shared.b32 %0, [%1];" : "=r"(w0) : "r"(a0));
+      asm volatile("ld.shared.b32 %0, [%1];" : "=r"(w1) : "r"(a0 + 8 * 128));
+      const float2 b = *reinterpret_cast<const float2*>(vec + 8 * j + 2 * t);
+      acc[4 * j] = (acc[4 * j] + b.x) + __uint_as_float(w0 << 16);
+      acc[4 * j + 1] = (acc[4 * j + 1] + b.y) + __uint_as_float(w0 & 0xffff0000u);
+      acc[4 * j + 2] = (acc[4 * j + 2] + b.x) + __uint_as_float(w1 << 16);
+      acc[4 * j + 3] = (acc[4 * j + 3] + b.y) + __uint_as_float(w1 & 0xffff0000u);
+    }
+    float sum = 0.f, sumsq = 0.f, piv = 0.f;
+#pragma unroll
+    for (int jj = 0; jj < 16; ++jj) {
+      float rc[4][2];
+#pragma unroll
+      for (int r = 0; r < 4; ++r) {
+        const int cs = (t - r) & 3;
+        const int src = (lane & ~3) | ((t + r) & 3);
+#pragma unroll
+        for (int e = 0; e < 2; ++e) {
+          const float mine = sel4(cs, acc[4 * jj + e], acc[4 * jj + 2 + e], acc[4 * (16 + jj) + e],
+                                  acc[4 * (16 + jj) + 2 + e]);
+          rc[r][e] = __shfl_sync(0xffffffffu, mine, src);
+        }
+      }
+#pragma unroll
+      for (int s = 0; s < 4; ++s) {
+        const int r = (s - t) & 3;
+#pragma unroll
+        for (int e = 0; e < 2; ++e) {
+          const float v = sel4(r, rc[0][e], rc[1][e], rc[2][e], rc[3][e]);
+          if (jj == 0 && s == 0 && e == 0) piv = v;
+          const float d = v - piv;
+          sum += d;
+          sumsq = fmaf(d, d, sumsq);
+        }
+      }
+    }
+    const float mean_h = piv + sum * (1.0f / 128.0f);
+    const float m2_h = fmaxf(sumsq - sum * sum * (1.0f / 128.0f), 0.f);
+    const float ot_x = __shfl_xor_sync(0xffffffffu, mean_h, 2), ot_y = __shfl_xor_sync(0xffffffffu, m2_h, 2);
+    const float mean = 0.5f * (mean_h + ot_x);
+    const float dm = mean_h - ot_x;
+    const float var = (m2_h + ot_y + dm * dm * 64.0f) * (1.0f / 256.0f);
+    const float rstd = rsqrtf(var + eps);
+    const float mean0 = __shfl_sync(0xffffffffu, mean, lane & ~3), rstd0 = __shfl_sync(0xffffffffu, rstd, lane & ~3);
+    const float mean1 = __shfl_sync(0xffffffffu, mean, (lane & ~3) | 1);
+    const float rstd1 = __shfl_sync(0xffffffffu, rstd, (lane & ~3) | 1);
+#pragma unroll
+    for (int j = 0; j < 32; ++j) {
+      const uint32_t a0 = sa + (j >> 3) * (IF_TILE * 128) + rs_off + ((((j & 7) ^ g)) << 4);
+      const float2 gm = *reinterpret_cast<const float2*>(vec + 256 + 8 * j + 2 * t);
+      const float2 bt = *reinterpret_cast<const float2*>(vec + 512 + 8 * j + 2 * t);
+      const float y0 = fmaf((acc[4 * j] - mean0) * rstd0, gm.x, bt.x);
+      const float y1 = fmaf((acc[4 * j + 1] - mean0) * rstd0, gm.y, bt.y);
+      const float y2 = fmaf((acc[4 * j + 2] - mean1) * rstd1, gm.x, bt.x);
+      const float y3 = fmaf((acc[4 * j + 3] - mean1) * rstd1, gm.y, bt.y);
+      asm volatile("st.shared.b32 [%0], %1;" ::"r"(a0), "r"(pack_bf16x2(y0, y1)) : "memory");
+      asm volatile("st.shared.b32 [%0], %1;" ::"r"(a0 + 8 * 128), "r"(pack_bf16x2(y2, y3)) : "memory");
+    }
+    fence_proxy_async_smem();
+    named_bar_sync(1 + wg, 128);
+    if (tw == 0) {
+      for (int kb = 0; kb < 4; ++kb) tma_store_2d(&tma_out, sa + kb * (IF_TILE * 128), kb * 64, row0);
+      bulk_commit();
+      bulk_wait_read0();
+      if (tile + stride < num_tiles) load_tile(tile + stride);
+    }
+  }
+  if (tw == 0) bulk_wait0();
+}
+
+int i2t_fused(const void* keys, int ldk, const void* wq, const float* qb, const void* pe_q, const void* ktok,
+              const void* vtok, const void* wo, const float* ob, const float* ln_g, const float* ln_b, float eps,
+              void* out, int N, int Tq, int HW, cudaStream_t stream) {
+  RSP_CHECK_ARG(keys && wq && qb && pe_q && ktok && vtok && wo && ob && ln_g && ln_b && out, "i2t_fused: null pointer");
+  RSP_CHECK_ARG(N > 0 && Tq > 0 && Tq <= 16 && HW > 0 && HW % IF_TILE == 0 && static_cast<long long>(N) * HW < (1ll << 31),
+                "i2t_fused: N %d, Tq %d, HW %d (Tq <= 16, HW %% 64 == 0, N * HW < 2^31)", N, Tq, HW);
+  RSP_CHECK_ARG(ldk >= 256 && ldk % 8 == 0, "i2t_fused: keys row stride %d", ldk);
+  const uintptr_t a16 = reinterpret_cast<uintptr_t>(keys) | reinterpret_cast<uintptr_t>(wq) |
+                        reinterpret_cast<uintptr_t>(wo) | reinterpret_cast<uintptr_t>(out) |
+                        reinterpret_cast<uintptr_t>(ktok) | reinterpret_cast<uintptr_t>(vtok);
+  const uintptr_t a8 = reinterpret_cast<uintptr_t>(qb) | reinterpret_cast<uintptr_t>(ob) |
+                       reinterpret_cast<uintptr_t>(ln_g) | reinterpret_cast<uintptr_t>(ln_b);
+  RSP_CHECK_ARG((a16 & 15) == 0 && (a8 & 7) == 0 && (reinterpret_cast<uintptr_t>(pe_q) & 3) == 0,
+                "i2t_fused: operand alignment");
+  const uint64_t M = static_cast<uint64_t>(N) * HW;
+  CUtensorMap tk, to, tq, tw;
+  RSP_TRY(make_tmap_bf16_2d(&tk, keys, M, 256, static_cast<uint64_t>(ldk) * 2, IF_TILE, 64));
+  RSP_TRY(make_tmap_bf16_2d(&to, out, M, 256, 256 * 2, IF_TILE, 64));
+  RSP_TRY(make_tmap_bf16_2d(&tq, wq, 128, 256, 256 * 2, 128, 64));
+  RSP_TRY(make_tmap_bf16_2d(&tw, wo, 256, 128, 128 * 2, 256, 64));
+  static bool attr_set_dev[kMaxDevices] = {};
+  bool& attr_set = attr_set_dev[current_device()];
+  if (!attr_set) {
+    RSP_CHECK_CUDA(cudaFuncSetAttribute(i2t_fused_kernel, cudaFuncAttributeMaxDynamicSharedMemorySize, IF_SMEM));
+    attr_set = true;
+  }
+  const int num_tiles = static_cast<int>(M / IF_TILE);
+  const int grid = num_tiles < num_sms() ? num_tiles : num_sms();
+  i2t_fused_kernel<<<grid, IF_THREADS, IF_SMEM, stream>>>(
+      tk, to, tq, tw, qb, static_cast<const __nv_bfloat16*>(pe_q), static_cast<const __nv_bfloat16*>(ktok),
+      static_cast<const __nv_bfloat16*>(vtok), ob, ln_g, ln_b, eps, Tq, HW, num_tiles, 0.25f);
+  RSP_CHECK_LAUNCH();
+  return RSP_OK;
+}
+
+}
diff --git a/rsprompter_b200/csrc/decoder.h b/rsprompter_b200/csrc/decoder.h
--- a/rsprompter_b200/csrc/decoder.h
+++ b/rsprompter_b200/csrc/decoder.h
@@ -9,7 +9,12 @@
                          int heads, int c, cudaStream_t stream);
 int t2i_attention(const void* q, const void* K, const void* V, int ldkv, const int* kv_block, void* out, int N,
                   int Tq, int HW, cudaStream_t stream);
+int t2i_fused(const void* keys, int ldk, const void* kvw, const float* kvb, const void* pe_kv, const void* q,
+              void* out, int N, int Tq, int HW, cudaStream_t stream);
 int i2t_attention(const void* Q, const int* q_block, const void* ktok, const void* vtok, void* out,
                   int N, int Tq, int HW, cudaStream_t stream);
+int i2t_fused(const void* keys, int ldk, const void* wq, const float* qb, const void* pe_q, const void* ktok,
+              const void* vtok, const void* wo, const float* ob, const float* ln_g, const float* ln_b, float eps,
+              void* out, int N, int Tq, int HW, cudaStream_t stream);
 
 }
diff --git a/rsprompter_b200/csrc/sm90.cuh b/rsprompter_b200/csrc/sm90.cuh
--- a/rsprompter_b200/csrc/sm90.cuh
+++ b/rsprompter_b200/csrc/sm90.cuh
@@ -252,6 +252,40 @@
         : "r"(a[0]), "r"(a[1]), "r"(a[2]), "r"(a[3]), "l"(b));
   }
 };
+
+__device__ __forceinline__ void wgmma_rs_bf16_n256(float (&d)[128], const uint32_t (&a)[4], uint64_t b, uint32_t acc) {
+  asm volatile(
+      "{\n.reg .pred p;\n"
+      "setp.ne.b32 p, %133, 0;\n"
+      "wgmma.mma_async.sync.aligned.m64n256k16.f32.bf16.bf16 "
+      "{"
+      "%0, %1, %2, %3, %4, %5, %6, %7, %8, %9, %10, %11, %12, %13, %14, %15, "
+      "%16, %17, %18, %19, %20, %21, %22, %23, %24, %25, %26, %27, %28, %29, %30, %31, "
+      "%32, %33, %34, %35, %36, %37, %38, %39, %40, %41, %42, %43, %44, %45, %46, %47, "
+      "%48, %49, %50, %51, %52, %53, %54, %55, %56, %57, %58, %59, %60, %61, %62, %63, "
+      "%64, %65, %66, %67, %68, %69, %70, %71, %72, %73, %74, %75, %76, %77, %78, %79, "
+      "%80, %81, %82, %83, %84, %85, %86, %87, %88, %89, %90, %91, %92, %93, %94, %95, "
+      "%96, %97, %98, %99, %100, %101, %102, %103, %104, %105, %106, %107, %108, %109, %110, %111, "
+      "%112, %113, %114, %115, %116, %117, %118, %119, %120, %121, %122, %123, %124, %125, %126, %127"
+      "}, {%128, %129, %130, %131}, %132, p, 1, 1, 0;\n}\n"
+      : "+f"(d[0]), "+f"(d[1]), "+f"(d[2]), "+f"(d[3]), "+f"(d[4]), "+f"(d[5]), "+f"(d[6]), "+f"(d[7]),
+        "+f"(d[8]), "+f"(d[9]), "+f"(d[10]), "+f"(d[11]), "+f"(d[12]), "+f"(d[13]), "+f"(d[14]), "+f"(d[15]),
+        "+f"(d[16]), "+f"(d[17]), "+f"(d[18]), "+f"(d[19]), "+f"(d[20]), "+f"(d[21]), "+f"(d[22]), "+f"(d[23]),
+        "+f"(d[24]), "+f"(d[25]), "+f"(d[26]), "+f"(d[27]), "+f"(d[28]), "+f"(d[29]), "+f"(d[30]), "+f"(d[31]),
+        "+f"(d[32]), "+f"(d[33]), "+f"(d[34]), "+f"(d[35]), "+f"(d[36]), "+f"(d[37]), "+f"(d[38]), "+f"(d[39]),
+        "+f"(d[40]), "+f"(d[41]), "+f"(d[42]), "+f"(d[43]), "+f"(d[44]), "+f"(d[45]), "+f"(d[46]), "+f"(d[47]),
+        "+f"(d[48]), "+f"(d[49]), "+f"(d[50]), "+f"(d[51]), "+f"(d[52]), "+f"(d[53]), "+f"(d[54]), "+f"(d[55]),
+        "+f"(d[56]), "+f"(d[57]), "+f"(d[58]), "+f"(d[59]), "+f"(d[60]), "+f"(d[61]), "+f"(d[62]), "+f"(d[63]),
+        "+f"(d[64]), "+f"(d[65]), "+f"(d[66]), "+f"(d[67]), "+f"(d[68]), "+f"(d[69]), "+f"(d[70]), "+f"(d[71]),
+        "+f"(d[72]), "+f"(d[73]), "+f"(d[74]), "+f"(d[75]), "+f"(d[76]), "+f"(d[77]), "+f"(d[78]), "+f"(d[79]),
+        "+f"(d[80]), "+f"(d[81]), "+f"(d[82]), "+f"(d[83]), "+f"(d[84]), "+f"(d[85]), "+f"(d[86]), "+f"(d[87]),
+        "+f"(d[88]), "+f"(d[89]), "+f"(d[90]), "+f"(d[91]), "+f"(d[92]), "+f"(d[93]), "+f"(d[94]), "+f"(d[95]),
+        "+f"(d[96]), "+f"(d[97]), "+f"(d[98]), "+f"(d[99]), "+f"(d[100]), "+f"(d[101]), "+f"(d[102]), "+f"(d[103]),
+        "+f"(d[104]), "+f"(d[105]), "+f"(d[106]), "+f"(d[107]), "+f"(d[108]), "+f"(d[109]), "+f"(d[110]), "+f"(d[111]),
+        "+f"(d[112]), "+f"(d[113]), "+f"(d[114]), "+f"(d[115]), "+f"(d[116]), "+f"(d[117]), "+f"(d[118]), "+f"(d[119]),
+        "+f"(d[120]), "+f"(d[121]), "+f"(d[122]), "+f"(d[123]), "+f"(d[124]), "+f"(d[125]), "+f"(d[126]), "+f"(d[127])
+      : "r"(a[0]), "r"(a[1]), "r"(a[2]), "r"(a[3]), "l"(b), "r"(acc));
+}
 
 __device__ __forceinline__ uint32_t acc_row(uint32_t base, int ld, int row) {
   return base + static_cast<uint32_t>(row * ld) * 4u;
diff --git a/rsprompter_b200/sam_decoder.py b/rsprompter_b200/sam_decoder.py
--- a/rsprompter_b200/sam_decoder.py
+++ b/rsprompter_b200/sam_decoder.py
@@ -198,9 +198,12 @@
         def t2i(layer: dict, queries: torch.Tensor, keys_b: torch.Tensor, pos_kv: torch.Tensor, kv_blk, ln):
             qin = _lib.add_cast_bf16(queries, tokens)
             q = _lib.gemm(qin, layer["qw"], layer["qb"])
-            KV = _lib.gemm(keys_b, layer["kvw"], layer["kvb"], residual=pos_kv, res_mod=HW)
-            n_k = layer["kw"].shape[0]
-            att = _lib.t2i_attention(q.view(N, Tt, -1), KV[:, :n_k], KV[:, n_k:], HW, kv_block=kv_blk)
+            if kv_blk is None:
+                att = _lib.t2i_fused(q.view(N, Tt, -1), keys_b, layer["kvw"], layer["kvb"], pos_kv, HW)
+            else:
+                KV = _lib.gemm(keys_b, layer["kvw"], layer["kvb"], residual=pos_kv, res_mod=HW)
+                n_k = layer["kw"].shape[0]
+                att = _lib.t2i_attention(q.view(N, Tt, -1), KV[:, :n_k], KV[:, n_k:], HW, kv_block=kv_blk)
             return _lib.gemm(att.view(N * Tt, -1), layer["ow"], layer["ob"], residual=queries,
                              out_dtype=torch.float32, ln=ln)
 
@@ -232,10 +235,14 @@
             qin = _lib.add_cast_bf16(queries, tokens)
             ktok = _lib.gemm(qin, i2t["kw"], i2t["kb"])
             vtok = _lib.gemm(_lib.cast_bf16(queries), i2t["vw"], i2t["vb"])
-            Qimg = _lib.gemm(keys_b, i2t["qw"], i2t["qb"], residual=pt["q"][li], res_mod=HW)
-            att = _lib.i2t_attention(Qimg, ktok.view(N, Tt, -1), vtok.view(N, Tt, -1), HW, q_block=kblk)
-            keys_b = _lib.gemm(att, i2t["ow"], i2t["ob"], residual=keys_res, ln=(*L["ln4"], a.layer_norm_eps),
-                               res_block_map=kblk, res_block_rows=HW if kblk is not None else 0)
+            if kblk is None and HW % 64 == 0:
+                keys_b = _lib.i2t_fused(keys_b, i2t["qw"], i2t["qb"], pt["q"][li], ktok.view(N, Tt, -1),
+                                        vtok.view(N, Tt, -1), i2t["ow"], i2t["ob"], (*L["ln4"], a.layer_norm_eps), HW)
+            else:
+                Qimg = _lib.gemm(keys_b, i2t["qw"], i2t["qb"], residual=pt["q"][li], res_mod=HW)
+                att = _lib.i2t_attention(Qimg, ktok.view(N, Tt, -1), vtok.view(N, Tt, -1), HW, q_block=kblk)
+                keys_b = _lib.gemm(att, i2t["ow"], i2t["ob"], residual=keys_res, ln=(*L["ln4"], a.layer_norm_eps),
+                                   res_block_map=kblk, res_block_rows=HW if kblk is not None else 0)
             keys_res, kblk = keys_b, None
         queries = t2i(p["final"], queries, keys_b, pt["kv"][-1], None, (*p["lnf"], 1e-5))
         qv = queries.view(N, Tt, C)
```

Measured after the change: 46.55, median of 6. 7.2% higher.
